# liupei101/AdvMIL

Measured on AMD Instinct MI355X. Metric: WSI bags/sec (full G+D step), higher is better.
Workload: dtype bf16x3 (fp32 operands split hi+lo, 3 bf16 MFMAs per product, fp32 accumulate; fp32 storage); 1 GPU; ABMIL+AdvMIL(RLIP prj discriminator), 8192-patch x 1024 fp32 bags (BASELINE.json configs[1] shape; fp32 storage, bf16x3 split arithmetic: >= the bf16 the config names, within 2e-5 of the fp32 reference); gen_updates=1, distinct_resident_bags_per_gpu=64, parallelism=bag-parallel dp1, dropout=shipped rates, launch=hipGraph replay (4 captured bag groups)

## Files before the change

advmil_amd/_lib.py:

```python
import ctypes
import os
from ctypes import c_float, c_int, c_int32, c_int64, c_size_t, c_uint64, c_void_p

LIB_PATH = os.environ.get("ADVMIL_HIP_LIB") or os.path.join(os.path.dirname(os.path.abspath(__file__)), "libadvmil_hip.so")


class HipLibraryMissing(RuntimeError):
    pass


class AdvmilHipError(RuntimeError):
    pass


class Epilogue(ctypes.Structure):
    _fields_ = [("bias", c_void_p), ("act0", c_int), ("act1", c_int), ("act_split", c_int), ("drop_p", c_float),
                ("seed", c_void_p), ("stream_id", c_uint64), ("rowv", c_void_p), ("colv", c_void_p), ("rowseg", c_void_p),
                ("maskref", c_void_p), ("ldmask", c_int), ("mask_scale", c_float), ("accumulate", c_int),
                ("alpha", c_float), ("a_hi", c_void_p), ("a_lo", c_void_p), ("b_hi", c_void_p), ("b_lo", c_void_p),
                ("c_hi", c_void_p), ("c_lo", c_void_p), ("gate_wc", c_void_p), ("gate_out", c_void_p), ("gate_np", c_int),
                ("rng_row", c_void_p), ("c2", c_void_p), ("ldc2", c_int64), ("n_split", c_int64), ("bias2", c_void_p), ("colsum", c_void_p), ("maskbits", c_void_p), ("ldbits", c_int64),
                ("gate_bits_a", c_void_p), ("gate_bits_b", c_void_p), ("ldgbits", c_int64), ("c_rows_pair32", c_int)]


class DenseLayer(ctypes.Structure):
    _fields_ = [("W", c_void_p), ("bias", c_void_p), ("dW", c_void_p), ("dbias", c_void_p), ("y", c_void_p), ("K", c_int), ("N", c_int),
                ("act", c_int), ("drop_p", c_float), ("stream_id", c_uint64)]


TAIL_MAXL = 3


class DTail(ctypes.Structure):
    _fields_ = [("B", c_int), ("nx", c_int), ("ny", c_int), ("prj_src", c_int), ("xin", c_void_p), ("tin", c_void_p),
                ("x", DenseLayer * TAIL_MAXL), ("y", DenseLayer * TAIL_MAXL), ("u", c_void_p), ("w_prj", c_void_p), ("b_prj", c_void_p),
                ("dw_prj", c_void_p), ("db_prj", c_void_p), ("seed", c_void_p), ("rng_row", c_void_p), ("out", c_void_p),
                ("dout", c_void_p), ("dxin", c_void_p), ("dtin", c_void_p), ("du", c_void_p)]


class GemmTnCall(ctypes.Structure):
    _fields_ = [("M", c_int64), ("N", c_int64), ("K", c_int64), ("A", c_void_p), ("lda", c_int64), ("B", c_void_p), ("ldb", c_int64),
                ("C", c_void_p), ("ldc", c_int64), ("accumulate", ctypes.c_int32)]


class GHead(ctypes.Structure):
    _fields_ = [("B", ctypes.c_int32), ("d0", ctypes.c_int32), ("d1", ctypes.c_int32), ("d2", ctypes.c_int32), ("noise_mode", ctypes.c_int32),
                ("out_act", ctypes.c_int32), ("x", c_void_p), ("ldx", c_int64), ("Wr", c_void_p), ("br", c_void_p), ("W0", c_void_p),
                ("b0", c_void_p), ("W1", c_void_p), ("b1", c_void_p), ("p1", c_float), ("p2", c_float), ("seed", c_void_p),
                ("sid1", c_uint64), ("sid2", c_uint64), ("sid_noise", c_uint64), ("rng_row", c_void_p), ("noise", c_void_p),
                ("hs", c_void_p), ("h2", c_void_p), ("pred", c_void_p), ("dpred", c_void_p), ("dx", c_void_p), ("lddx", c_int64),
                ("dWr", c_void_p), ("dbr", c_void_p), ("dW0", c_void_p), ("db0", c_void_p), ("dW1", c_void_p), ("db1", c_void_p),
                ("ws", c_void_p), ("ws_bytes", c_size_t)]


class GHeadK(ctypes.Structure):
    _fields_ = [("B", ctypes.c_int32), ("d0", ctypes.c_int32), ("d1", ctypes.c_int32), ("d2", ctypes.c_int32), ("K", ctypes.c_int32),
                ("noise_mode", ctypes.c_int32), ("out_act", ctypes.c_int32), ("reserved", ctypes.c_int32)] + GHead._fields_[6:]


class Optim(ctypes.Structure):
    _fields_ = [("kind", ctypes.c_int32), ("lookahead", ctypes.c_int32), ("n", c_int64), ("p", c_void_p), ("grad", c_void_p),
                ("s1", c_void_p), ("s2", c_void_p), ("wd", c_void_p), ("slow", c_void_p), ("lr", ctypes.c_double),
                ("beta1", ctypes.c_double), ("beta2", ctypes.c_double), ("eps", ctypes.c_double), ("schedule_decay", ctypes.c_double),
                ("grad_scale", c_float), ("l1_coef", c_float), ("la_alpha", c_float), ("la_k", ctypes.c_int32), ("tick", ctypes.c_int32),
                ("step", c_void_p), ("la_state", c_void_p), ("m_sched", c_void_p), ("p_hi", c_void_p), ("p_lo", c_void_p),
                ("abs_partial", c_void_p), ("clear_grad", ctypes.c_int32)]


OPT_KINDS = {"adam": 0, "adamw": 1, "nadam": 2, "radam": 3, "adadelta": 4}

CINDEX_BOOT_ROW_TILE = 256
CINDEX_BOOT_RESAMPLE_CHUNK = 8
CINDEX_BOOT_MAX_CHUNK_BLOCKS = 4096


SIGNATURES = {
    "advmil_version": (c_int, []),
    "advmil_gemm_f32_workspace_bytes": (c_size_t, [c_int64, c_int64, c_int]),
    "advmil_gemm_f32": (c_int, [c_int, c_int, c_int64, c_int64, c_int64, c_void_p, c_int64, c_void_p, c_int64, c_void_p,
                                c_int64, ctypes.POINTER(Epilogue), c_int, c_void_p, c_size_t, c_void_p]),
    "advmil_split_planes": (c_int, [c_void_p, c_int64, c_void_p, c_void_p, c_void_p]),
    "advmil_stage_bag": (c_int, [c_void_p, c_void_p, c_size_t, c_void_p, c_void_p, c_void_p, c_void_p, c_size_t, c_void_p]),
    "advmil_stage_bag_masked": (c_int, [c_void_p, c_void_p, c_size_t, c_int64, c_void_p, c_void_p, c_void_p, c_void_p, c_size_t, c_void_p,
                                        c_void_p]),
    "advmil_gate_interleave": (c_int, [c_void_p, c_void_p, c_void_p, c_void_p, c_int, c_void_p, c_void_p, c_void_p, c_void_p, c_int, c_void_p]),
    "advmil_gate_partial_sum": (c_int, [c_void_p, c_int, c_void_p, c_int64, c_void_p, c_void_p]),
    "advmil_gemm_f32_gate_blocks": (c_int, [c_int, c_int64]),
    "advmil_gemm_f32_colsum_rows": (c_int64, [c_int, c_int64, c_int64]),
    "advmil_merge_partials": (c_int, [c_void_p, c_int, c_int64, c_int64, c_void_p, c_int, c_void_p]),
    "advmil_set_gemm_mode": (c_int, [c_int]),
    "advmil_get_gemm_mode": (c_int, []),
    "advmil_gemm_f32_plan": (c_int, [c_int64, c_int64, c_int64, ctypes.POINTER(c_int), ctypes.POINTER(c_int)]),
    "advmil_gemm_f32_plan_layout": (c_int, [c_int, c_int, c_int64, c_int64, c_int64, ctypes.POINTER(c_int), ctypes.POINTER(c_int)]),
    "advmil_gemm_f32_plan_planes": (c_int, [c_int, c_int, c_int64, c_int64, c_int64, ctypes.POINTER(c_int)]),
    "advmil_gemm_f32_plan_tn_planes": (c_int, [c_int64, c_int64, c_int64, ctypes.POINTER(c_int), ctypes.POINTER(c_int)]),
    "advmil_gemm_f32_tiled": (c_int, [c_int, c_int, c_int64, c_int64, c_int64, c_void_p, c_int64, c_void_p, c_int64, c_void_p,
                                      c_int64, ctypes.POINTER(Epilogue), c_int, c_int, c_void_p, c_size_t, c_void_p]),
    "advmil_mha_fwd": (c_int, [c_void_p, c_void_p, c_int64, c_int, c_int, c_int, c_void_p, c_int64, c_float, c_void_p, c_uint64,
                               c_void_p, c_void_p, c_void_p, c_void_p]),
    "advmil_mha_fwd_lse": (c_int, [c_void_p, c_void_p, c_int64, c_int, c_int, c_int, c_void_p, c_int64, c_float, c_void_p, c_uint64,
                                   c_void_p, c_void_p, c_void_p, c_void_p]),
    "advmil_mha_bwd_workspace_bytes": (c_size_t, [c_int64, c_int, c_int]),
    "advmil_mha_bwd": (c_int, [c_void_p, c_void_p, c_void_p, c_void_p, c_void_p, c_int64, c_int, c_int, c_int, c_void_p, c_int64,
                               c_float, c_void_p, c_uint64, c_void_p, c_void_p, c_void_p, c_size_t, c_void_p]),
    "advmil_mha_bwd1_workspace_bytes": (c_size_t, [c_int64, c_int, c_int, c_int64]),
    "advmil_mha_bwd1": (c_int, [c_void_p, c_void_p, c_void_p, c_void_p, c_void_p, c_int64, c_int, c_int, c_int, c_void_p, c_int64,
                                c_float, c_void_p, c_uint64, c_void_p, c_void_p, c_void_p, c_size_t, c_void_p]),
    "advmil_add_dropout_ln_fwd": (c_int, [c_void_p, c_void_p, c_void_p, c_void_p, c_float, c_int64, c_int64, c_float, c_void_p,
                                          c_uint64, c_void_p, c_void_p, c_void_p, c_void_p, c_void_p, c_void_p, c_void_p, c_void_p]),
    "advmil_add_dropout_ln_bwd_workspace_bytes": (c_size_t, [c_int64, c_int64]),
    "advmil_add_dropout_ln_bwd": (c_int, [c_void_p, c_void_p, c_void_p, c_void_p, c_void_p, c_int64, c_int64, c_float, c_void_p,
                                          c_uint64, c_void_p, c_void_p, c_void_p, c_void_p, c_void_p, c_int, c_void_p, c_size_t,
                                          c_void_p]),
    "advmil_gate_score_fwd": (c_int, [c_void_p, c_void_p, c_void_p, c_float, c_void_p, c_uint64, c_uint64, c_int64, c_int64,
                                      c_void_p, c_void_p, c_void_p]),
    "advmil_softmax_pool_workspace_bytes": (c_size_t, [c_int64, c_int64, c_int]),
    "advmil_softmax_pool_fwd": (c_int, [c_void_p, c_void_p, c_int64, c_int64, c_int64, c_int, c_void_p, c_int64, c_void_p,
                                        c_void_p, c_void_p, c_size_t, c_void_p]),
    "advmil_softmax_pool_mean_workspace_bytes": (c_size_t, [c_int64, c_int64, c_int]),
    "advmil_softmax_pool_mean_fwd": (c_int, [c_void_p, c_void_p, c_int64, c_int64, c_int64, c_int, c_void_p, c_int64, c_void_p,
                                             c_void_p, c_void_p, c_void_p, c_size_t, c_void_p]),
    "advmil_softmax_pool_bwd": (c_int, [c_void_p, c_void_p, c_void_p, c_void_p, c_int64, c_int64, c_int64, c_int, c_void_p,
                                        c_int64, c_void_p, c_void_p, c_size_t, c_void_p]),
    "advmil_softmax_pool_fwd_planes": (c_int, [c_void_p, c_void_p, c_void_p, c_int64, c_int64, c_int64, c_int, c_void_p, c_int64, c_void_p,
                                               c_void_p, c_void_p, c_size_t, c_void_p]),
    "advmil_softmax_pool_bwd_planes": (c_int, [c_void_p, c_void_p, c_void_p, c_void_p, c_void_p, c_int64, c_int64, c_int64, c_int, c_void_p,
                                               c_int64, c_void_p, c_void_p, c_size_t, c_void_p]),
    "advmil_dropout_planes": (c_int, [c_void_p, c_void_p, c_int64, c_int64, c_float, c_void_p, c_uint64, c_void_p, c_void_p, c_void_p, c_void_p,
                                      c_float, c_uint64, c_uint64, c_void_p, c_void_p, c_void_p]),
    "advmil_gate_bwd_workspace_bytes": (c_size_t, [c_int64, c_int64]),
    "advmil_gate_bwd": (c_int, [c_void_p, c_void_p, c_void_p, c_float, c_void_p, c_uint64, c_uint64, c_int64, c_int64,
                                c_void_p, c_void_p, c_void_p, c_void_p, c_int, c_void_p, c_void_p, c_void_p, c_int, c_void_p, c_size_t,
                                c_void_p]),
    "advmil_colsum_workspace_bytes": (c_size_t, [c_int64, c_int64]),
    "advmil_act_dropout_bwd": (c_int, [c_void_p, c_void_p, c_int, c_float, c_void_p, c_uint64, c_int64, c_int64, c_void_p,
                                       c_void_p, c_int, c_void_p, c_void_p, c_void_p, c_void_p, c_void_p, c_size_t, c_void_p]),
    "advmil_colsum": (c_int, [c_void_p, c_int64, c_int64, c_void_p, c_int, c_void_p, c_size_t, c_void_p]),
    "advmil_ln_relu_mean16_fwd": (c_int, [c_void_p, c_void_p, c_void_p, c_float, c_int64, c_int64, c_void_p, c_void_p,
                                          c_void_p, c_void_p, c_void_p, c_int, c_void_p]),
    "advmil_ln_relu_mean16_bwd_workspace_bytes": (c_size_t, [c_int64, c_int64]),
    "advmil_ln_relu_mean16_bwd": (c_int, [c_void_p, c_void_p, c_void_p, c_void_p, c_void_p, c_void_p, c_int64, c_int64,
                                          c_void_p, c_void_p, c_void_p, c_int, c_void_p, c_void_p, c_void_p, c_int, c_void_p, c_size_t, c_void_p]),
    "advmil_ln_relu_fwd": (c_int, [c_void_p, c_void_p, c_void_p, c_float, c_int64, c_int64, c_void_p, c_void_p, c_void_p, c_void_p]),
    "advmil_ln_relu_bwd_workspace_bytes": (c_size_t, [c_int64, c_int64]),
    "advmil_ln_relu_bwd": (c_int, [c_void_p, c_void_p, c_void_p, c_void_p, c_void_p, c_void_p, c_int64, c_int64, c_void_p,
                                   c_void_p, c_void_p, c_int, c_void_p, c_size_t, c_void_p]),
    "advmil_gcn_res_fwd": (c_int, [c_void_p, c_void_p, c_int64, c_void_p, c_void_p, c_float, c_int64, c_int64, c_float, c_void_p,
                                   c_uint64, c_void_p, c_void_p, c_int64, c_void_p, c_void_p, c_void_p]),
    "advmil_gcn_res_bwd_workspace_bytes": (c_size_t, [c_int64, c_int64]),
    "advmil_gcn_res_bwd": (c_int, [c_void_p, c_int64, c_void_p, c_void_p, c_void_p, c_void_p, c_void_p, c_int64, c_int64, c_float,
                                   c_void_p, c_uint64, c_void_p, c_void_p, c_void_p, c_int64, c_int, c_void_p, c_void_p, c_int,
                                   c_void_p, c_size_t, c_void_p]),
    "advmil_gapool16_fwd": (c_int, [c_void_p, c_void_p, c_int64, c_int64, c_int64, c_void_p, c_void_p, c_int, c_void_p]),
    "advmil_gapool16_bwd": (c_int, [c_void_p, c_void_p, c_void_p, c_int64, c_int64, c_int64, c_int, c_void_p, c_void_p, c_int, c_void_p]),
    "advmil_genconv_fwd": (c_int, [c_void_p, c_void_p, c_void_p, c_void_p, c_float, c_int64, c_int64, c_void_p, c_void_p,
                                   c_void_p, c_void_p]),
    "advmil_genconv_bwd_workspace_bytes": (c_size_t, [c_int64, c_int64]),
    "advmil_genconv_bwd": (c_int, [c_void_p, c_void_p, c_void_p, c_void_p, c_void_p, c_void_p, c_void_p, c_float, c_int64,
                                   c_int64, c_void_p, c_void_p, c_void_p, c_size_t, c_void_p]),
    "advmil_adam_step": (c_int, [c_void_p, c_void_p, c_void_p, c_void_p, c_void_p, c_int64, c_float, c_float, c_float,
                                 c_float, c_float, c_float, c_void_p, c_void_p, c_void_p, c_int, c_void_p, c_int, c_void_p]),
    "advmil_adam_blocks": (c_int, [c_int64]),
    "advmil_optim_step": (c_int, [ctypes.POINTER(Optim), c_void_p]),
    "advmil_step_seed_tick": (c_int, [c_void_p, c_void_p, c_void_p, c_uint64, c_void_p]),
    "advmil_abs_sum": (c_int, [c_void_p, c_int64, c_void_p, c_void_p, c_size_t, c_void_p]),
    "advmil_abs_sum_workspace_bytes": (c_size_t, [c_int64]),
    "advmil_uniform_fill": (c_int, [c_void_p, c_int64, c_void_p, c_uint64, c_void_p, c_int64, c_void_p]),
    "advmil_dropout_apply": (c_int, [c_void_p, c_void_p, c_int64, c_float, c_void_p, c_uint64, c_void_p, c_int64, c_void_p]),
    "advmil_seed_advance": (c_int, [c_void_p, c_uint64, c_void_p]),
    "advmil_seg_scale_rows": (c_int, [c_void_p, c_void_p, c_void_p, c_int64, c_int64, c_void_p, c_void_p]),
    "advmil_stamp_clock": (c_int, [c_void_p, c_void_p]),
    "advmil_clock_rate_khz": (c_int64, []),
    "advmil_small_linear_fwd": (c_int, [c_void_p, c_int64, c_void_p, c_void_p, c_int, c_int, c_int, c_int, c_float, c_void_p, c_uint64,
                                        c_void_p, c_void_p, c_void_p]),
    "advmil_small_linear_bwd_workspace_bytes": (c_size_t, [c_int, c_int]),
    "advmil_small_linear_bwd": (c_int, [c_void_p, c_void_p, c_void_p, c_int64, c_void_p, c_int, c_int, c_int, c_int, c_float, c_void_p,
                                        c_uint64, c_void_p, c_void_p, c_int, c_void_p, c_int, c_void_p, c_int64, c_void_p, c_size_t, c_void_p]),
    "advmil_skinny_linear_fwd": (c_int, [c_void_p, c_void_p, c_void_p, c_int, c_int, c_int, c_int, c_void_p, c_void_p]),
    "advmil_skinny_linear_bwd": (c_int, [c_void_p, c_void_p, c_void_p, c_void_p, c_int, c_int, c_int, c_int, c_void_p, c_void_p,
                                         c_void_p, c_int, c_void_p]),
    "advmil_prj_head_fwd": (c_int, [c_void_p, c_void_p, c_void_p, c_void_p, c_void_p, c_int, c_int, c_void_p, c_void_p]),
    "advmil_prj_head_bwd": (c_int, [c_void_p, c_void_p, c_void_p, c_void_p, c_void_p, c_int, c_int, c_void_p, c_void_p, c_void_p, c_void_p,
                                    c_void_p, c_int, c_void_p]),
    "advmil_gan_d_loss": (c_int, [c_void_p, c_int, c_void_p, c_void_p, c_int, c_int, c_float, c_float, c_void_p, c_void_p, c_void_p, c_void_p]),
    "advmil_gan_g_loss": (c_int, [c_void_p, c_void_p, c_void_p, c_void_p, c_void_p, c_int, c_float, c_float, c_int, c_float, c_float,
                                  c_float, c_void_p, c_void_p, c_void_p, c_void_p]),
    "advmil_gan_g_loss_disc": (c_int, [c_void_p, c_void_p, c_void_p, c_void_p, c_void_p, c_int, c_int, c_float, c_float, c_float, c_float,
                                       c_float, c_void_p, c_void_p, c_void_p, c_void_p]),
    "advmil_mask_rows": (c_int, [c_void_p, c_void_p, c_int64, c_int64, c_void_p, c_void_p]),
    "advmil_dx_chain_fwd": (c_int, [c_void_p, c_int64, c_int, c_void_p, c_void_p, c_void_p, c_void_p, c_void_p, c_void_p, c_void_p, c_void_p,
                                    c_void_p, c_void_p, c_void_p, c_float, c_float, c_void_p, c_uint64, c_uint64, c_uint64, c_void_p, c_void_p,
                                    c_void_p, c_void_p, c_void_p, c_void_p]),
    "advmil_dx_chain_bwd_workspace_bytes": (c_size_t, [c_int64, c_int]),
    "advmil_dx_chain_prep": (c_int, [c_void_p, c_void_p, c_void_p, c_int, c_void_p, c_void_p, c_void_p, c_void_p, c_void_p, c_void_p, c_void_p]),
    "advmil_dx_chain_bwd": (c_int, [c_int64, c_int, c_void_p, c_void_p, c_void_p, c_void_p, c_void_p, c_void_p, c_void_p, c_void_p, c_void_p,
                                    c_void_p, c_float, c_float, c_void_p, c_uint64, c_uint64, c_void_p, c_void_p, c_void_p, c_void_p, c_void_p,
                                    c_void_p, c_void_p, c_void_p, c_void_p, c_void_p, c_void_p, c_void_p, c_void_p, c_void_p, c_void_p, c_void_p,
                                    c_void_p, c_size_t, c_void_p]),
    "advmil_dtail_fwd": (c_int, [ctypes.POINTER(DTail), c_void_p]),
    "advmil_dtail_bwd": (c_int, [ctypes.POINTER(DTail), c_void_p]),
    "advmil_gemm_tn_group_workspace_bytes": (c_size_t, [ctypes.POINTER(GemmTnCall), c_int]),
    "advmil_gemm_tn_group": (c_int, [ctypes.POINTER(GemmTnCall), c_int, c_void_p, c_size_t, c_void_p]),
    "advmil_ghead_workspace_bytes": (c_size_t, [c_int, c_int, c_int, c_int]),
    "advmil_ghead_fwd": (c_int, [ctypes.POINTER(GHead), c_void_p]),
    "advmil_ghead_bwd": (c_int, [ctypes.POINTER(GHead), c_void_p]),
    "advmil_gheadk_workspace_bytes": (c_size_t, [c_int, c_int, c_int, c_int, c_int]),
    "advmil_gheadk_fwd": (c_int, [ctypes.POINTER(GHeadK), c_void_p]),
    "advmil_gheadk_bwd": (c_int, [ctypes.POINTER(GHeadK), c_void_p]),
# ... 69 lines not shown
```

advmil_amd/csrc/gemm_core.h:

```cpp
#pragma once
#include <cstdlib>
#include "common.h"
#include "bf16split.h"
#include "sumq.h"
#include "../../include/advmil_hip.h"

#define BK 32
#define PITCH_KC 36

#define WAVE_LDS_SYNC()                                   \
  do {                                                    \
    __builtin_amdgcn_fence(__ATOMIC_RELEASE, "wavefront"); \
    __builtin_amdgcn_s_waitcnt(0xc07f);                   \
    __builtin_amdgcn_wave_barrier();                      \
    __builtin_amdgcn_fence(__ATOMIC_ACQUIRE, "wavefront"); \
  } while (0)

struct GemmArgs {
  int64_t M, N, K;
  const float* A; int64_t lda;
  const float* B; int64_t ldb;
  float* C; int64_t ldc;
  int64_t k_chunk;
  float* ws;
  int splits;
  int mtiles, ntiles;
  advmil_epilogue_t epi;
};

__device__ __forceinline__ float epilogue_elem(const advmil_epilogue_t& e, float acc, int64_t m, int64_t n, int64_t N,
                                               uint64_t key, float inv_keep) {
  float v = acc * e.alpha;
  if (e.bias) v += e.bias[n];
  if (e.rowv) v += e.rowv[m] * e.colv[(e.rowseg ? (int64_t)e.rowseg[m] * N : 0) + n];
  v = act_apply(n < e.act_split ? e.act0 : e.act1, v);
  if (e.seed && e.drop_p > 0.0f) v *= rng_keep(key, (uint64_t)((e.rng_row ? e.rng_row[m] : m) * N + n), e.drop_p, inv_keep);
  if (e.maskref) v *= (e.maskref[m * (int64_t)e.ldmask + n] > 0.0f ? e.mask_scale : 0.0f);
  return v;
}

template <bool KC, int ROWS, int BKT, int NT>
__device__ __forceinline__ void load_tile(const float* __restrict__ src, int64_t ld, int64_t row0, int64_t rows,
                                          int64_t k0, int64_t kend, int tid, float4 (&r)[ROWS * BKT / (4 * NT)]) {
#pragma unroll
  for (int p = 0; p < ROWS * BKT / (4 * NT); ++p) {
    const int e = p * NT + tid;
    if (KC) {
      const int64_t row = row0 + e / (BKT / 4);
      const int64_t k = k0 + (e % (BKT / 4)) * 4;
      r[p] = (row < rows && k < kend) ? *reinterpret_cast<const float4*>(src + row * ld + k) : make_float4(0.f, 0.f, 0.f, 0.f);
    } else {
      const int64_t k = k0 + e / (ROWS / 4);
      const int64_t m = row0 + (e % (ROWS / 4)) * 4;
      r[p] = (k < kend && m < rows) ? *reinterpret_cast<const float4*>(src + k * ld + m) : make_float4(0.f, 0.f, 0.f, 0.f);
    }
  }
}

template <bool KC, int ROWS, int BKT, int NT>
__device__ __forceinline__ void store_tile(float* __restrict__ s, int tid, const float4 (&r)[ROWS * BKT / (4 * NT)]) {
#pragma unroll
  for (int p = 0; p < ROWS * BKT / (4 * NT); ++p) {
    const int e = p * NT + tid;
    if (KC)
      *reinterpret_cast<float4*>(s + (e / (BKT / 4)) * (BKT + 4) + (e % (BKT / 4)) * 4) = r[p];
    else
      *reinterpret_cast<float4*>(s + (e / (ROWS / 4)) * ROWS + (e % (ROWS / 4)) * 4) = r[p];
  }
}

template <bool KC, int ROWS, int BKT>
__device__ __forceinline__ void read_frag(const float* __restrict__ s, int rbase, int t4, int i, int hi, float (&f)[4]) {
  if (KC) {
    const float4 v = *reinterpret_cast<const float4*>(s + (rbase + i) * (BKT + 4) + t4 * 8 + hi * 4);
    f[0] = v.x; f[1] = v.y; f[2] = v.z; f[3] = v.w;
  } else {
#pragma unroll
    for (int u = 0; u < 4; ++u) f[u] = s[(t4 * 8 + hi * 4 + u) * ROWS + rbase + i];
  }
}


#define PITCH_PS(BKT) (BKT)
__device__ __forceinline__ int ps_unit(int row, int unit, int units_per_row) {
  return units_per_row == 2 ? (unit ^ ((row >> 3) & 1)) : (unit ^ ((row >> 2) & (units_per_row - 1)));
}

template <int ROWS, int BKT, int NT>
__device__ __forceinline__ void store_tile_presplit(bf16raw* __restrict__ planes, int tid, const float4 (&r)[ROWS * BKT / (4 * NT)]) {
  bf16raw* const hiP = planes;
  bf16raw* const loP = planes + ROWS * PITCH_PS(BKT);
#pragma unroll
  for (int p = 0; p < ROWS * BKT / (4 * NT); ++p) {
    const int e = p * NT + tid;
    const int row = e / (BKT / 4), p4 = e % (BKT / 4);
    const int off = row * PITCH_PS(BKT) + ps_unit(row, p4 >> 1, BKT / 8) * 8 + (p4 & 1) * 4;
    uint2 h, l;
    split4(r[p], h, l);
    *reinterpret_cast<uint2*>(hiP + off) = h;
    *reinterpret_cast<uint2*>(loP + off) = l;
  }
}

template <int ROWS, int BKT>
__device__ __forceinline__ void read_frag_presplit(const bf16raw* __restrict__ planes, int rbase, int ks, int i, int hi,
                                                   bf16x8& h, bf16x8& l) {
  const int row = rbase + i;
  const bf16raw* p = planes + row * PITCH_PS(BKT) + ps_unit(row, ks * 2 + hi, BKT / 8) * 8;
  Frag8 a, b;
  a.u = *reinterpret_cast<const uint4*>(p);
  b.u = *reinterpret_cast<const uint4*>(p + ROWS * PITCH_PS(BKT));
  h = a.v; l = b.v;
}

template <int BKT>
__device__ __forceinline__ void read_frag_hi(const bf16raw* __restrict__ planes, int rbase, int ks, int i, int hi, bf16x8& h) {
  const int row = rbase + i;
  Frag8 a;
  a.u = *reinterpret_cast<const uint4*>(planes + row * PITCH_PS(BKT) + ps_unit(row, ks * 2 + hi, BKT / 8) * 8);
  h = a.v;
}

#define PITCH_MC(ROWS) ((ROWS) + 32)

template <int ROWS, int BKT, int NT>
__device__ __forceinline__ void store_tile_presplit_mc(bf16raw* __restrict__ planes, int tid, const float4 (&r)[ROWS * BKT / (4 * NT)]) {
  bf16raw* const hiP = planes;
  bf16raw* const loP = planes + BKT * PITCH_MC(ROWS);
#pragma unroll
  for (int p = 0; p < ROWS * BKT / (4 * NT); ++p) {
    const int e = p * NT + tid;
    const int k = e / (ROWS / 4), m4 = (e % (ROWS / 4)) * 4;
    uint2 h, l;
    split4(r[p], h, l);
    *reinterpret_cast<uint2*>(hiP + k * PITCH_MC(ROWS) + m4) = h;
    *reinterpret_cast<uint2*>(loP + k * PITCH_MC(ROWS) + m4) = l;
  }
}

template <int ROWS, int BKT>
__device__ __forceinline__ void read_frag_presplit_mc(const bf16raw* __restrict__ planes, int rbase, int ks, int lane,
                                                      bf16x8& h, bf16x8& l) {
  const int krow = ks * 16 + (lane >> 5) * 8 + ((lane & 15) >> 2);
  const int mcol = rbase + ((lane >> 4) & 1) * 16 + (lane & 3) * 4;
  const bf16raw* p = planes + krow * PITCH_MC(ROWS) + mcol;
  union { bf16x4_t q[2]; bf16x8 v; } a, b;
  a.q[0] = __builtin_amdgcn_ds_read_tr16_b64_v4bf16((LDS_AS bf16x4_t*)(p));
  a.q[1] = __builtin_amdgcn_ds_read_tr16_b64_v4bf16((LDS_AS bf16x4_t*)(p + 4 * PITCH_MC(ROWS)));
  b.q[0] = __builtin_amdgcn_ds_read_tr16_b64_v4bf16((LDS_AS bf16x4_t*)(p + BKT * PITCH_MC(ROWS)));
  b.q[1] = __builtin_amdgcn_ds_read_tr16_b64_v4bf16((LDS_AS bf16x4_t*)(p + (BKT + 4) * PITCH_MC(ROWS)));
  h = a.v; l = b.v;
}

__device__ __forceinline__ void emit_planes4(const advmil_epilogue_t& e, int64_t off, const float (&v)[4], int nvalid) {
  union { __bf16 b[4]; uint2 u; bf16raw r[4]; } h, l;
#pragma unroll
  for (int j = 0; j < 4; ++j) {
    h.b[j] = (__bf16)v[j];
    l.b[j] = (__bf16)(v[j] - (float)h.b[j]);
  }
  bf16raw* ch = reinterpret_cast<bf16raw*>(e.c_hi) + off;
  bf16raw* cl = reinterpret_cast<bf16raw*>(e.c_lo) + off;
  if (nvalid == 4 && ((off & 3) == 0)) {
    *reinterpret_cast<uint2*>(ch) = h.u;
    *reinterpret_cast<uint2*>(cl) = l.u;
  } else {
#pragma unroll
    for (int j = 0; j < 4; ++j)
// ... 37 lines not shown

  __device__ __forceinline__ void store(bf16raw* __restrict__ planes, int tid) const {
    if constexpr (!PRE) {
      if (KC) store_tile_presplit<ROWS, BKT, NT>(planes, tid, f);
      else store_tile_presplit_mc<ROWS, BKT, NT>(planes, tid, f);
    } else {
#pragma unroll
      for (int p = 0; p < NP; ++p) {
        const int e = p * NT + tid;
        if (!FULL && e >= NPIECE) break;
        if (KC) {
          const int row = e / (BKT / 8);
          bf16raw* d = planes + row * PITCH_PS(BKT) + ps_unit(row, e % (BKT / 8), BKT / 8) * 8;
          *reinterpret_cast<uint4*>(d) = ph[p];
          *reinterpret_cast<uint4*>(d + ROWS * PITCH_PS(BKT)) = pl[p];
        } else {
          bf16raw* d = planes + (e / (ROWS / 8)) * PITCH_MC(ROWS) + (e % (ROWS / 8)) * 8;
          *reinterpret_cast<uint4*>(d) = ph[p];
          *reinterpret_cast<uint4*>(d + BKT * PITCH_MC(ROWS)) = pl[p];
        }
      }
    }
  }
};

#define EPI_WAVE_FLOATS(TM, TN) (32 * PITCH_KC + 32 * ((TN) + 2 * (TM)) + 32 * (TM) * (TN))

template <int TM, int TN, int WR, int WC, bool PLAIN = false>
__device__ __forceinline__ void gemm_epilogue_stream(const GemmArgs& g, f32x16 (&acc)[TM][TN], float* patch, int lane, int wr, int wc,
                                                     int64_t m0, int64_t n0, uint64_t key, float inv_keep, int nt_i = 0) {
  const advmil_epilogue_t& e = g.epi;
  const int i = lane & 31, hi = lane >> 5;
  const int c4 = (lane & 7) * 4, rq = lane >> 3;
  const int64_t N = g.N, ldo = g.ldc;
  float* const out = g.C;
  const bool drop = !PLAIN && e.seed && e.drop_p > 0.0f;
  const bool mapped = drop && e.rng_row;
  const int kind = PLAIN ? 0 : (e.rowv ? 1 : (e.maskref ? 2 : (e.accumulate ? 3 : 0)));
  const bool rmask = !PLAIN && kind == 1 && e.maskref != nullptr;
  const bool csum = !PLAIN && e.colsum != nullptr;
  const bool bmask = !PLAIN && e.maskbits != nullptr;
  const bool gpair = PLAIN && e.gate_wc != nullptr && e.gate_bits_a != nullptr;
  const float* const xbase = kind == 1 ? e.colv : (kind == 2 ? e.maskref : out);
  const int64_t xld = kind == 1 ? N : (kind == 2 ? (int64_t)e.ldmask : ldo);
  const int64_t rbase = m0 + wr * 32 * TM, cbase = n0 + wc * 32 * TN;
  const int64_t nsp = (PLAIN && e.c2) ? e.n_split : N;
  float* const sbias = patch + 32 * PITCH_KC;
  int* const srow_i = reinterpret_cast<int*>(sbias + 32 * TN);
  float* const srow_f = sbias + 32 * TN + 32 * TM;
  uint32_t* const smask = reinterpret_cast<uint32_t*>(sbias + 32 * TN + 64 * TM);
  if (gpair) {
    constexpr int NW = 32 * TM * TN;
    uint32_t mv[(NW + 63) / 64];
#pragma unroll
    for (int u = 0; u < (NW + 63) / 64; ++u) {
      const int idx = u * 64 + lane;
      const int br = idx & 1, pu = (idx >> 1) % (TN / 2), row = (idx >> 1) / (TN / 2);
      const uint32_t* src = br ? e.gate_bits_b : e.gate_bits_a;
      mv[u] = idx < NW ? src[(rbase + row) * e.ldgbits + (cbase >> 6) + pu] : 0u;
    }
#pragma unroll
    for (int u = 0; u < (NW + 63) / 64; ++u)
      if (u * 64 + lane < NW) smask[u * 64 + lane] = mv[u];
  }
  if (bmask) {
    uint32_t mv[(32 * TM * TN + 63) / 64];
#pragma unroll
    for (int u = 0; u < (32 * TM * TN + 63) / 64; ++u) {
      const int idx = u * 64 + lane;
      mv[u] = idx < 32 * TM * TN ? e.maskbits[(rbase + idx / TN) * e.ldbits + (cbase >> 5) + idx % TN] : 0u;
    }
#pragma unroll
    for (int u = 0; u < (32 * TM * TN + 63) / 64; ++u)
      if (u * 64 + lane < 32 * TM * TN) smask[u * 64 + lane] = mv[u];
  }
  {
    float bv[(32 * TN + 63) / 64];
    int iv[(32 * TM + 63) / 64];
    float fv[(32 * TM + 63) / 64];
#pragma unroll
    for (int u = 0; u < (32 * TN + 63) / 64; ++u) {
      const int c = u * 64 + lane;
      const int64_t cg = cbase + c;
      bv[u] = c >= 32 * TN ? 0.f : (cg < nsp ? (e.bias ? e.bias[cg] : 0.f) : (e.bias2 ? e.bias2[cg - nsp] : 0.f));
    }
#pragma unroll
    for (int u = 0; u < (32 * TM + 63) / 64; ++u) {
      const int r = u * 64 + lane;
      const bool ok = r < 32 * TM;
      iv[u] = !ok ? 0 : (kind == 1 ? (e.rowseg ? e.rowseg[rbase + r] : 0) : (mapped ? (int)e.rng_row[rbase + r] : 0));
      fv[u] = (ok && kind == 1) ? e.rowv[rbase + r] : ((gpair && r < 16 * TN) ? e.gate_wc[(cbase >> 1) + r] : 0.f);
    }
#pragma unroll
    for (int u = 0; u < (32 * TN + 63) / 64; ++u)
      if (u * 64 + lane < 32 * TN) sbias[u * 64 + lane] = bv[u];
#pragma unroll
    for (int u = 0; u < (32 * TM + 63) / 64; ++u)
      if (u * 64 + lane < 32 * TM) { srow_i[u * 64 + lane] = iv[u]; srow_f[u * 64 + lane] = fv[u]; }
    WAVE_LDS_SYNC();
  }
  float4 ext[4], ext2[4];
  float cs[TN][4];
  float gpa[4][4], gps[TM][4];
#pragma unroll
  for (int a_ = 0; a_ < TM; ++a_)
#pragma unroll
    for (int q = 0; q < 4; ++q) gps[a_][q] = 0.f;
#pragma unroll
  for (int q = 0; q < 4; ++q) { ext[q] = make_float4(0.f, 0.f, 0.f, 0.f); ext2[q] = make_float4(1.f, 1.f, 1.f, 1.f); }
#pragma unroll
  for (int b = 0; b < TN; ++b)
#pragma unroll
    for (int t = 0; t < 4; ++t) cs[b][t] = 0.f;
#define ADVMIL_EPI_PREFETCH(a_, b_)                                                                             \
  do {                                                                                                          \
    if (kind != 0) {                                                                                            \
      _Pragma("unroll") for (int q = 0; q < 4; ++q) {                                                           \
        const int rr_ = (a_) * 32 + q * 8 + rq;                                                                 \
        const int64_t xrow_ = kind == 1 ? (int64_t)srow_i[rr_] : rbase + rr_;                                   \
        ext[q] = *reinterpret_cast<const float4*>(xbase + xrow_ * xld + cbase + (b_) * 32 + c4);                \
        if (rmask) ext2[q] = *reinterpret_cast<const float4*>(e.maskref + (rbase + rr_) * (int64_t)e.ldmask + cbase + (b_) * 32 + c4); \
      }                                                                                                         \
    }                                                                                                           \
  } while (0)
  ADVMIL_EPI_PREFETCH(0, 0);
#pragma unroll
  for (int a = 0; a < TM; ++a) {
#pragma unroll
    for (int b = 0; b < TN; ++b) {
      const int64_t col = cbase + b * 32 + c4;
#pragma unroll
      for (int r = 0; r < 16; ++r) patch[((r & 3) + 8 * (r >> 2) + 4 * hi) * PITCH_KC + i] = acc[a][b][r];
      WAVE_LDS_SYNC();
      float res[4][4];
#pragma unroll
      for (int q = 0; q < 4; ++q) {
        const float4 v4 = *reinterpret_cast<const float4*>(patch + (q * 8 + rq) * PITCH_KC + c4);
        res[q][0] = v4.x; res[q][1] = v4.y; res[q][2] = v4.z; res[q][3] = v4.w;
      }
      const float4 b4 = *reinterpret_cast<const float4*>(sbias + b * 32 + c4);
      WAVE_LDS_SYNC();
      const int act = gpair ? ((b & 1) ? ACT_SIGMOID : ACT_TANH) : (cbase + b * 32 < e.act_split ? e.act0 : e.act1);
      const float bb[4] = {b4.x, b4.y, b4.z, b4.w};
      if (!drop && kind == 0 && !bmask) {
        const float al = e.alpha;
        if (act == ACT_RELU) {
#pragma unroll
          for (int q = 0; q < 4; ++q)
#pragma unroll
            for (int t = 0; t < 4; ++t) res[q][t] = fmaxf(res[q][t] * al + bb[t], 0.0f);
        } else if (act == ACT_NONE) {
#pragma unroll
          for (int q = 0; q < 4; ++q)
#pragma unroll
            for (int t = 0; t < 4; ++t) res[q][t] = res[q][t] * al + bb[t];
        } else if (act == ACT_TANH) {
#pragma unroll
          for (int q = 0; q < 4; ++q)
#pragma unroll
            for (int t = 0; t < 4; ++t) res[q][t] = act_apply(ACT_TANH, res[q][t] * al + bb[t]);
        } else {
#pragma unroll
          for (int q = 0; q < 4; ++q)
#pragma unroll
            for (int t = 0; t < 4; ++t) res[q][t] = act_apply(ACT_SIGMOID, res[q][t] * al + bb[t]);
        }
      } else if (!drop && kind == 1 && act == ACT_NONE && !rmask && !bmask) {
// ... 124 lines not shown
#pragma unroll
      for (int q = 0; q < 4; ++q) {
        float t = gps[a_][q];
        t += __shfl_xor(t, 1, 64); t += __shfl_xor(t, 2, 64); t += __shfl_xor(t, 4, 64);
        if ((lane & 7) == 0) e.gate_out[(rbase + a_ * 32 + q * 8 + rq) * e.gate_np + nt_i * WC + wc] = t;
      }
  }
  if (csum) {
    const int64_t prow = (m0 / (32 * TM * WR)) * WR + wr;
#pragma unroll
    for (int b = 0; b < TN; ++b) {
#pragma unroll
      for (int t = 0; t < 4; ++t) {
        float v = cs[b][t];
        v += __shfl_xor(v, 8, 64); v += __shfl_xor(v, 16, 64); v += __shfl_xor(v, 32, 64);
        cs[b][t] = v;
      }
      if (rq == 0) *reinterpret_cast<float4*>(e.colsum + prow * N + cbase + b * 32 + c4) = make_float4(cs[b][0], cs[b][1], cs[b][2], cs[b][3]);
    }
  }
}

template <int TM, int TN, int WR, int WC, bool RAWBAR = false, int EPI = 0>
__device__ __forceinline__ int gemm_epilogue(const GemmArgs& g, f32x16 (&acc)[TM][TN], float* smem, int wave, int lane, int wr, int wc,
                                             int64_t m0, int64_t n0, int z, int nt_i) {
  const int i = lane & 31, hi = lane >> 5;
  const advmil_epilogue_t& e = g.epi;
  const bool direct = (g.splits == 1);
  uint64_t key = 0;
  float inv_keep = 1.0f;
  if (direct && e.seed && e.drop_p > 0.0f) {
    key = rng_key(*e.seed, e.stream_id);
    inv_keep = hw_rcp(1.0f - e.drop_p);
  } else if (direct && e.gate_bits_a && e.drop_p > 0.0f) {
    inv_keep = hw_rcp(1.0f - e.drop_p);
  }
  float* const out = direct ? g.C : g.ws + (int64_t)z * g.M * g.N;
  const int64_t ldo = direct ? g.ldc : g.N;
  const bool vec_ok = ((ldo & 3) == 0) && (((uintptr_t)out & 15) == 0);
  float* const patch = smem + wave * EPI_WAVE_FLOATS(TM, TN);
  if constexpr (RAWBAR) {
    asm volatile("s_waitcnt lgkmcnt(0)" ::: "memory");
    __builtin_amdgcn_s_barrier();
    asm volatile("" ::: "memory");
  } else {
    __syncthreads();
  }
  const bool gate_store = direct && e.gate_wc != nullptr && e.gate_bits_a != nullptr;
  const bool gate_mode = direct && e.gate_wc != nullptr && !gate_store;
  if constexpr (TM * TN >= 4 && EPI != 1) {
    const int nmode = (e.rowv && e.maskref && !e.accumulate) ? 1 : (e.rowv ? 1 : 0) + (e.maskref ? 1 : 0) + (e.accumulate ? 1 : 0);
    const bool stream = direct && !gate_mode && vec_ok && (g.N % (32 * TN * WC)) == 0 && (g.M % (32 * TM * WR)) == 0 && (e.act_split & 31) == 0 &&
                        nmode <= 1 && !(e.rowv && e.seed && e.rng_row) && (!e.bias || ((uintptr_t)e.bias & 15) == 0) && (!e.rowv || ((uintptr_t)e.colv & 15) == 0) &&
                        (!e.maskref || ((e.ldmask & 3) == 0 && ((uintptr_t)e.maskref & 15) == 0)) &&
                        (!e.c_hi || ((((uintptr_t)e.c_hi) | ((uintptr_t)e.c_lo)) & 7) == 0) &&
                        (!e.c2 || ((((uintptr_t)e.c2) & 15) == 0 && (e.ldc2 & 3) == 0 && (e.n_split & 31) == 0));
    if (stream) {
      if constexpr (EPI == 2) {
        if (nmode == 0 && !(e.seed && e.drop_p > 0.0f)) {
          gemm_epilogue_stream<TM, TN, WR, WC, true>(g, acc, patch, lane, wr, wc, m0, n0, key, inv_keep, nt_i);
          return TM * TN * 4;
        }
      } else {
        gemm_epilogue_stream<TM, TN, WR, WC>(g, acc, patch, lane, wr, wc, m0, n0, key, inv_keep);
        return nmode == 0 ? TM * TN * 4 : 0;
      }
    }
  }
#pragma unroll
  for (int a = 0; a < TM; ++a) {
    float gsum[4] = {0.f, 0.f, 0.f, 0.f};
#pragma unroll
    for (int b = 0; b < TN; ++b) {
#pragma unroll
      for (int r = 0; r < 16; ++r) patch[((r & 3) + 8 * (r >> 2) + 4 * hi) * PITCH_KC + i] = acc[a][b][r];
      WAVE_LDS_SYNC();
      const int64_t rbase = m0 + wr * 32 * TM + a * 32;
      if (gate_mode) {
        const int64_t col = n0 + wc * 32 * TN + b * 32 + (lane & 7) * 4;
        float w0 = 0.f, w1 = 0.f;
        float4 b4 = make_float4(0.f, 0.f, 0.f, 0.f);
        if (col < g.N) {
          w0 = e.gate_wc[col >> 1]; w1 = e.gate_wc[(col >> 1) + 1];
          if (e.bias) b4 = *reinterpret_cast<const float4*>(e.bias + col);
        }
#pragma unroll
        for (int q = 0; q < 4; ++q) {
          const int pr = q * 8 + (lane >> 3);
          const float4 v4 = *reinterpret_cast<const float4*>(patch + pr * PITCH_KC + (lane & 7) * 4);
          const float t0 = act_apply(ACT_TANH, v4.x * e.alpha + b4.x), s0 = act_apply(ACT_SIGMOID, v4.y * e.alpha + b4.y);
          const float t1 = act_apply(ACT_TANH, v4.z * e.alpha + b4.z), s1 = act_apply(ACT_SIGMOID, v4.w * e.alpha + b4.w);
          gsum[q] += t0 * s0 * w0 + t1 * s1 * w1;
        }
        WAVE_LDS_SYNC();
        continue;
      }
      const int64_t col = n0 + wc * 32 * TN + b * 32 + (lane & 7) * 4;
      const int nvalid = col >= g.N ? 0 : ((g.N - col >= 4) ? 4 : (int)(g.N - col));
      float bias4[4] = {0.f, 0.f, 0.f, 0.f};
      int act4[4];
#pragma unroll
      for (int t = 0; t < 4; ++t) {
        if (direct && e.bias && t < nvalid) bias4[t] = e.bias[col + t];
        act4[t] = (col + t) < e.act_split ? e.act0 : e.act1;
      }
      const bool same_act = act4[0] == act4[3];
#pragma unroll 1
      for (int q = 0; q < 4; ++q) {
        const int pr = q * 8 + (lane >> 3);
        const int64_t row = rbase + pr;
        const float4 v4 = *reinterpret_cast<const float4*>(patch + pr * PITCH_KC + (lane & 7) * 4);
        float v[4] = {v4.x, v4.y, v4.z, v4.w};
        if (row < g.M && nvalid > 0) {
          float* c = out + row * ldo + col;
          if (direct) {
            float r1 = 0.f;
            const float* cv = nullptr;
            const int64_t grow = (e.seed && e.rng_row) ? e.rng_row[row] : row;
            if (e.rowv) {
              r1 = e.rowv[row];
              cv = e.colv + (e.rowseg ? (int64_t)e.rowseg[row] * g.N : 0) + col;
            }
#pragma unroll
            for (int t = 0; t < 4; ++t)
              if (t < nvalid) {
                float x = v[t] * e.alpha + bias4[t];
                if (cv) x += r1 * cv[t];
                x = act_apply(same_act ? act4[0] : act4[t], x);
                if (e.seed && e.drop_p > 0.0f) x *= rng_keep(key, (uint64_t)(grow * g.N + col + t), e.drop_p, inv_keep);
                if (e.maskref) x *= (e.maskref[row * (int64_t)e.ldmask + col + t] > 0.0f ? e.mask_scale : 0.0f);
                if (e.accumulate) x += c[t];
                v[t] = x;
              }
          }
          if (!out) {
          } else if (nvalid == 4 && vec_ok) {
            *reinterpret_cast<float4*>(c) = make_float4(v[0], v[1], v[2], v[3]);
          } else {
#pragma unroll
            for (int t = 0; t < 4; ++t)
              if (t < nvalid) c[t] = v[t];
          }
          if (direct && e.c_hi) emit_planes4(e, row * ldo + col, v, nvalid);
        }
      }
      WAVE_LDS_SYNC();
    }
    if (gate_mode) {
#pragma unroll
      for (int q = 0; q < 4; ++q) {
        float t = gsum[q];
        t += __shfl_xor(t, 1, 64); t += __shfl_xor(t, 2, 64); t += __shfl_xor(t, 4, 64);
        const int64_t row = m0 + wr * 32 * TM + a * 32 + q * 8 + (lane >> 3);
        if ((lane & 7) == 0 && row < g.M) e.gate_out[row * e.gate_np + nt_i * WC + wc] = t;
      }
    }
  }
  return 0;
}

#define GLB_AS __attribute__((address_space(1)))
template <int N>
__device__ __forceinline__ void wait_vmcnt() { asm volatile("s_waitcnt vmcnt(%0)" ::"n"(N) : "memory"); }
```

advmil_amd/csrc/gemm_host.hip:

```cpp
#include "gemm_core.h"

int advmil_launch_generic(int tile, int a_kc, int b_kc, int pre, dim3 grid, hipStream_t stream, const GemmArgs& g);
int advmil_launch_nt_planes(int tile, bool a_single, dim3 pgrid, hipStream_t stream, const GemmArgs& g);
int advmil_launch_tn_planes(int tile, bool b_single, dim3 tgrid, hipStream_t stream, const GemmArgs& g);
int advmil_launch_splitk_reduce(const GemmArgs& g, hipStream_t stream);

extern "C" size_t advmil_gemm_f32_workspace_bytes(int64_t M, int64_t N, int splits) {
  return splits > 1 ? (size_t)splits * (size_t)M * (size_t)N * sizeof(float) : 0;
}

int g_gemm_mode = 0;
static int g_nt_planes = []() { const char* e = getenv("ADVMIL_NT_PLANES"); return (e && e[0] == '0') ? 0 : 1; }();
extern "C" int advmil_set_gemm_mode(int mode) {
  if (mode != 0 && mode != 1) return ADVMIL_EINVAL;
  g_gemm_mode = mode;
  return ADVMIL_OK;
}
extern "C" int advmil_get_gemm_mode(void) { return g_gemm_mode; }

static int planes_usable(const void* hi, const void* lo, int64_t ld, int64_t contiguous_extent) {
  return hi && !((uintptr_t)hi & 15) && !((uintptr_t)lo & 15) && !(ld & 7) && !(contiguous_extent & 7);
}

static int64_t n_tiles(int tile, int64_t M, int64_t N) {
// ... 132 lines not shown
  return ((M % bm) || (N % bn)) ? 0 : (M / bm) * wr;
}

static int device_cus() {
  static const int ncu = []() { int dev = 0, n = 0; hipGetDevice(&dev); hipDeviceGetAttribute(&n, hipDeviceAttributeMultiprocessorCount, dev); return n > 0 ? n : 256; }();
  return ncu;
}

extern "C" int advmil_merge_partials(const float* partial, int nblk, int64_t stride, int64_t ncols, float* out, int accumulate,
                                     advmil_stream_t stream) {
  if (!partial || !out || nblk <= 0 || ncols <= 0 || stride < ncols) return ADVMIL_EINVAL;
  return advmil_sumq((hipStream_t)stream, partial, nblk, stride, ncols, out, accumulate);
}

extern "C" int advmil_gemm_f32_tiled(int a_kc, int b_kc, int64_t M, int64_t N, int64_t K, const float* A, int64_t lda,
                                     const float* B, int64_t ldb, float* C, int64_t ldc, const advmil_epilogue_t* epi,
                                     int splits, int tile, void* ws, size_t ws_bytes, advmil_stream_t stream_) {
  hipStream_t stream = (hipStream_t)stream_;
  if (!A || !B || !epi || (!C && !epi->gate_wc && !epi->c_hi) || M <= 0 || N <= 0 || K <= 0) return ADVMIL_EINVAL;
  if (!C && !epi->gate_wc && (epi->accumulate || splits != 1 || (epi->c2 && tile != 85 && tile != 86))) return ADVMIL_EINVAL;
  if ((lda & 3) || (ldb & 3)) return ADVMIL_EINVAL;
  if (lda < (a_kc ? K : M) || ldb < (b_kc ? K : N)) return ADVMIL_EINVAL;
  if (ldc < (epi->c2 ? (int64_t)epi->n_split : N) && (C || epi->c_hi)) return ADVMIL_EINVAL;
  if (a_kc ? (K & 3) : (M & 3)) return ADVMIL_EINVAL;
  if (b_kc ? (K & 3) : (N & 3)) return ADVMIL_EINVAL;
  if (((uintptr_t)A & 15) || ((uintptr_t)B & 15)) return ADVMIL_EINVAL;
  if (splits < 1) splits = 1;
  const int64_t kchunks = (K + BK - 1) / BK;
  if (splits > kchunks) splits = (int)kchunks;
  if (splits > 1 && (N & 3)) return ADVMIL_EINVAL;
  GemmArgs g;
  g.M = M; g.N = N; g.K = K; g.A = A; g.lda = lda; g.B = B; g.ldb = ldb; g.C = C; g.ldc = ldc;
  g.k_chunk = ((kchunks + splits - 1) / splits) * BK;
  splits = (int)((K + g.k_chunk - 1) / g.k_chunk);
  g.splits = splits;
  g.ws = (float*)ws;
  g.epi = *epi;
  if (splits > 1) {
    if (!ws || ws_bytes < advmil_gemm_f32_workspace_bytes(M, N, splits)) return ADVMIL_EWORKSPACE;
    if ((uintptr_t)ws & 15) return ADVMIL_EINVAL;
  }
  if (tile == 0) { int t = 0, sp = 0; advmil_gemm_f32_plan_layout(a_kc, b_kc, M, N, K, &t, &sp); tile = t; }
  if (g_gemm_mode != 1) {
    if (tile / 10 == 4) tile = 20 + tile % 10;
    else if (tile % 10 == 4) tile = (tile / 10 == 3) ? 23 : 22;
  }
  const int tm = tile / 10, tn = tile % 10;
  g.mtiles = (int)((M + 64 * tm - 1) / (64 * tm));
  const int ntiles = (int)((N + 64 * tn - 1) / (64 * tn));
  g.ntiles = ntiles;
  dim3 grid(g.mtiles * ntiles, splits);
  int pre = 0;
  if (g_gemm_mode == 1) {
    if (planes_usable(epi->a_hi, epi->a_lo, lda, a_kc ? K : M)) pre |= 1;
    if (planes_usable(epi->b_hi, epi->b_lo, ldb, b_kc ? K : N)) pre |= 2;
  }
  if ((epi->c_hi != nullptr) != (epi->c_lo != nullptr)) return ADVMIL_EINVAL;
  if (epi->c_rows_pair32 && (splits < 2 || !epi->accumulate || (M & 63) || ldc != N)) return ADVMIL_EINVAL;
  if (epi->maskbits) {
    int tm_, tn_, wr_, wc_;
    if (g_gemm_mode != 1 || splits != 1 || !tile_geom(tile, tm_, tn_, wr_, wc_) || tm_ * tn_ < 4 || epi->gate_wc || epi->maskref || epi->accumulate ||
        (M % (32 * tm_ * wr_)) || (N % (32 * tn_ * wc_)) || (epi->act_split & 31) || epi->ldbits < N / 32 || (epi->seed && epi->drop_p > 0.0f && epi->rowv && epi->rng_row))
      return ADVMIL_EINVAL;
    if ((C && ((((uintptr_t)C) & 15) || (ldc & 3))) || (((uintptr_t)epi->bias) & 15) || (epi->rowv && (((uintptr_t)epi->colv) & 15)) ||
        (epi->c_hi && ((((uintptr_t)epi->c_hi) | ((uintptr_t)epi->c_lo)) & 7)) || epi->c2)
      return ADVMIL_EINVAL;
  }
  if (epi->colsum) {
    int tm_, tn_, wr_, wc_;
    if (g_gemm_mode != 1 || splits != 1 || !tile_geom(tile, tm_, tn_, wr_, wc_) || tm_ * tn_ < 4 || epi->gate_wc || epi->accumulate ||
        (epi->seed && epi->drop_p > 0.0f))
      return ADVMIL_EINVAL;
    if ((M % (32 * tm_ * wr_)) || (N % (32 * tn_ * wc_)) || (((uintptr_t)epi->colsum) & 15) || (epi->act_split & 31)) return ADVMIL_EINVAL;
  }
  const bool gate_store = epi->gate_wc && epi->gate_bits_a;
  if (gate_store && (!epi->gate_bits_b || !C || (tile != 85 && tile != 86) || epi->seed || !(epi->drop_p > 0.0f) || epi->drop_p >= 1.0f ||
                     (N & 127) || epi->ldgbits < N / 64 || epi->c2 || epi->c_hi || (((uintptr_t)epi->gate_wc) & 15)))
    return ADVMIL_EINVAL;
  if (epi->gate_wc) {
    if (splits != 1 || !epi->gate_out || (N & 3) || (epi->drop_p > 0.0f && !gate_store)) return ADVMIL_EINVAL;
    if (epi->gate_np != advmil_gemm_f32_gate_blocks(tile, N)) return ADVMIL_EINVAL;
  }
  if (tile == 0 && pre == 3 && splits == 1) { int t = 0; advmil_gemm_f32_plan_planes(a_kc, b_kc, M, N, K, &t); if (t) tile = t; }
  if (tile == 87) {
    if (epi->gate_wc || epi->rowv || epi->maskref || epi->maskbits || epi->colsum || epi->accumulate || epi->c2 || (epi->seed && epi->drop_p > 0.0f))
      return ADVMIL_EINVAL;
    if (g_gemm_mode != 1 || !a_kc || !b_kc || pre != 3 || splits != 1 || (M % 512) || N != 128 || K < 64 || (K % 32) || !epi->b_lo) return ADVMIL_EINVAL;
    if ((uint64_t)M * (uint64_t)lda * 2 >= (1ull << 32) || (uint64_t)N * (uint64_t)ldb * 2 >= (1ull << 32)) return ADVMIL_EINVAL;
    g.mtiles = (int)(M / 512);
    g.ntiles = 1;
    const int cus = device_cus();
    return advmil_launch_nt_planes(tile, !epi->a_lo, dim3(g.mtiles < cus ? g.mtiles : cus), stream, g);
  }
  if (tile >= 82 && tile <= 86) {
    const int tnp = tile == 85 ? 4 : tile == 86 ? 2 : tile % 10, bm = 256, bkt = 32;
    const bool plain = tile == 85 || tile == 86;
    if (tile == 84 && !epi->gate_wc) return ADVMIL_EINVAL;
    if (plain && ((epi->gate_wc && !gate_store) || epi->rowv || epi->maskref || epi->accumulate || (epi->seed && epi->drop_p > 0.0f))) return ADVMIL_EINVAL;
    if (epi->c2) {
      if (!plain || epi->n_split <= 0 || epi->n_split >= N || (epi->n_split & 31) || (epi->ldc2 & 3) || ((uintptr_t)epi->c2 & 15) ||
          epi->act_split != epi->n_split)
        return ADVMIL_EINVAL;
      if ((ldc & 3) || (((uintptr_t)C) & 15) || (((uintptr_t)epi->bias) & 15) || (epi->c_hi && ((((uintptr_t)epi->c_hi) | ((uintptr_t)epi->c_lo)) & 7)))
        return ADVMIL_EINVAL;
    }
    if (g_gemm_mode != 1 || !a_kc || !b_kc || pre != 3 || splits != 1 || (M % bm) || (K % bkt) || (N % (64 * tnp))) return ADVMIL_EINVAL;
    if (epi->gate_wc && (!epi->gate_out || (epi->drop_p > 0.0f && !gate_store) || epi->gate_np != advmil_gemm_f32_gate_blocks(tile, N))) return ADVMIL_EINVAL;
    if (K < 64) return ADVMIL_EINVAL;
    if ((uint64_t)M * (uint64_t)lda * 2 >= (1ull << 32) || (uint64_t)N * (uint64_t)ldb * 2 >= (1ull << 32)) return ADVMIL_EINVAL;
    g.mtiles = (int)(M / bm);
    g.ntiles = (int)(N / (64 * tnp));
    const int ncu = device_cus();
    const int ntile_all = g.mtiles * g.ntiles;
    dim3 pgrid(ntile_all < ncu ? ntile_all : ncu);
    if (!epi->b_lo) return ADVMIL_EINVAL;
    return advmil_launch_nt_planes(tile, !epi->a_lo, pgrid, stream, g);
  }
  if (tile >= 91 && tile <= 93) {
    const int bm = tile == 91 ? 128 : 256, bn = tile == 92 ? 128 : 256;
    if (g_gemm_mode != 1 || a_kc || b_kc || pre != 3 || (M % bm) || (N % bn) || (K % 32) || (g.k_chunk % 32)) return ADVMIL_EINVAL;
    if (g.k_chunk / 32 < 3 || epi->gate_wc || epi->c2) return ADVMIL_EINVAL;
    if ((uint64_t)32 * (uint64_t)lda * 2 + (uint64_t)M * 2 >= (1ull << 32) || (uint64_t)32 * (uint64_t)ldb * 2 + (uint64_t)N * 2 >= (1ull << 32)) return ADVMIL_EINVAL;
    g.mtiles = (int)(M / bm);
    g.ntiles = (int)(N / bn);
    const int gs = M >= N ? g.ntiles : g.mtiles, og = M >= N ? g.mtiles : g.ntiles;
    const dim3 tgrid((unsigned)(8 * ((splits * og + 7) / 8) * gs));
    if (!epi->a_lo) return ADVMIL_EINVAL;
    { const int rc = advmil_launch_tn_planes(tile, !epi->b_lo, tgrid, stream, g); if (rc) return rc; }
    if (splits > 1) {
      const int rc = advmil_launch_splitk_reduce(g, stream);
      if (rc) return rc;
    }
    return ADVMIL_OK;
  }
  { const int rc = advmil_launch_generic(tile, a_kc, b_kc, pre, grid, stream, g); if (rc) return rc; }
  if (splits > 1) {
    const int rc = advmil_launch_splitk_reduce(g, stream);
    if (rc) return rc;
  }
  return ADVMIL_OK;
}

extern "C" int advmil_gemm_f32(int a_kc, int b_kc, int64_t M, int64_t N, int64_t K, const float* A, int64_t lda,
                               const float* B, int64_t ldb, float* C, int64_t ldc, const advmil_epilogue_t* epi,
                               int splits, void* ws, size_t ws_bytes, advmil_stream_t stream) {
  return advmil_gemm_f32_tiled(a_kc, b_kc, M, N, K, A, lda, B, ldb, C, ldc, epi, splits, 0, ws, ws_bytes, stream);
}
```

advmil_amd/csrc/gemm_nt_planes.hip:

```cpp
#include "gemm_core.h"


template <int TN, int NBUF, int WR, int BKT, int EPI = 0, int ALO = 1, int TM = 2>
__global__ __launch_bounds__(128 * WR, 2) void gemm_nt_planes_kernel(GemmArgs g) {
  constexpr int WC = 2, NW = WR * WC;
  constexpr int BM_ = 32 * TM * WR, BN_ = 64 * TN;
  constexpr int AROWS = (1 + ALO) * BM_;
  constexpr int ROWS_ALL = AROWS + 2 * BN_;
  constexpr int RPP = 512 / BKT, LPR = BKT / 8;
  constexpr int NPIECE = ROWS_ALL / RPP, PPW = NPIECE / NW;
  static_assert(NPIECE % NW == 0, "pieces must divide evenly over the waves");
  constexpr int BUF_HW = ROWS_ALL * BKT;
  constexpr int PATCH_FLOATS = NW * EPI_WAVE_FLOATS(TM, TN);
  constexpr bool EPI_IN_SLOT = PATCH_FLOATS <= BUF_HW / 2;
  static_assert(EPI_IN_SLOT || ALO == 0, "the epilogue area must fit one ring slot");
  constexpr int EST = TM * TN * 4;
  static_assert(EST + PPW <= 63, "counted waits are 6-bit");
  __shared__ __attribute__((aligned(16))) float smem[NBUF * BUF_HW / 2 + (EPI_IN_SLOT ? 0 : PATCH_FLOATS)];
  bf16raw* const lds = reinterpret_cast<bf16raw*>(smem);
  const int wave = __builtin_amdgcn_readfirstlane((int)threadIdx.x >> 6);
  const int wr = wave / WC, wc = wave % WC;
  const int ntile = g.mtiles * g.ntiles, G = (int)gridDim.x;
  auto tile_of = [&](int v, int& mt, int& nt) {
    const int inner = g.ntiles, outer = g.mtiles;
    const int per_group = 8 * inner, full = (outer / 8) * per_group;
    if (v < full) {
      const int r = v % per_group;
      mt = (v / per_group) * 8 + (r & 7);
      nt = r >> 3;
    } else {
      const int rem = outer - (outer / 8) * 8, r = v - full;
      mt = (outer / 8) * 8 + r % rem;
      nt = r / rem;
    }
  };
  int v = (int)blockIdx.x;
  int mt_i, nt_i;
  tile_of(v, mt_i, nt_i);
  uint32_t soff[PPW];
  auto set_src = [&](int mt, int nt, int lane) {
#pragma unroll
    for (int it = 0; it < PPW; ++it) {
      const int prow = (wave + NW * it) * RPP + lane / LPR;
      int r;
      int64_t ld, row0;
      if (prow < BM_) { r = prow; ld = g.lda; row0 = (int64_t)mt * BM_; }
      else if (prow < AROWS) { r = prow - BM_; ld = g.lda; row0 = (int64_t)mt * BM_; }
      else if (prow < AROWS + BN_) { r = prow - AROWS; ld = g.ldb; row0 = (int64_t)nt * BN_; }
      else { r = prow - AROWS - BN_; ld = g.ldb; row0 = (int64_t)nt * BN_; }
      soff[it] = (uint32_t)(((row0 + r) * ld + ps_unit(r, lane % LPR, LPR) * 8) * 2);
    }
  };
  set_src(mt_i, nt_i, (int)threadIdx.x & 63);
  int64_t dA = 0, dB = 0;
  auto dma = [&](int buf, int64_t k0, bool next) {
#pragma unroll
    for (int it = 0; it < PPW; ++it) {
      const int p0 = (wave + NW * it) * RPP;
      const char* base = reinterpret_cast<const char*>(p0 < BM_ ? g.epi.a_hi : (p0 < AROWS ? g.epi.a_lo : (p0 < AROWS + BN_ ? g.epi.b_hi : g.epi.b_lo)));
      base += (k0 + (next ? (p0 < AROWS ? dA : dB) : 0)) * 2;
      __builtin_amdgcn_global_load_lds((const GLB_AS void*)(base + soff[it]), (LDS_AS void*)(lds + buf * BUF_HW + (wave + NW * it) * 512), 16, 0, 0);
    }
  };
  const int64_t K = g.K;
  const int C = (int)(K / BKT);
  dma(0, 0, false);
  if (NBUF == 3) dma(1, BKT, false);
  int cur = 0;
  int young = 0;
  for (; v < ntile; v += G) {
    int lane = (int)threadIdx.x & 63;
    asm volatile("" : "+v"(lane));
    const int i = lane & 31, hi = lane >> 5;
    const bool has_next = v + G < ntile;
    const int64_t m0 = (int64_t)mt_i * BM_, n0 = (int64_t)nt_i * BN_;
    int mt_n = mt_i, nt_n = nt_i;
    if (has_next) tile_of(v + G, mt_n, nt_n);
    dA = (int64_t)(mt_n - mt_i) * BM_ * g.lda;
    dB = (int64_t)(nt_n - nt_i) * BN_ * g.ldb;
    f32x16 acc[TM][TN];
#pragma unroll
    for (int a = 0; a < TM; ++a)
#pragma unroll
      for (int b = 0; b < TN; ++b)
#pragma unroll
        for (int r = 0; r < 16; ++r) acc[a][b][r] = 0.0f;
    for (int c = 0; c < C; ++c) {
      const bool more = c + 1 < C || has_next;
      if constexpr (NBUF == 3) {
        const bool st = young && c < 2;
        if (more) { if (st) wait_vmcnt<PPW + EST>(); else wait_vmcnt<PPW>(); }
        else { if (st) wait_vmcnt<EST>(); else wait_vmcnt<0>(); }
      } else {
        if (young && c == 0) wait_vmcnt<EST>(); else wait_vmcnt<0>();
      }
      __builtin_amdgcn_s_barrier();
      asm volatile("" ::: "memory");
      {
        const int pc = c + NBUF - 1;
        const int pbuf = cur == 0 ? NBUF - 1 : cur - 1;
        if (pc < C) dma(pbuf, (int64_t)pc * BKT, false);
        else if (has_next) dma(pbuf, (int64_t)(pc - C) * BKT, true);
      }
      const bf16raw* cA = lds + cur * BUF_HW;
      const bf16raw* cB = cA + AROWS * BKT;
#pragma unroll
      for (int ks = 0; ks < BKT / 16; ++ks) {
        bf16x8 ah[TM], al[TM], bh[TN], bl[TN];
#pragma unroll
        for (int a = 0; a < TM; ++a) {
          if constexpr (ALO) read_frag_presplit<BM_, BKT>(cA, wr * 32 * TM + a * 32, ks, i, hi, ah[a], al[a]);
          else read_frag_hi<BKT>(cA, wr * 32 * TM + a * 32, ks, i, hi, ah[a]);
        }
#pragma unroll
        for (int b = 0; b < TN; ++b) read_frag_presplit<BN_, BKT>(cB, wc * 32 * TN + b * 32, ks, i, hi, bh[b], bl[b]);
#pragma unroll
        for (int a = 0; a < TM; ++a)
#pragma unroll
          for (int b = 0; b < TN; ++b) {
            if constexpr (ALO) acc[a][b] = __builtin_amdgcn_mfma_f32_32x32x16_bf16(al[a], bh[b], acc[a][b], 0, 0, 0);
            acc[a][b] = __builtin_amdgcn_mfma_f32_32x32x16_bf16(ah[a], bl[b], acc[a][b], 0, 0, 0);
            acc[a][b] = __builtin_amdgcn_mfma_f32_32x32x16_bf16(ah[a], bh[b], acc[a][b], 0, 0, 0);
          }
      }
      cur = cur == NBUF - 1 ? 0 : cur + 1;
    }
    const int last = cur == 0 ? NBUF - 1 : cur - 1;
    young = gemm_epilogue<TM, TN, WR, WC, true, EPI>(g, acc, EPI_IN_SLOT ? smem + last * (BUF_HW / 2) : smem + NBUF * (BUF_HW / 2), wave, lane, wr,
                                                     wc, m0, n0, 0, nt_i);
    mt_i = mt_n; nt_i = nt_n;
    if (has_next) {
      int lane2 = (int)threadIdx.x & 63;
      asm volatile("" : "+v"(lane2));
      set_src(mt_i, nt_i, lane2);
    }
  }
}


int advmil_launch_nt_planes(int tile, bool a_single, dim3 pgrid, hipStream_t stream, const GemmArgs& g) {
  if (a_single) {
    switch (tile) {
      case 85: hipLaunchKernelGGL((gemm_nt_planes_kernel<4, 2, 4, 32, 2, 0>), pgrid, dim3(512), 0, stream, g); break;
      case 86: hipLaunchKernelGGL((gemm_nt_planes_kernel<2, 3, 4, 32, 2, 0>), pgrid, dim3(512), 0, stream, g); break;
      case 83: hipLaunchKernelGGL((gemm_nt_planes_kernel<3, 2, 4, 32, 0, 0>), pgrid, dim3(512), 0, stream, g); break;
      case 82: hipLaunchKernelGGL((gemm_nt_planes_kernel<2, 3, 4, 32, 0, 0>), pgrid, dim3(512), 0, stream, g); break;
      case 87: hipLaunchKernelGGL((gemm_nt_planes_kernel<2, 2, 4, 32, 2, 0, 4>), pgrid, dim3(512), 0, stream, g); break;
      default: return ADVMIL_EINVAL;
    }
    ADVMIL_LAUNCH_CHECK();
    return ADVMIL_OK;
  }
  switch (tile) {
    case 84: hipLaunchKernelGGL((gemm_nt_planes_kernel<4, 2, 4, 32, 1>), pgrid, dim3(512), 0, stream, g); break;
    case 85: hipLaunchKernelGGL((gemm_nt_planes_kernel<4, 2, 4, 32, 2>), pgrid, dim3(512), 0, stream, g); break;
    case 86: hipLaunchKernelGGL((gemm_nt_planes_kernel<2, 3, 4, 32, 2>), pgrid, dim3(512), 0, stream, g); break;
    case 83: hipLaunchKernelGGL((gemm_nt_planes_kernel<3, 2, 4, 32>), pgrid, dim3(512), 0, stream, g); break;
    case 82: hipLaunchKernelGGL((gemm_nt_planes_kernel<2, 3, 4, 32>), pgrid, dim3(512), 0, stream, g); break;
    case 87: hipLaunchKernelGGL((gemm_nt_planes_kernel<2, 2, 4, 32, 2, 1, 4>), pgrid, dim3(512), 0, stream, g); break;
    default: return ADVMIL_EINVAL;
  }
  ADVMIL_LAUNCH_CHECK();
// ... 3 lines not shown
```

advmil_amd/csrc/pool.hip:

```cpp
#include <cstdlib>
#include "common.h"
#include "bf16split.h"
#include "sumq.h"
#include "../../include/advmil_hip.h"

#define ROWS_PER_BLOCK 32
static inline int rows_per_block(int64_t rows) {
  int64_t r = (rows + 1023) / 1024;
  r = (r + 31) / 32 * 32;
  if (r < ROWS_PER_BLOCK) r = ROWS_PER_BLOCK;
  if (r > 512) r = 512;
  return (int)r;
}

struct RowColMap {
  int cols4, rpp, c4, r;
  bool active;
};
__device__ __forceinline__ RowColMap make_map(int64_t D) {
  RowColMap m;
  m.cols4 = (int)(D >> 2);
  m.rpp = 256 / m.cols4;
  if (m.rpp < 1) m.rpp = 1;
  m.c4 = threadIdx.x % m.cols4;
// ... 215 lines not shown
  __shared__ __attribute__((aligned(16))) float red[1024];
  const RowColMap m = make_map(D);
  const int b = blockIdx.y;
  int64_t beg, end;
  seg_range(seg_ptr, b, N, beg, end);
  const float mx = stats[2 * b], inv = stats[2 * b + 1];
  const int64_t r0 = beg + (int64_t)blockIdx.x * rpb;
  float4 acc = make_float4(0.f, 0.f, 0.f, 0.f);
  if (m.active) {
    for (int r = m.r; r < rpb; r += m.rpp) {
      const int64_t n = r0 + r;
      if (n >= end) break;
      const float w = hw_exp(s[n] - mx) * inv;
      if (m.c4 == 0) A[n] = w;
      const float4 v = *reinterpret_cast<const float4*>(h + n * ldh + m.c4 * 4);
      acc.x += w * v.x; acc.y += w * v.y; acc.z += w * v.z; acc.w += w * v.w;
    }
  }
  const float4 t = reduce_rows(acc, m, red);
  if (m.active && m.r == 0)
    *reinterpret_cast<float4*>(partial + ((int64_t)b * gridDim.x + blockIdx.x) * D + m.c4 * 4) = t;
}

__global__ __launch_bounds__(256) void pool_partial8_kernel(const float* __restrict__ s, const float* __restrict__ h, int64_t ldh,
                                                            int64_t N, int64_t D, const int64_t* __restrict__ seg_ptr,
                                                            const float* __restrict__ stats, float* __restrict__ A,
                                                            float* __restrict__ partial, int rpb) {
  __shared__ __attribute__((aligned(16))) float red[2048];
  const int cols8 = (int)(D >> 3), rpp = 256 / cols8;
  const int c8 = threadIdx.x % cols8, rl = threadIdx.x / cols8;
  const int b = blockIdx.y;
  int64_t beg, end;
  seg_range(seg_ptr, b, N, beg, end);
  const float mx = stats[2 * b], inv = stats[2 * b + 1];
  const int64_t r0 = beg + (int64_t)blockIdx.x * rpb;
  float acc[8];
#pragma unroll
  for (int j = 0; j < 8; ++j) acc[j] = 0.f;
  if (rl < rpp) {
#pragma unroll 4
    for (int r = rl; r < rpb; r += rpp) {
      const int64_t n = r0 + r;
      const bool ok = n < end;
      const int64_t nn = ok ? n : beg;
      const float w = ok ? hw_exp(s[nn] - mx) * inv : 0.f;
      const float4 v0 = *reinterpret_cast<const float4*>(h + nn * ldh + c8 * 8);
      const float4 v1 = *reinterpret_cast<const float4*>(h + nn * ldh + c8 * 8 + 4);
      if (ok && c8 == 0) A[n] = w;
      acc[0] += w * v0.x; acc[1] += w * v0.y; acc[2] += w * v0.z; acc[3] += w * v0.w;
      acc[4] += w * v1.x; acc[5] += w * v1.y; acc[6] += w * v1.z; acc[7] += w * v1.w;
    }
    float* dst = red + (int64_t)rl * D + c8 * 8;
    *reinterpret_cast<float4*>(dst) = make_float4(acc[0], acc[1], acc[2], acc[3]);
    *reinterpret_cast<float4*>(dst + 4) = make_float4(acc[4], acc[5], acc[6], acc[7]);
  }
  __syncthreads();
  if ((int)threadIdx.x < (int)(D >> 2)) {
    float4 t = make_float4(0.f, 0.f, 0.f, 0.f);
    for (int q = 0; q < rpp; ++q) {
      const float4 v = *reinterpret_cast<const float4*>(red + (int64_t)q * D + threadIdx.x * 4);
      t.x += v.x; t.y += v.y; t.z += v.z; t.w += v.w;
    }
    *reinterpret_cast<float4*>(partial + ((int64_t)b * gridDim.x + blockIdx.x) * D + threadIdx.x * 4) = t;
  }
}

__device__ __forceinline__ void planes8(const bf16raw* __restrict__ hi, const bf16raw* __restrict__ lo, int64_t off, float4& v0, float4& v1) {
  const uint4 a = *reinterpret_cast<const uint4*>(hi + off);
  const uint4 b = *reinterpret_cast<const uint4*>(lo + off);
  v0.x = __uint_as_float(a.x << 16) + __uint_as_float(b.x << 16);
  v0.y = __uint_as_float(a.x & 0xffff0000u) + __uint_as_float(b.x & 0xffff0000u);
  v0.z = __uint_as_float(a.y << 16) + __uint_as_float(b.y << 16);
  v0.w = __uint_as_float(a.y & 0xffff0000u) + __uint_as_float(b.y & 0xffff0000u);
  v1.x = __uint_as_float(a.z << 16) + __uint_as_float(b.z << 16);
  v1.y = __uint_as_float(a.z & 0xffff0000u) + __uint_as_float(b.z & 0xffff0000u);
  v1.z = __uint_as_float(a.w << 16) + __uint_as_float(b.w << 16);
  v1.w = __uint_as_float(a.w & 0xffff0000u) + __uint_as_float(b.w & 0xffff0000u);
}

template <bool MEAN, bool PL = false>
__global__ __launch_bounds__(256) void pool_partial8_online_kernel(const float* __restrict__ s, const float* __restrict__ h, int64_t ldh,
                                                                   int64_t N, int64_t D, const int64_t* __restrict__ seg_ptr,
                                                                   float* __restrict__ partial, float* __restrict__ pstats, int rpb,
                                                                   float* __restrict__ mpartial, const bf16raw* __restrict__ hlo = nullptr) {
  __shared__ __attribute__((aligned(16))) float red[2048];
  __shared__ float wts[512];
  __shared__ float wred[8];
  const int cols8 = (int)(D >> 3), rpp = 256 / cols8;
  const int c8 = threadIdx.x % cols8, rl = threadIdx.x / cols8;
  const int tid = threadIdx.x, lane = tid & 63, w = tid >> 6;
  const int b = blockIdx.y;
  int64_t beg, end;
  seg_range(seg_ptr, b, N, beg, end);
  const int64_t r0 = beg + (int64_t)blockIdx.x * rpb;
  float* pst = pstats + ((int64_t)b * gridDim.x + blockIdx.x) * 2;
  float* prow = partial + ((int64_t)b * gridDim.x + blockIdx.x) * D;
  float* mrow = MEAN ? mpartial + ((int64_t)b * gridDim.x + blockIdx.x) * D : nullptr;
  if (r0 >= end) {
    if (tid < (int)(D >> 2)) {
      *reinterpret_cast<float4*>(prow + tid * 4) = make_float4(0.f, 0.f, 0.f, 0.f);
      if (MEAN) *reinterpret_cast<float4*>(mrow + tid * 4) = make_float4(0.f, 0.f, 0.f, 0.f);
    }
    if (tid == 0) { pst[0] = -INFINITY; pst[1] = 0.f; }
    return;
  }
  float mx = -INFINITY;
  for (int r = tid; r < rpb; r += 256) {
    const int64_t n = r0 + r;
    const float v = n < end ? s[n] : -INFINITY;
    wts[r] = v;
    mx = fmaxf(mx, v);
  }
  mx = wave_max(mx);
  if (lane == 0) wred[w] = mx;
  __syncthreads();
  mx = fmaxf(fmaxf(wred[0], wred[1]), fmaxf(wred[2], wred[3]));
  float ls = 0.f;
  for (int r = tid; r < rpb; r += 256) {
    const float e = (r0 + r < end) ? hw_exp(wts[r] - mx) : 0.f;
    wts[r] = e;
    ls += e;
  }
  ls = wave_sum(ls);
  if (lane == 0) wred[4 + w] = ls;
  __syncthreads();
  if (tid == 0) { pst[0] = mx; pst[1] = (wred[4] + wred[5]) + (wred[6] + wred[7]); }
  float acc[8], macc[8];
#pragma unroll
  for (int j = 0; j < 8; ++j) { acc[j] = 0.f; macc[j] = 0.f; }
  if (rl < rpp) {
#pragma unroll 4
    for (int r = rl; r < rpb; r += rpp) {
      const int64_t n = r0 + r;
      const int64_t nn = n < end ? n : beg;
      const float wgt = wts[r];
      float4 v0, v1;
      if constexpr (PL) {
        planes8(reinterpret_cast<const bf16raw*>(h), hlo, nn * ldh + c8 * 8, v0, v1);
      } else {
        v0 = *reinterpret_cast<const float4*>(h + nn * ldh + c8 * 8);
        v1 = *reinterpret_cast<const float4*>(h + nn * ldh + c8 * 8 + 4);
      }
      acc[0] += wgt * v0.x; acc[1] += wgt * v0.y; acc[2] += wgt * v0.z; acc[3] += wgt * v0.w;
      acc[4] += wgt * v1.x; acc[5] += wgt * v1.y; acc[6] += wgt * v1.z; acc[7] += wgt * v1.w;
      if (MEAN) {
        const float one = n < end ? 1.f : 0.f;
        macc[0] += one * v0.x; macc[1] += one * v0.y; macc[2] += one * v0.z; macc[3] += one * v0.w;
        macc[4] += one * v1.x; macc[5] += one * v1.y; macc[6] += one * v1.z; macc[7] += one * v1.w;
      }
    }
    float* dst = red + (int64_t)rl * D + c8 * 8;
    *reinterpret_cast<float4*>(dst) = make_float4(acc[0], acc[1], acc[2], acc[3]);
    *reinterpret_cast<float4*>(dst + 4) = make_float4(acc[4], acc[5], acc[6], acc[7]);
  }
  __syncthreads();
  if (tid < (int)(D >> 2)) {
    float4 t = make_float4(0.f, 0.f, 0.f, 0.f);
    for (int q = 0; q < rpp; ++q) {
      const float4 v = *reinterpret_cast<const float4*>(red + (int64_t)q * D + tid * 4);
      t.x += v.x; t.y += v.y; t.z += v.z; t.w += v.w;
    }
    *reinterpret_cast<float4*>(prow + tid * 4) = t;
  }
  if (MEAN) {
    __syncthreads();
    if (rl < rpp) {
      float* dst = red + (int64_t)rl * D + c8 * 8;
      *reinterpret_cast<float4*>(dst) = make_float4(macc[0], macc[1], macc[2], macc[3]);
      *reinterpret_cast<float4*>(dst + 4) = make_float4(macc[4], macc[5], macc[6], macc[7]);
    }
    __syncthreads();
    if (tid < (int)(D >> 2)) {
      float4 t = make_float4(0.f, 0.f, 0.f, 0.f);
      for (int q = 0; q < rpp; ++q) {
        const float4 v = *reinterpret_cast<const float4*>(red + (int64_t)q * D + tid * 4);
        t.x += v.x; t.y += v.y; t.z += v.z; t.w += v.w;
      }
      *reinterpret_cast<float4*>(mrow + tid * 4) = t;
    }
  }
}

#define POOL_ONLINE_MAX_NBLK 2048
__global__ __launch_bounds__(256) void pool_merge_online_kernel(const float* __restrict__ partial, const float* __restrict__ pstats, int nblk,
                                                                int64_t D, const float* __restrict__ s, int64_t N,
                                                                const int64_t* __restrict__ seg_ptr, float* __restrict__ pooled,
                                                                float* __restrict__ A, float* __restrict__ stats,
                                                                const float* __restrict__ mpartial = nullptr, float* __restrict__ mean = nullptr) {
  __shared__ float sc[POOL_ONLINE_MAX_NBLK];
  __shared__ float red[16][17];
  __shared__ float wred[8];
  const int tid = threadIdx.x, lane = tid & 63, w = tid >> 6;
  const int b = blockIdx.y;
  const float* pst = pstats + (int64_t)b * nblk * 2;
  float mx = -INFINITY;
  for (int j = tid; j < nblk; j += 256) mx = fmaxf(mx, pst[2 * j]);
  mx = wave_max(mx);
  if (lane == 0) wred[w] = mx;
  __syncthreads();
  const float M = fmaxf(fmaxf(wred[0], wred[1]), fmaxf(wred[2], wred[3]));
  float ls = 0.f;
  for (int j = tid; j < nblk; j += 256) {
    const float mj = pst[2 * j];
    const float c = mj == -INFINITY ? 0.f : hw_exp(mj - M);
    sc[j] = c;
    ls += pst[2 * j + 1] * c;
  }
  ls = wave_sum(ls);
  if (lane == 0) wred[4 + w] = ls;
  __syncthreads();
  const float inv = hw_rcp((wred[4] + wred[5]) + (wred[6] + wred[7]));
  if (blockIdx.x == 0 && tid == 0 && stats) { stats[2 * b] = M; stats[2 * b + 1] = inv; }
  const int cl = tid & 15, rl = tid >> 4;
  const int64_t c = (int64_t)blockIdx.x * 16 + cl;
  const float* pp = partial + (int64_t)b * nblk * D;
  float sv[4] = {0.f, 0.f, 0.f, 0.f};
  if (c < D) {
    int j = rl;
    for (; j + 48 < nblk; j += 64) {
#pragma unroll
      for (int u = 0; u < 4; ++u) sv[u] += pp[(int64_t)(j + 16 * u) * D + c] * sc[j + 16 * u];
    }
    for (; j < nblk; j += 16) sv[0] += pp[(int64_t)j * D + c] * sc[j];
  }
  red[rl][cl] = (sv[0] + sv[1]) + (sv[2] + sv[3]);
  __syncthreads();
  if (rl == 0 && c < D) {
    float t = 0.f;
#pragma unroll
    for (int r = 0; r < 16; ++r) t += red[r][cl];
    pooled[(int64_t)b * D + c] = t * inv;
  }
  int64_t beg, end;
  seg_range(seg_ptr, b, N, beg, end);
  if (mean) {
    __syncthreads();
    const float* mp = mpartial + (int64_t)b * nblk * D;
    float mv[4] = {0.f, 0.f, 0.f, 0.f};
    if (c < D) {
      int j = rl;
      for (; j + 48 < nblk; j += 64) {
#pragma unroll
        for (int u = 0; u < 4; ++u) mv[u] += mp[(int64_t)(j + 16 * u) * D + c];
      }
      for (; j < nblk; j += 16) mv[0] += mp[(int64_t)j * D + c];
    }
    red[rl][cl] = (mv[0] + mv[1]) + (mv[2] + mv[3]);
    __syncthreads();
    if (rl == 0 && c < D) {
      float t = 0.f;
#pragma unroll
      for (int r = 0; r < 16; ++r) t += red[r][cl];
      mean[(int64_t)b * D + c] = end > beg ? t / (float)(end - beg) : 0.f;
    }
  }
  for (int64_t n = beg + (int64_t)blockIdx.x * 256 + tid; n < end; n += (int64_t)gridDim.x * 256) A[n] = hw_exp(s[n] - M) * inv;
}

static inline int64_t pool_nblk(int64_t max_len) { const int r = rows_per_block(max_len); return (max_len + r - 1) / r; }

extern "C" size_t advmil_softmax_pool_workspace_bytes(int64_t max_len, int64_t D, int nseg) {
  if (nseg < 1) nseg = 1;
  const int64_t a = 4 * (int64_t)nseg + (int64_t)nseg * pool_nblk(max_len) * (D + 2);
  const int64_t b = 4 + (int64_t)nseg * ((max_len + 3) / 4);
  return (size_t)(a > b ? a : b) * sizeof(float);
}

static int softmax_pool_fwd_impl(const float* s, const float* h, int64_t ldh, int64_t N, int64_t D, int nseg, const int64_t* seg_ptr,
                                 int64_t max_len, float* A, float* pooled, float* mean, void* ws, size_t ws_bytes, hipStream_t stream,
                                 const bf16raw* hlo = nullptr);

extern "C" int advmil_softmax_pool_fwd(const float* s, const float* h, int64_t ldh, int64_t N, int64_t D, int nseg,
                                       const int64_t* seg_ptr, int64_t max_len, float* A, float* pooled, void* ws,
                                       size_t ws_bytes, advmil_stream_t stream_) {
  return softmax_pool_fwd_impl(s, h, ldh, N, D, nseg, seg_ptr, max_len, A, pooled, nullptr, ws, ws_bytes, (hipStream_t)stream_);
}

extern "C" int advmil_softmax_pool_fwd_planes(const float* s, const void* h_hi, const void* h_lo, int64_t ldh, int64_t N, int64_t D, int nseg,
                                              const int64_t* seg_ptr, int64_t max_len, float* A, float* pooled, void* ws,
                                              size_t ws_bytes, advmil_stream_t stream_) {
  if (!h_hi || !h_lo) return ADVMIL_EINVAL;
  return softmax_pool_fwd_impl(s, (const float*)h_hi, ldh, N, D, nseg, seg_ptr, max_len, A, pooled, nullptr, ws, ws_bytes, (hipStream_t)stream_,
                               (const bf16raw*)h_lo);
}

static inline size_t pool_mean_offset_bytes(int64_t max_len, int64_t D, int nseg) {
  return (advmil_softmax_pool_workspace_bytes(max_len, D, nseg) + 15) / 16 * 16;
}

extern "C" size_t advmil_softmax_pool_mean_workspace_bytes(int64_t max_len, int64_t D, int nseg) {
  if (nseg < 1) nseg = 1;
  return pool_mean_offset_bytes(max_len, D, nseg) + (size_t)((int64_t)nseg * pool_nblk(max_len) * D) * sizeof(float);
}

extern "C" int advmil_softmax_pool_mean_fwd(const float* s, const float* h, int64_t ldh, int64_t N, int64_t D, int nseg,
                                            const int64_t* seg_ptr, int64_t max_len, float* A, float* pooled, float* mean, void* ws,
                                            size_t ws_bytes, advmil_stream_t stream_) {
  if (!mean) return ADVMIL_EINVAL;
  return softmax_pool_fwd_impl(s, h, ldh, N, D, nseg, seg_ptr, max_len, A, pooled, mean, ws, ws_bytes, (hipStream_t)stream_);
}

static int softmax_pool_fwd_impl(const float* s, const float* h, int64_t ldh, int64_t N, int64_t D, int nseg, const int64_t* seg_ptr,
                                 int64_t max_len, float* A, float* pooled, float* mean, void* ws, size_t ws_bytes, hipStream_t stream,
                                 const bf16raw* hlo) {
  if (!s || !h || !A || !pooled || !ws || N <= 0 || D <= 0 || (D & 3) || D > 1024 || (ldh & 3)) return ADVMIL_EINVAL;
  if (ldh < D || ((uintptr_t)h & 15)) return ADVMIL_EINVAL;
  if (hlo && (((uintptr_t)hlo & 15) || (D & 7) || (ldh & 7) || D < 16 || mean)) return ADVMIL_EINVAL;
  if (!seg_ptr && nseg > 1) return ADVMIL_EINVAL;
  if (!seg_ptr) { nseg = 1; max_len = N; }
  if (nseg < 1 || max_len <= 0 || max_len > N) return ADVMIL_EINVAL;
  if (ws_bytes < (mean ? advmil_softmax_pool_mean_workspace_bytes(max_len, D, nseg) : advmil_softmax_pool_workspace_bytes(max_len, D, nseg)))
    return ADVMIL_EWORKSPACE;
  float* stats = (float*)ws;
  float* partial = stats + 4 * nseg;
  const int nblk = (int)pool_nblk(max_len);
  if ((D & 7) == 0 && D >= 16 && nblk <= POOL_ONLINE_MAX_NBLK) {
    float* pstats = partial + (int64_t)nseg * nblk * D;
    if (mean) {
      float* mpartial = (float*)ws + pool_mean_offset_bytes(max_len, D, nseg) / sizeof(float);
      hipLaunchKernelGGL((pool_partial8_online_kernel<true, false>), dim3(nblk, nseg), dim3(256), 0, stream, s, h, ldh, N, D, seg_ptr, partial, pstats,
                         rows_per_block(max_len), mpartial, (const bf16raw*)nullptr);
      ADVMIL_LAUNCH_CHECK();
      hipLaunchKernelGGL(pool_merge_online_kernel, dim3((unsigned)((D + 15) / 16), nseg), dim3(256), 0, stream, partial, pstats, nblk, D, s,
                         N, seg_ptr, pooled, A, stats, (const float*)mpartial, mean);
      ADVMIL_LAUNCH_CHECK();
      return ADVMIL_OK;
    }
    if (hlo)
      hipLaunchKernelGGL((pool_partial8_online_kernel<false, true>), dim3(nblk, nseg), dim3(256), 0, stream, s, h, ldh, N, D, seg_ptr, partial,
                         pstats, rows_per_block(max_len), (float*)nullptr, hlo);
    else
      hipLaunchKernelGGL((pool_partial8_online_kernel<false, false>), dim3(nblk, nseg), dim3(256), 0, stream, s, h, ldh, N, D, seg_ptr, partial,
                         pstats, rows_per_block(max_len), (float*)nullptr, (const bf16raw*)nullptr);
    ADVMIL_LAUNCH_CHECK();
    hipLaunchKernelGGL(pool_merge_online_kernel, dim3((unsigned)((D + 15) / 16), nseg), dim3(256), 0, stream, partial, pstats, nblk, D, s,
                       N, seg_ptr, pooled, A, stats, (const float*)nullptr, (float*)nullptr);
    ADVMIL_LAUNCH_CHECK();
    return ADVMIL_OK;
  }
  if (mean || hlo) return ADVMIL_EINVAL;
  hipLaunchKernelGGL(softmax_stats_kernel, dim3(nseg), dim3(1024), 0, stream, s, N, seg_ptr, stats);
  ADVMIL_LAUNCH_CHECK();
  if ((D & 7) == 0 && D >= 16)
    hipLaunchKernelGGL(pool_partial8_kernel, dim3(nblk, nseg), dim3(256), 0, stream, s, h, ldh, N, D, seg_ptr, stats, A, partial,
                       rows_per_block(max_len));
  else
    hipLaunchKernelGGL(pool_partial_kernel, dim3(nblk, nseg), dim3(256), 0, stream, s, h, ldh, N, D, seg_ptr, stats, A, partial,
                       rows_per_block(max_len));
  ADVMIL_LAUNCH_CHECK();
  hipLaunchKernelGGL(colsum_merge_kernel, dim3((unsigned)((D + 15) / 16), nseg), dim3(256), 0, stream, partial, nblk, D, D, pooled,
                     0, (int64_t)nblk * D, D);
  ADVMIL_LAUNCH_CHECK();
  return ADVMIL_OK;
}

#define PBD_ROWS 4
template <bool PL>
__global__ __launch_bounds__(256) void pool_bwd_dot_kernel(const float* __restrict__ dp, const float* __restrict__ dA,
                                                           const float* __restrict__ A, const float* __restrict__ h,
                                                           int64_t ldh, int64_t N, int64_t D,
                                                           const int64_t* __restrict__ seg_ptr, float* __restrict__ t,
                                                           float* __restrict__ partial, const bf16raw* __restrict__ hlo) {
  __shared__ float red[4];
  const int lane = threadIdx.x & 63, w = threadIdx.x >> 6;
  const int b = blockIdx.y;
  int64_t beg, end;
  seg_range(seg_ptr, b, N, beg, end);
  const int64_t n0 = beg + ((int64_t)blockIdx.x * 4 + w) * PBD_ROWS;
  const float* dpb = dp + (int64_t)b * D;
  float acc[PBD_ROWS];
#pragma unroll
  for (int rr = 0; rr < PBD_ROWS; ++rr) acc[rr] = 0.f;
  if (PL && n0 < end) {
    const int nch = (int)(D >> 3), items = PBD_ROWS * nch;
    for (int g = lane; g < items; g += 64) {
      const int rr = g / nch, ch = g - rr * nch;
      if (n0 + rr < end) {
        float4 v0, v1;
        planes8(reinterpret_cast<const bf16raw*>(h), hlo, (n0 + rr) * ldh + ch * 8, v0, v1);
        const float4 a0 = *reinterpret_cast<const float4*>(dpb + ch * 8), a1 = *reinterpret_cast<const float4*>(dpb + ch * 8 + 4);
        const float d = a0.x * v0.x + a0.y * v0.y + a0.z * v0.z + a0.w * v0.w + a1.x * v1.x + a1.y * v1.y + a1.z * v1.z + a1.w * v1.w;
#pragma unroll
        for (int k = 0; k < PBD_ROWS; ++k) acc[k] += (k == rr) ? d : 0.f;
      }
    }
  } else if (n0 < end) {
    if ((D & 3) == 0 && (ldh & 3) == 0) {
      const float4* d4 = reinterpret_cast<const float4*>(dpb);
      for (int64_t q = lane; q < (D >> 2); q += 64) {
        const float4 a = d4[q];
        float4 v[PBD_ROWS];
#pragma unroll
        for (int rr = 0; rr < PBD_ROWS; ++rr)
          v[rr] = (n0 + rr < end) ? reinterpret_cast<const float4*>(h + (n0 + rr) * ldh)[q] : make_float4(0.f, 0.f, 0.f, 0.f);
#pragma unroll
        for (int rr = 0; rr < PBD_ROWS; ++rr) acc[rr] += a.x * v[rr].x + a.y * v[rr].y + a.z * v[rr].z + a.w * v[rr].w;
      }
    } else {
      for (int64_t j = lane; j < D; j += 64) {
        const float a = dpb[j];
#pragma unroll
        for (int rr = 0; rr < PBD_ROWS; ++rr)
          if (n0 + rr < end) acc[rr] += a * h[(n0 + rr) * ldh + j];
      }
    }
  }
  float contrib = 0.f;
#pragma unroll
  for (int rr = 0; rr < PBD_ROWS; ++rr) {
    const int64_t n = n0 + rr;
    float s = wave_sum(acc[rr]);
    if (n < end) {
      if (dA) s += dA[n];
      if (lane == 0) t[n] = s;
      contrib += A[n] * s;
    }
// ... 1050 lines not shown
```

advmil_amd/ops.py:

```python
import ctypes
import os

import torch

from . import _lib
from ._lib import Epilogue

ACT_NONE, ACT_RELU, ACT_TANH, ACT_SIGMOID = 0, 1, 2, 3
FUSED_WGRAD = True
KERNEL_PROFILE = None
STAMPS = None


class Stamps:

    def __init__(self, device, cap=2048):
        self.buf = torch.zeros(cap, dtype=torch.int64, device=device)
        self.tags = []
        self.khz = int(_lib.lib().advmil_clock_rate_khz()) or 100000

    def mark(self, tag):
        i = len(self.tags)
        if i >= self.buf.numel():
            return
# ... 238 lines not shown
        _lib.check(_lib.lib().advmil_gemm_f32_plan_tn_planes(M, N, K, ctypes.byref(t), ctypes.byref(sp)), "gemm_plan_tn_planes")
        _PLAN_CACHE[key] = (t.value, sp.value)
    return _PLAN_CACHE[key]


TN_GROUP = os.environ.get("ADVMIL_TN_GROUP", "1") != "0"


def gemm_tn_group(calls):
    n = len(calls)
    arr = (_lib.GemmTnCall * n)()
    for c, (A, B, out, acc) in zip(arr, calls):
        K, M = A.shape
        c.M, c.N, c.K = M, B.shape[1], K
        c.A, c.lda, c.B, c.ldb = A.data_ptr(), A.stride(0), B.data_ptr(), B.stride(0)
        c.C, c.ldc, c.accumulate = out.data_ptr(), out.stride(0), 1 if acc else 0
    L = _lib.lib()
    wsb = L.advmil_gemm_tn_group_workspace_bytes(arr, n)
    ws = _ws(wsb, calls[0][0].device) if wsb else None
    _lib.check(L.advmil_gemm_tn_group(arr, n, _p(ws), wsb, _stream()), "gemm_tn_group")


def auto_splits(M, N, K):
    return gemm_plan(M, N, K)[1]


class Planes:
    __slots__ = ("hi", "lo", "fp32_stale")

    def __init__(self, hi, lo):
        self.hi, self.lo = hi, lo
        self.fp32_stale = False

    @property
    def single(self):
        return self.lo is None

    def ptrs(self):
        return self.hi.data_ptr() | (0 if self.lo is None else self.lo.data_ptr())

    def lo_ptr(self):
        return 0 if self.lo is None else self.lo.data_ptr()

    SKEW = 32768

    @staticmethod
    def alloc(shape, device):
        n = 1
        for v in shape:
            n *= int(v)
        pad = (-n) % 8
        buf = torch.empty(2 * n + pad + Planes.SKEW, dtype=torch.bfloat16, device=device)
        return Planes(buf[:n].view(*shape), buf[n + pad + Planes.SKEW:n + pad + Planes.SKEW + n].view(*shape))

    @staticmethod
    def empty_like(x):
        if x.is_contiguous():
            return Planes.alloc(tuple(x.shape), x.device)
        return Planes(torch.empty_strided(x.shape, x.stride(), dtype=torch.bfloat16, device=x.device),
                      torch.empty_strided(x.shape, x.stride(), dtype=torch.bfloat16, device=x.device))

    def view_rows(self, r0, r1):
        return Planes(self.hi[r0:r1], None if self.lo is None else self.lo[r0:r1])


USE_PLANES = os.environ.get("ADVMIL_PLANES", "1") != "0"
DH_NT_FUSED = os.environ.get("ADVMIL_DH_NT_FUSED", "1") != "0"
ACT_BWD_IN_DH = os.environ.get("ADVMIL_ACT_BWD_IN_DH", "1") != "0"
DG_PLANES_ONLY = os.environ.get("ADVMIL_DG_PLANES_ONLY", "1") != "0"
DW_PLANES = os.environ.get("ADVMIL_DW_PLANES", "1") != "0"
MEMO_PLANES = os.environ.get("ADVMIL_MEMO_PLANES", "1") != "0"
H_PLANES_ONLY = os.environ.get("ADVMIL_H_PLANES_ONLY", "1") != "0"
FUSED_GATE_TRAIN = os.environ.get("ADVMIL_FUSED_GATE_TRAIN", "1") != "0"
SLAB_PLANES_ANY = os.environ.get("ADVMIL_SLAB_PLANES_ANY", "1") != "0"
GENERIC_PLANES = os.environ.get("ADVMIL_GENERIC_PLANES", "1") != "0"
SMALL_LINEAR = os.environ.get("ADVMIL_SMALL_LINEAR", "1") != "0"
SMALL_LINEAR_ROWS = int(os.environ.get("ADVMIL_SMALL_LINEAR_ROWS", "8"))


def slab_takes_planes(rows, C):
    return bool(rows >= 4096 and USE_PLANES and get_gemm_mode() == "bf16x3" and (SLAB_PLANES_ANY or gemm_plan_planes(rows, 128, C)))


def planes_transposed(pl):
    R, C = pl.hi.shape
    out = Planes.alloc((C, R), pl.hi.device)
    d = (pl.lo.data_ptr() - pl.hi.data_ptr()) // 2
    do = (out.lo.data_ptr() - out.hi.data_ptr()) // 2
    if (pl.hi.untyped_storage().data_ptr() == pl.lo.untyped_storage().data_ptr() and d > 0 and pl.hi.stride() == pl.lo.stride()
            and pl.hi.stride(1) == 1):
        src = pl.hi.as_strided((2, C, R), (d, 1, pl.hi.stride(0)), pl.hi.storage_offset())
        dst = out.hi.as_strided((2, C, R), (do, R, 1), out.hi.storage_offset())
        dst.copy_(src)
    else:
        out.hi.copy_(pl.hi.t())
        out.lo.copy_(pl.lo.t())
    return out


def _token(M, N, device):
    t = torch.empty(M, N, dtype=torch.float32, device=device)
    if POISON_TOKENS:
        t.fill_(float("nan"))
    return t


def planes_of(x):
    if is_bf16_slab(x):
        return Planes(x, None)
    return getattr(x, "_advmil_planes", None) if USE_PLANES else None


def weight_planes(W):
    if not USE_PLANES:
        return None
    ent = getattr(W, "_advmil_planes", None)
    if ent is None:
        return None
    owner, ver, pl = ent
    if ver != W._version:
        owner.refresh_planes()
        owner, ver, pl = W._advmil_planes
    return pl


def split_planes(x, out=None):
    _chk(x, "x")
    if out is None:
        out = Planes.empty_like(x)
    _lib.check(_lib.lib().advmil_split_planes(_p(x), x.numel(), _p(out.hi), _p(out.lo), _stream()), "split_planes")
    return out


def pre_a_tile_ok(tile, a_kc, b_kc, b_planes=False):
    return tile in (22, 12, 11) or (tile == 43 and not b_kc and not b_planes) or (tile in (34, 24) and not a_kc and not b_kc and b_planes)


def gemm(A, B, a_kc, b_kc, M, N, K, out=None, ldc=None, bias=None, act0=0, act1=None, act_split=None, drop_p=0.0,
         seed=None, stream_id=0, rowv=None, colv=None, rowseg=None, maskref=None, mask_scale=1.0, accumulate=False,
         alpha=1.0, splits=None, tile=0, a_planes=None, b_planes=None, c_planes=None, c_planes_only=False, gate_wc=None, rng_row=None,
         colsum=None, maskbits=None, gate_bits=None, c_rows_pair32=False):
    planes_only_a = A is None
    if planes_only_a:
        if a_planes is None or get_gemm_mode() != "bf16x3":
            raise ValueError("gemm(A=None) needs a_planes in bf16x3 mode")
        A = a_planes.hi
    else:
        if is_bf16_slab(A):
            a_planes = a_planes or Planes(A, None)
            planes_only_a = True
        else:
            _chk(A, "A")
            if a_planes is not None and a_planes.fp32_stale:
                planes_only_a = True
    b_single = False
    planes_only_b = B is None
    if planes_only_b:
        if b_planes is None or b_planes.single or get_gemm_mode() != "bf16x3" or not (82 <= tile <= 87 or 91 <= tile <= 93):
            raise ValueError("gemm(B=None) needs two-plane b_planes, bf16x3 mode and a plane-fed tile")
        B = b_planes.hi
    elif is_bf16_slab(B):
        b_planes = b_planes or Planes(B, None)
        b_single = True
    else:
        _chk(B, "B")
    b_only = b_single or (b_planes is not None and b_planes.fp32_stale)
    if (planes_only_a or b_only) and get_gemm_mode() != "bf16x3":
        raise ValueError("bf16 slabs need gemm_mode 'bf16x3' (ops.as_f32 gives their fp32 image)")
    if (tile == 0 and a_planes is not None and b_planes is not None and (splits is None or splits == 1) and not b_planes.single
            and not ((a_planes.ptrs() | b_planes.ptrs()) & 15)
            and a_planes.hi.stride(0) % 8 == 0 and b_planes.hi.stride(0) % 8 == 0):
        ptile = gemm_plan_planes(M, N, K, a_kc, b_kc)
        if ptile:
            tile, splits = ptile, 1
            if ptile == 87 and (gate_wc is not None or rowv is not None or maskref is not None or maskbits is not None or colsum is not None
                                or accumulate or (drop_p > 0.0 and seed is not None)):
                tile = 82
            if gate_wc is not None and gate_bits is not None:
                tile = 85 if (N % 256 == 0 and (M // 256) * (N // 256) >= 256) else 86
            elif gate_wc is not None and N % 256 == 0 and (M // 256) * (N // 256) >= 384:
                tile = 84
            elif (gate_wc is None and N % 256 == 0 and (M // 256) * (N // 256) >= 384 and rowv is None and maskref is None
                  and not accumulate and (drop_p <= 0.0 or seed is None)):
                tile = 85
    if (tile == 0 and splits is None and a_planes is not None and b_planes is not None and not a_kc and not b_kc and gate_wc is None
            and not a_planes.single and not ((a_planes.ptrs() | b_planes.ptrs()) & 15)
            and a_planes.hi.stride(0) % 8 == 0 and b_planes.hi.stride(0) % 8 == 0):
        ttile, tsplits = gemm_plan_tn_planes(M, N, K)
        if ttile:
            tile, splits = ttile, tsplits
    if gate_wc is not None:
        tile, _ = gemm_plan(M, N, K, a_kc, b_kc) if tile == 0 else (tile, 1)
        npart = _lib.lib().advmil_gemm_f32_gate_blocks(tile, N)
        gate_out = torch.empty(M, npart, dtype=torch.float32, device=A.device)
        splits, ldc = 1, N
        if gate_bits is None:
            out = None
        else:
            if not (85 <= tile <= 86):
                raise ValueError("gemm(gate_bits=...) needs the plane-fed plain tiles (operands as planes, slab-sized M)")
            out = torch.empty(M, N, dtype=torch.float32, device=A.device)
    elif c_planes_only:
        if c_planes is None or out is not None or accumulate:
            raise ValueError("gemm(c_planes_only=True) needs c_planes, no `out`, no accumulate")
        splits, ldc = 1, N
    elif out is None:
        out = torch.empty(M, N, dtype=torch.float32, device=A.device)
        ldc = N
    elif ldc is None:
        ldc = out.stride(0)
    lda = A.stride(0)
    ldb = B.stride(0)
    e = Epilogue()
    if bias is not None:
        e.bias = bias.data_ptr()
    e.act0 = act0
    e.act1 = act0 if act1 is None else act1
    e.act_split = (1 << 30) if act_split is None else act_split
    use_seed = seed is not None and drop_p > 0.0
    if use_seed:
        e.drop_p = float(drop_p)
        e.seed = seed.data_ptr()
        e.stream_id = stream_id
        if rng_row is not None:
            e.rng_row = rng_row.data_ptr()
    elif drop_p:
        e.drop_p = float(drop_p)
    if rowv is not None:
        e.rowv = rowv.data_ptr()
    if colv is not None:
        e.colv = colv.data_ptr()
    if rowseg is not None:
        e.rowseg = rowseg.data_ptr()
    if maskref is not None:
        e.maskref = maskref.data_ptr()
        e.ldmask = maskref.stride(0)
    e.mask_scale = float(mask_scale)
    if accumulate:
        e.accumulate = 1
    e.alpha = float(alpha)
    if a_planes is not None:
        e.a_hi, e.a_lo = a_planes.hi.data_ptr(), a_planes.lo_ptr()
    if b_planes is not None:
        e.b_hi, e.b_lo = b_planes.hi.data_ptr(), b_planes.lo_ptr()
    if c_planes is not None:
        e.c_hi, e.c_lo = c_planes.hi.data_ptr(), c_planes.lo.data_ptr()
    if gate_wc is not None:
        e.gate_wc, e.gate_out, e.gate_np = gate_wc.data_ptr(), gate_out.data_ptr(), npart
        if gate_bits is not None:
            e.gate_bits_a, e.gate_bits_b, e.ldgbits = gate_bits[0].data_ptr(), gate_bits[1].data_ptr(), gate_bits[0].stride(0)
    if c_rows_pair32:
        e.c_rows_pair32 = 1
    if colsum is not None:
        e.colsum = colsum.data_ptr()
    if maskbits is not None:
        e.maskbits, e.ldbits = maskbits.data_ptr(), maskbits.stride(0)
        e.mask_scale = float(mask_scale)
    if splits is None:
        ptile, splits = gemm_plan(M, N, K, a_kc, b_kc)
        if tile == 0:
            tile = ptile
    if accumulate and splits > 1 and _DEFER_KEEP is not None and out is not None and not _is_arena(out):
        splits = 1
    if (b_only and not (91 <= tile <= 93) and not (82 <= tile <= 87 and not b_single) and tile not in (22, 12, 11)
            and not (tile in (34, 24) and not a_kc and not b_kc)):
        tile = 22
    if planes_only_a and a_planes.single and not (82 <= tile <= 87) and tile not in (22, 12, 11):
        tile = 22
    if planes_only_a and a_planes.fp32_stale and not (82 <= tile <= 87) and not (91 <= tile <= 93) and tile not in (22, 12, 11) \
            and not pre_a_tile_ok(tile, a_kc, b_kc, b_planes is not None):
        tile = 22
    if planes_only_a and not (82 <= tile <= 87) and not (91 <= tile <= 93) and not pre_a_tile_ok(tile if tile else gemm_plan(M, N, K, a_kc, b_kc)[0], a_kc, b_kc,
                                                                     b_planes is not None):
        raise ValueError(f"gemm(A=None): tile {tile} has no pre-split-A instantiation for this layout")
    L = _lib.lib()
    wsb = L.advmil_gemm_f32_workspace_bytes(M, N, splits)
    ws = _ws(wsb, A.device) if wsb else None
    prof = KERNEL_PROFILE
    name = None
    if prof is not None or STAMPS is not None:
        name = ("gemm_nt_planes_kernel<%d>" % (tile - 80)) if 82 <= tile <= 84 else "gemm_nt_planes_kernel<4,plain>" if tile == 85 else "gemm_nt_planes_kernel<2,plain>" if tile == 86 else \
            "gemm_nt_planes_kernel<2,plain,512>" if tile == 87 else \
            ("gemm_tn_planes_kernel<%d>" % tile) if 91 <= tile <= 93 else \
            "gemm_f32_kernel<%d,%d,%d,%d>" % (bool(a_kc), bool(b_kc), tile // 10, tile % 10)
    if prof is not None:
        e0 = torch.cuda.Event(enable_timing=True)
        e0.record()
    if STAMPS is not None and M * N * K >= (1 << 30):
        _stamp("b", name, (M, N, K, splits), 2.0 * M * N * K)
    _lib.check(L.advmil_gemm_f32_tiled(1 if a_kc else 0, 1 if b_kc else 0, M, N, K, _p(A), lda, _p(B), ldb, _p(out), ldc,
                                       ctypes.byref(e), splits, tile, _p(ws), wsb, _stream()), f"gemm_f32[{M}x{N}x{K}]")
    if STAMPS is not None and M * N * K >= (1 << 30):
        _stamp("e", name, (M, N, K, splits), 2.0 * M * N * K)
    if prof is not None:
        e1 = torch.cuda.Event(enable_timing=True)
        e1.record()
        prof.append((name, (M, N, K, splits), 2.0 * M * N * K, e0, e1))
    if gate_wc is not None and gate_bits is not None:
        return out, gate_out
    return gate_out if gate_wc is not None else out


ATTN_QKV_PLANES = os.environ.get("ADVMIL_ATTN_QKV_PLANES", "1") != "0"
TWO_LAYERS_MIN_TILES = int(os.environ.get("ADVMIL_TWO_LAYERS_MIN_TILES", "256"))
TWO_LAYERS_NARROW = os.environ.get("ADVMIL_TWO_LAYERS_NARROW", "1") != "0"


def gemm_two_layers_tile(M, N1, N2, K):
    if not (get_gemm_mode() == "bf16x3" and USE_PLANES and M >= 4096 and M % 256 == 0 and K % 32 == 0 and K >= 64 and N1 % 32 == 0
            and M * K * 2 < (1 << 32)):
        return 0
    if (N1 + N2) % 256 == 0 and (M // 256) * ((N1 + N2) // 256) >= TWO_LAYERS_MIN_TILES:
        return 85
    if TWO_LAYERS_NARROW and (N1 + N2) % 128 == 0 and N1 % 128 == 0 and (M // 256) * ((N1 + N2) // 128) >= TWO_LAYERS_MIN_TILES:
        return 86
    return 0


def gemm_two_layers_ok(M, N1, N2, K):
    return gemm_two_layers_tile(M, N1, N2, K) != 0


def gemm_two_layers(x, xpl, W1, w1pl, b1, act1, W2, w2pl, b2, act2, emit_planes1=False, y1_planes_only=False):
    M, K = x.shape
    N1, N2 = W1.shape[0], W2.shape[0]

    def pair(pl, N):
        hi, lo = pl.hi.reshape(N, K), pl.lo.reshape(N, K)
        d = (lo.data_ptr() - hi.data_ptr()) // 2
        if hi.untyped_storage().data_ptr() != lo.untyped_storage().data_ptr() or d <= 0 or not hi.is_contiguous() or not lo.is_contiguous():
            return None
        return hi.as_strided((2, N, K), (d, K, 1), hi.storage_offset())
    v1, v2 = pair(w1pl, N1), pair(w2pl, N2)
    if v1 is not None and v2 is not None:
        stk = torch.cat((v1, v2), dim=1)
        wcat = Planes(stk[0], stk[1])
    else:
        wcat = Planes(torch.cat((w1pl.hi.reshape(N1, K), w2pl.hi.reshape(N2, K)), dim=0), torch.cat((w1pl.lo.reshape(N1, K), w2pl.lo.reshape(N2, K)), dim=0))
    dev = x.device
    y1 = _token(M, N1, dev) if y1_planes_only else torch.empty(M, N1, dtype=torch.float32, device=dev)
    y2 = torch.empty(M, N2, dtype=torch.float32, device=dev)
    cpl = None
    if emit_planes1 or y1_planes_only:
        cpl = Planes.alloc((M, N1), dev)
    e = Epilogue()
    e.bias = None if b1 is None else b1.data_ptr()
    e.bias2 = None if b2 is None else b2.data_ptr()
    e.act0, e.act1, e.act_split = act1, act2, N1
    e.alpha = 1.0
    e.a_hi, e.a_lo = xpl.hi.data_ptr(), xpl.lo_ptr()
    e.b_hi, e.b_lo = wcat.hi.data_ptr(), wcat.lo.data_ptr()
    if cpl is not None:
        e.c_hi, e.c_lo = cpl.hi.data_ptr(), cpl.lo.data_ptr()
    e.c2, e.ldc2, e.n_split = y2.data_ptr(), N2, N1
    prof = KERNEL_PROFILE
    if prof is not None:
        e0 = torch.cuda.Event(enable_timing=True)
        e0.record()
    _stamp("b", f"gemm_nt_planes_kernel<4,two layers,{N1}>", (M, N1 + N2, K, 1), 2.0 * M * (N1 + N2) * K)
    _lib.check(_lib.lib().advmil_gemm_f32_tiled(1, 1, M, N1 + N2, K, _p(x), x.stride(0), _p(W1), K, None if y1_planes_only else _p(y1), N1,
                                                ctypes.byref(e), 1, gemm_two_layers_tile(M, N1, N2, K), None, 0, _stream()),
               f"gemm_two_layers[{M}x({N1}+{N2})x{K}]")
    if cpl is not None:
        cpl.fp32_stale = bool(y1_planes_only)
    _stamp("e", f"gemm_nt_planes_kernel<4,two layers,{N1}>", (M, N1 + N2, K, 1), 2.0 * M * (N1 + N2) * K)
    if prof is not None:
        e1 = torch.cuda.Event(enable_timing=True)
        e1.record()
        prof.append((f"gemm_nt_planes_kernel<4,two layers,{N1}>", (M, N1 + N2, K, 1), 2.0 * M * (N1 + N2) * K, e0, e1))
    return y1, y2, cpl


def gate_score(ab, wc, bc, N, D, p=0.0, seed=None, stream_a=0, stream_b=0, rng_row=None):
    s = torch.empty(N, dtype=torch.float32, device=ab.device)
    sd = seed if p > 0.0 else None
    _lib.check(_lib.lib().advmil_gate_score_fwd(_p(ab), _p(wc), _p(bc), p, _p(sd), stream_a, stream_b, N, D, _p(s),
                                                _p(rng_row if sd is not None else None), _stream()), "gate_score_fwd")
    return s


class Segments:

    def __init__(self, lens, device):
        import numpy as np
        self.lens = [int(v) for v in lens]
        self.nseg = len(self.lens)
        self.total = sum(self.lens)
        self.max_len = max(self.lens)
        self.device = torch.device(device)
        offs = [0]
        for v in self.lens:
            offs.append(offs[-1] + v)
        self.offsets = offs
        nb = (8 * (self.nseg + 1) + 15) // 16 * 16
        host = torch.empty(nb + 4 * self.total, dtype=torch.uint8, pin_memory=self.device.type == "cuda")
        hv = host.numpy()
        hv[:8 * (self.nseg + 1)].view(np.int64)[:] = offs
        hv[nb:].view(np.int32)[:] = np.repeat(np.arange(self.nseg, dtype=np.int32), self.lens)
        buf = host.to(self.device, non_blocking=True)
        self._host, self._buf = host, buf
        self.ptr = buf[:8 * (self.nseg + 1)].view(torch.int64)
        self.rowseg = buf[nb:].view(torch.int32)
        self._div = {}

    @property
    def rowseg_long(self):
        if "long" not in self._div:
            self._div["long"] = self.rowseg.to(torch.long)
        return self._div["long"]

    def div(self, k):
        if k not in self._div:
            assert all(v % k == 0 for v in self.lens)
            self._div[k] = Segments([v // k for v in self.lens], self.device)
        return self._div[k]

    def twice(self):
        if "x2" not in self._div:
            self._div["x2"] = Segments(self.lens + self.lens, self.device)
        return self._div["x2"]

    def uniform(self, rows):
        key = ("u", rows)
        if key not in self._div:
            self._div[key] = Segments([rows] * self.nseg, self.device)
        return self._div[key]


def softmax_pool(s, h, N, D, seg=None, hpl=None):
    L = _lib.lib()
    nseg = 1 if seg is None else seg.nseg
    mlen = N if seg is None else seg.max_len
    A = torch.empty(N, dtype=torch.float32, device=h.device)
    pooled = torch.empty(nseg, D, dtype=torch.float32, device=h.device)
    wsb = L.advmil_softmax_pool_workspace_bytes(mlen, D, nseg)
    ws = _ws(wsb, h.device)
    big = STAMPS is not None and N * D >= (1 << 24)
    if big:
        _stamp("b", "softmax_pool_fwd", (N, D, nseg), 4.0 * N * D + 12.0 * N)
    if hpl is not None:
        _lib.check(L.advmil_softmax_pool_fwd_planes(_p(s), _p(hpl.hi), _p(hpl.lo), hpl.hi.stride(0), N, D, nseg,
                                                    _p(None if seg is None else seg.ptr), mlen, _p(A), _p(pooled), _p(ws), wsb, _stream()),
                   "softmax_pool_fwd_planes")
    else:
        _lib.check(L.advmil_softmax_pool_fwd(_p(s), _p(h), h.stride(0), N, D, nseg, _p(None if seg is None else seg.ptr), mlen, _p(A),
                                             _p(pooled), _p(ws), wsb, _stream()), "softmax_pool_fwd")
    if big:
        _stamp("e", "softmax_pool_fwd", (N, D, nseg), 4.0 * N * D + 12.0 * N)
    return A, pooled


def softmax_pool_mean(s, h, N, D, seg=None):
    L = _lib.lib()
    nseg = 1 if seg is None else seg.nseg
    mlen = N if seg is None else seg.max_len
    A = torch.empty(N, dtype=torch.float32, device=h.device)
    pooled = torch.empty(nseg, D, dtype=torch.float32, device=h.device)
    mean = torch.empty(nseg, D, dtype=torch.float32, device=h.device)
    wsb = L.advmil_softmax_pool_mean_workspace_bytes(mlen, D, nseg)
    ws = _ws(wsb, h.device)
    _lib.check(L.advmil_softmax_pool_mean_fwd(_p(s), _p(h), h.stride(0), N, D, nseg, _p(None if seg is None else seg.ptr), mlen, _p(A),
                                              _p(pooled), _p(mean), _p(ws), wsb, _stream()), "softmax_pool_mean_fwd")
    return A, pooled, mean


def softmax_pool_bwd(dpooled, dA, A, h, N, D, seg=None, hpl=None):
    L = _lib.lib()
    nseg = 1 if seg is None else seg.nseg
    mlen = N if seg is None else seg.max_len
    ds = torch.empty(N, dtype=torch.float32, device=h.device)
    wsb = L.advmil_softmax_pool_workspace_bytes(mlen, D, nseg)
    ws = _ws(wsb, h.device)
    if hpl is not None:
        _lib.check(L.advmil_softmax_pool_bwd_planes(_p(dpooled), _p(dA), _p(A), _p(hpl.hi), _p(hpl.lo), hpl.hi.stride(0), N, D, nseg,
                                                    _p(None if seg is None else seg.ptr), mlen, _p(ds), _p(ws), wsb, _stream()),
                   "softmax_pool_bwd_planes")
    else:
        _lib.check(L.advmil_softmax_pool_bwd(_p(dpooled), _p(dA), _p(A), _p(h), h.stride(0), N, D, nseg,
                                             _p(None if seg is None else seg.ptr), mlen, _p(ds), _p(ws), wsb, _stream()),
                   "softmax_pool_bwd")
    return ds


def dropout_planes(pl, M, N, p, seed, sid, rng_row=None, gate=None):
    out = Planes.alloc((M, N), pl.hi.device)
    out.fp32_stale = True
    bits = torch.empty(M, N // 32, dtype=torch.int32, device=pl.hi.device)
    gb = None
    if gate is not None:
        gb = (torch.empty(M, N // 32, dtype=torch.int32, device=pl.hi.device), torch.empty(M, N // 32, dtype=torch.int32, device=pl.hi.device))
    _lib.check(_lib.lib().advmil_dropout_planes(_p(pl.hi), _p(pl.lo), M, N, float(p), _p(seed), sid, _p(rng_row), _p(out.hi), _p(out.lo),
                                                _p(bits), 0.0 if gate is None else float(gate[0]), 0 if gate is None else int(gate[1]),
                                                0 if gate is None else int(gate[2]), _p(None if gb is None else gb[0]),
                                                _p(None if gb is None else gb[1]), _stream()), "dropout_planes")
    return (out, bits, gb) if gate is not None else (out, bits)


def planes_f32(pl):
    return pl.hi.float().add_(pl.lo)


def gate_bwd(ab, ds, wc, N, D, p=0.0, seed=None, stream_a=0, stream_b=0, dwc=None, dbc=None, dbias=None, rng_row=None, planes=None,
             planes_only=False, pair32=False):
    L = _lib.lib()
    dev = ab.device
    acc = dwc is not None
    dG = None if (planes_only and planes is not None) else torch.empty(N, 2 * D, dtype=torch.float32, device=dev)
    if not acc:
        dwc = torch.empty(D, dtype=torch.float32, device=dev)
        dbc = torch.empty(1, dtype=torch.float32, device=dev)
        dbias = torch.empty(2 * D, dtype=torch.float32, device=dev)
    wsb = L.advmil_gate_bwd_workspace_bytes(N, D)
    ws = _ws(wsb, dev)
    sd = seed if p > 0.0 else None
    _lib.check(L.advmil_gate_bwd(_p(ab), _p(ds), _p(wc), p, _p(sd), stream_a, stream_b, N, D, _p(dG), _p(dwc), _p(dbc),
                                 _p(dbias), 1 if acc else 0, _p(rng_row if sd is not None else None),
                                 _p(None if planes is None else planes.hi), _p(None if planes is None else planes.lo), 1 if pair32 else 0,
                                 _p(ws), wsb, _stream()), "gate_bwd")
    return dG, dwc, dbc, dbias


def act_dropout_bwd(dy, y, act, M, N, p=0.0, seed=None, stream_id=0, want_bias=True, db_out=None, rng_row=None, planes=None,
                    planes_only=False, bits=None):
    L = _lib.lib()
    dpre = None if (planes_only and planes is not None) else torch.empty(M, N, dtype=torch.float32, device=dy.device)
    acc = db_out is not None
    db = db_out if acc else (torch.empty(N, dtype=torch.float32, device=dy.device) if want_bias else None)
    need = acc or want_bias
    wsb = L.advmil_colsum_workspace_bytes(M, N) if need else 0
    ws = _ws(wsb, dy.device) if need else None
    sd = seed if p > 0.0 else None
    _lib.check(L.advmil_act_dropout_bwd(_p(dy), _p(y), act, p, _p(sd), stream_id, M, N, _p(dpre), _p(db), 1 if acc else 0,
                                        _p(rng_row if sd is not None else None), _p(None if planes is None else planes.hi),
                                        _p(None if planes is None else planes.lo), _p(bits), _p(ws), wsb, _stream()), "act_dropout_bwd")
    return dpre, db


def colsum(x, M, N, out=None):
    L = _lib.lib()
    acc = out is not None
    if not acc:
        out = torch.empty(N, dtype=torch.float32, device=x.device)
    wsb = L.advmil_colsum_workspace_bytes(M, N)
# ... 45 lines not shown
               "adam_step")


class OptimCall:

    def __init__(self, kind, p, grad, s1, s2, wd, step, planes=None, m_sched=None, slow=None, la_state=None):
        for nm, t in (("p", p), ("grad", grad), ("s1", s1), ("s2", s2), ("wd", wd), ("slow", slow)):
            if t is not None and (t.dtype != torch.float32 or t.numel() != p.numel() or not t.is_contiguous()):
                raise ValueError(f"optim_step: {nm} must be a contiguous fp32 arena of p's size")
        if m_sched is not None and (m_sched.dtype != torch.float64 or m_sched.numel() < 2):
            raise ValueError("optim_step: m_sched holds two float64")
        if la_state is not None and (la_state.dtype != torch.int32 or la_state.numel() < 2):
            raise ValueError("optim_step: la_state holds two int32")
        self.keep = (p, grad, s1, s2, wd, step, planes, m_sched, slow, la_state)
        self.blocks, self.wd = adam_blocks(p.numel()), _p(wd)
        a = self.a = _lib.Optim()
        a.kind, a.lookahead, a.n = _lib.OPT_KINDS[kind], 0 if slow is None else 1, p.numel()
        a.p, a.grad, a.s1, a.s2, a.wd, a.slow = _p(p), _p(grad), _p(s1), _p(s2), self.wd, _p(slow)
        a.step, a.la_state, a.m_sched = _p(step), _p(la_state), _p(m_sched)
        a.p_hi, a.p_lo = _p(None if planes is None else planes.hi), _p(None if planes is None else planes.lo)
        self.ref = ctypes.byref(a)

    def __call__(self, lr, beta1=0.9, beta2=0.999, eps=1e-8, grad_scale=1.0, l1_coef=0.0, tick=True, abs_partial=None, clear_grad=False,
                 schedule_decay=4e-3, la_alpha=0.5, la_k=6, use_wd=True):
        if abs_partial is not None and (abs_partial.numel() < self.blocks or abs_partial.dtype != torch.float32):
            raise ValueError("optim_step: abs_partial needs adam_blocks(n) fp32 entries")
        a = self.a
        a.lr, a.beta1, a.beta2, a.eps, a.schedule_decay = lr, beta1, beta2, eps, schedule_decay
        a.grad_scale, a.l1_coef, a.la_alpha, a.la_k, a.tick = grad_scale, l1_coef, la_alpha, la_k, 1 if tick else 0
        a.wd = self.wd if use_wd else None
        a.abs_partial, a.clear_grad = _p(abs_partial), 1 if clear_grad else 0
        _lib.check(_lib.lib().advmil_optim_step(self.ref, _stream()), "optim_step")


def optim_step(kind, p, grad, s1, s2, wd, step, lr, beta1=0.9, beta2=0.999, eps=1e-8, grad_scale=1.0, l1_coef=0.0, planes=None, tick=True,
               abs_partial=None, clear_grad=False, schedule_decay=4e-3, m_sched=None, slow=None, la_state=None, la_alpha=0.5, la_k=6):
    OptimCall(kind, p, grad, s1, s2, wd, step, planes=planes, m_sched=m_sched, slow=slow, la_state=la_state)(
        lr, beta1, beta2, eps, grad_scale, l1_coef, tick=tick, abs_partial=abs_partial, clear_grad=clear_grad,
        schedule_decay=schedule_decay, la_alpha=la_alpha, la_k=la_k)


def step_seed_tick(step, seed, inc=1, step2=None):
    _lib.check(_lib.lib().advmil_step_seed_tick(_p(step), _p(step2), _p(seed), int(inc), _stream()), "step_seed_tick")


def abs_sum(p):
    L = _lib.lib()
    out = torch.empty(1, dtype=torch.float32, device=p.device)
    wsb = L.advmil_abs_sum_workspace_bytes(p.numel())
    ws = _ws(wsb, p.device)
    _lib.check(L.advmil_abs_sum(_p(p), p.numel(), _p(out), _p(ws), wsb, _stream()), "abs_sum")
    return out


def _arena_grad(p):
    g = getattr(p, "_arena_grad", None) if p is not None else None
    if g is not None and FUSED_WGRAD and p.requires_grad:
        o = getattr(p, "_arena_owner", None)
        if o is not None and o._grad_clean and not torch.cuda.is_current_stream_capturing():
            o._grad_clean = False
        return g
    return None


ARENA_STORAGES = set()


def _is_arena(t):
    return t.untyped_storage().data_ptr() in ARENA_STORAGES


def _adjacent(a, b, itemsize=4):
    return (a is not None and b is not None and a.is_contiguous() and b.is_contiguous()
            and b.data_ptr() == a.data_ptr() + a.numel() * itemsize
            and a.untyped_storage().data_ptr() == b.untyped_storage().data_ptr())


def _stack2(a, b, rows, cols):
    if _adjacent(a, b):
        shape = (2 * rows, cols) if cols else (2 * rows,)
        stride = (cols, 1) if cols else (1,)
        return a.detach().as_strided(shape, stride, a.storage_offset()), True
    return torch.cat([a.detach(), b.detach()], dim=0).contiguous(), False


class DropoutFn(torch.autograd.Function):

    @staticmethod
    def forward(ctx, x, p, seed, sid, rr=None):
        x = x.contiguous()
        y = torch.empty_like(x)
        w = x.shape[-1] if rr is not None else 0
        _lib.check(_lib.lib().advmil_dropout_apply(_p(x), _p(y), x.numel(), p, _p(seed), sid, _p(rr), w, _stream()), "dropout_apply")
        ctx.cfg = (p, seed, sid, rr, w)
        return y

    @staticmethod
    def backward(ctx, dy):
        p, seed, sid, rr, w = ctx.cfg
        dy = dy.contiguous()
        dx = torch.empty_like(dy)
        _lib.check(_lib.lib().advmil_dropout_apply(_p(dy), _p(dx), dy.numel(), p, _p(seed), sid, _p(rr), w, _stream()), "dropout_apply")
        return dx, None, None, None, None


def dropout(x, p, rng, tag=""):
    if p <= 0.0 or x.numel() == 0:
        return x
    _chk(x, "x")
    sid = rng.site(tag, tuple(x.shape), p)
    return DropoutFn.apply(x, float(p), rng.seed, sid, rng.row_map(x.numel() // x.shape[-1], tag))


class LinearActFn(torch.autograd.Function):
    last_planes = None
    last_wants_dy_planes = False
    last_act_fusable = None
    last_maskbits = None
    gate_request = None
    last_gate = None

    @staticmethod
    def forward(ctx, x, W, b, act, p, seed, sid, y0=None, rr=None, xpl=None, wpl=None, emit=False):
        if not is_bf16_slab(x):
            _chk(x, "x")
        _chk(W, "weight")
        x = x.contiguous()
        W2 = W.detach().reshape(W.shape[0], -1)
        M, K = x.shape
        N = W2.shape[0]
        cpl = None
        ctx.small = False
        y0pl = getattr(y0, "_advmil_planes", None) if (y0 is not None and getattr(y0, "_advmil_planes_only", False)) else None
        if (SMALL_LINEAR and y0 is None and M <= min(32, SMALL_LINEAR_ROWS) and K % 4 == 0 and N <= 1024 and xpl is None and not emit and x.dtype == torch.float32
                and (b is None or b.dtype == torch.float32)):
            y = torch.empty(M, N, dtype=torch.float32, device=x.device)
            use = seed is not None and p > 0.0
            _lib.check(_lib.lib().advmil_small_linear_fwd(_p(x), K, _p(W2), _p(b), M, N, K, act, float(p) if use else 0.0,
                                                          _p(seed if use else None), sid, _p(rr if use else None), _p(y), _stream()),
                       f"small_linear_fwd[{M}x{N}x{K}]")
            ctx.small = True
        elif y0 is None:
            if emit and get_gemm_mode() == "bf16x3":
                cpl = Planes.alloc((M, N), x.device)
            if emit == "only" and cpl is not None:
                gemm(x, W2, True, True, M, N, K, bias=b, act0=act, drop_p=p, seed=seed, stream_id=sid, rng_row=rr,
                     a_planes=xpl, b_planes=wpl, c_planes=cpl, c_planes_only=True)
                cpl.fp32_stale = True
                y = _token(M, N, x.device)
            else:
                y = gemm(x, W2, True, True, M, N, K, bias=b, act0=act, drop_p=p, seed=seed, stream_id=sid, rng_row=rr,
                         a_planes=xpl, b_planes=wpl, c_planes=cpl, splits=1 if cpl is not None else None)
        elif p > 0.0 and y0pl is not None:
            greq, LinearActFn.gate_request = LinearActFn.gate_request, None
            gate = None
            if greq is not None and N % 32 == 0:
                pg, tag_a, tag_b, grng = greq
                if grng.row_map(M, tag_a) is rr and grng.row_map(M, tag_b) is rr:
                    gate = (pg, grng.site(tag_a, (M, N), pg), grng.site(tag_b, (M, N), pg))
            if gate is not None:
                cpl, mbits, gb = dropout_planes(y0pl, M, N, p, seed, sid, rr, gate=gate)
                LinearActFn.last_gate = (gate[1], gate[2], gb[0], gb[1], gate[0], rr)
            else:
                cpl, mbits = dropout_planes(y0pl, M, N, p, seed, sid, rr)
            y = _token(M, N, x.device)
            LinearActFn.last_maskbits = mbits if act == ACT_RELU else None
# ... 170 lines not shown
    if PREFILL and p <= 0.0:
        pf = PREFILL.pop((x2.data_ptr(), tuple(x2.shape), W.data_ptr(), W._version, _ACT[act]), None)
        if pf is not None:
            y0, pre_planes = pf
    if y0 is None and memo is not None and memo.mode == "replay":
        y0 = memo.store.pop(key, None)
        if y0 is not None:
            y0.record_stream(torch.cuda.current_stream())
    xpl = wpl = None
    if y0 is not None and p <= 0.0 and emit_planes:
        emit_planes = False
    big = x2.shape[0] >= 4096 and get_gemm_mode() == "bf16x3"
    stale = bool(getattr(x2, "_advmil_fp32_stale", False))
    if stale and (planes_of(x2) is None or get_gemm_mode() != "bf16x3"):
        raise RuntimeError("advmil_amd: a step slab staged as operand planes only reached a layer without its planes")
    if (y0 is None and big and (gemm_plan_planes(x2.shape[0], W.shape[0], x2.shape[1]) or (GENERIC_PLANES and planes_of(x2) is not None))) or stale:
        xpl, wpl = planes_of(x2), weight_planes(W)
        if wpl is not None:
            wpl = Planes(wpl.hi.reshape(W.shape[0], -1), wpl.lo.reshape(W.shape[0], -1))
    if is_bf16_slab(x2) and get_gemm_mode() != "bf16x3":
        x2 = as_f32(x2)
    emit = bool(emit_planes) and big and bool(gemm_plan_planes(x2.shape[0], 2 * W.shape[0], W.shape[0]))
    if emit_planes == "only":
        emit = "only" if (big and (act == "none" or not torch.is_grad_enabled()) and p <= 0.0 and y0 is None and W.shape[0] % 8 == 0
                          and ATTN_QKV_PLANES and (act == "none" or emit)) else (emit if act != "none" else False)
    LinearActFn.gate_request = ((float(gate_sites[0]), gate_sites[1], gate_sites[2], rng) if (gate_sites is not None and FUSED_GATE_TRAIN
                                and p > 0.0 and gate_sites[0] > 0.0 and torch.is_grad_enabled()) else None)
    LinearActFn.last_gate = None
    y = LinearActFn.apply(x2, W, b, _ACT[act], float(p), seed, sid, y0, rr, xpl, wpl, emit)
    LinearActFn.gate_request = None
    cpl, LinearActFn.last_planes = LinearActFn.last_planes, None
    if pre_planes is not None and cpl is None:
        cpl = pre_planes
    if memo is not None and memo.mode == "record" and p <= 0.0 and not torch.is_grad_enabled():
        memo.store[key] = y
        memo.derived[y.data_ptr()] = y
    out = y if len(lead) == 1 else y.reshape(*lead, y.shape[-1])
    if cpl is not None:
        out._advmil_planes = cpl
        if emit == "only" or cpl.fp32_stale:
            out._advmil_planes_only = True
    if LinearActFn.last_wants_dy_planes:
        out._advmil_wants_dy_planes = True
    LinearActFn.last_wants_dy_planes = False
    if LinearActFn.last_act_fusable is not None and out.requires_grad:
        out._advmil_act_fusable = LinearActFn.last_act_fusable + (LinearActFn.last_maskbits,)
    LinearActFn.last_act_fusable = None
    LinearActFn.last_maskbits = None
    if LinearActFn.last_gate is not None:
        out._advmil_gate = LinearActFn.last_gate
        LinearActFn.last_gate = None
    return out


def linear_act_any(x, W, b, act="none", p=0.0, rng=None, tag=""):
    K, N = W.shape[1], W.shape[0]
    if x.dim() != 2 or not x.is_cuda:
        raise RuntimeError("advmil_amd: linear layers run on 2-D HIP tensors only (no CPU / eager fallback)")
    if K % 4 == 0 and N % 4 == 0:
        return linear_act(x, W, b, act, p, rng, tag)
    pk, pn = (-K) % 4, (-N) % 4
    xp = torch.nn.functional.pad(x, (0, pk)) if pk else x
    Wp = torch.nn.functional.pad(W, (0, pk, 0, pn)) if (pk or pn) else W
    bp = None if b is None else (torch.nn.functional.pad(b, (0, pn)) if pn else b)
    y = linear_act(xp.contiguous(), Wp.contiguous(), bp, act)[:, :N]
    if p > 0.0:
        y = dropout(y.contiguous(), p, rng or default_rng(x.device), tag)
    return y


class GatedAttnPoolFn(torch.autograd.Function):

    @staticmethod
    def forward(ctx, h, Wa, ba, Wb, bb, wc, bc, p, seed, sa, sb, seg, nograd=False, rr=None, hpl=None, act_fuse=None, gate=None):
        _chk(h, "h")
        h = h.contiguous()
        N, D = h.shape
        ctx.act_fuse = act_fuse
        ctx.pair32 = False
        wcv = wc.detach().reshape(-1)
        stale = hpl is not None and hpl.fp32_stale
        ppl = hpl if stale else None
        if FUSED_GATE_SCORE and p <= 0.0 and N >= 4096 and nograd:
            Wi, bi, wipl = gate_interleave(Wa.detach(), ba.detach(), Wb.detach(), bb.detach(), D, planes=hpl is not None)
            s = gate_partial_sum(gemm(h, Wi, True, True, N, 2 * D, D, bias=bi, gate_wc=wcv, a_planes=hpl, b_planes=wipl), bc.detach())
            A, pooled = softmax_pool(s, h, N, D, seg, ppl)
            ctx.mark_non_differentiable(s)
            return pooled, A, s
        gs = [_arena_grad(t) for t in (Wa, ba, Wb, bb, wc, bc)]
        arena_ok = all(g is not None for g in gs) and _adjacent(gs[0], gs[2]) and _adjacent(gs[1], gs[3])
        if (gate is not None and FUSED_GATE_TRAIN and p > 0.0 and hpl is not None and arena_ok and N % 256 == 0 and D % 64 == 0
                and get_gemm_mode() == "bf16x3" and gemm_plan_planes(N, 2 * D, D) and gemm_plan_tn_planes(2 * D, D, N)[1] > 1
                and gemm_plan_planes(N, D, 2 * D)):
            Wp, bp, wppl = gate_interleave(Wa.detach(), ba.detach(), Wb.detach(), bb.detach(), D, planes=True, pair32=True)
            ab, part = gemm(h, Wp, True, True, N, 2 * D, D, bias=bp, gate_wc=wcv, drop_p=p, a_planes=hpl, b_planes=wppl, gate_bits=gate)
            s = gate_partial_sum(part, bc.detach())
            A, pooled = softmax_pool(s, h, N, D, seg, ppl)
            ctx.save_for_backward(h, Wp, ab, A, wcv)
            ctx.hpl, ctx.wabpl, ctx.pair32 = hpl, wppl, True
            ctx.cfg = (p, seed, sa, sb, N, D, wc.shape, seg, rr)
            ctx.arena = (gs[0].as_strided((2 * D, D), (D, 1), gs[0].storage_offset()),
                         gs[1].as_strided((2 * D,), (1,), gs[1].storage_offset()), gs[4].view(-1), gs[5])
            ctx.mark_non_differentiable(s)
            ctx.set_materialize_grads(False)
            return pooled, A, s
        Wab, _ = _stack2(Wa, Wb, D, D)
        bab, _ = _stack2(ba, bb, D, 0)
        wabpl = None
        if hpl is not None:
            pa_, pb_ = weight_planes(Wa), weight_planes(Wb)
            if pa_ is not None and pb_ is not None and _adjacent(pa_.hi, pb_.hi, 2) and _adjacent(pa_.lo, pb_.lo, 2):
                wabpl = Planes(pa_.hi.as_strided((2 * D, D), (D, 1), pa_.hi.storage_offset()),
                               pa_.lo.as_strided((2 * D, D), (D, 1), pa_.lo.storage_offset()))
            if wabpl is None and stale:
                wabpl = split_planes(Wab.detach().contiguous())
        ab = gemm(h, Wab, True, True, N, 2 * D, D, bias=bab, act0=ACT_TANH, act1=ACT_SIGMOID, act_split=D,
                  a_planes=hpl if wabpl is not None else None, b_planes=wabpl)
        s = gate_score(ab, wcv, bc, N, D, p, seed, sa, sb, rr)
        A, pooled = softmax_pool(s, h, N, D, seg, ppl)
        ctx.save_for_backward(h, Wab, ab, A, wcv)
        ctx.hpl = hpl
        ctx.wabpl = wabpl
        ctx.cfg = (p, seed, sa, sb, N, D, wc.shape, seg, rr)
        ctx.arena = None
        if arena_ok:
            ctx.arena = (gs[0].as_strided((2 * D, D), (D, 1), gs[0].storage_offset()),
                         gs[1].as_strided((2 * D,), (1,), gs[1].storage_offset()), gs[4].view(-1), gs[5])
        ctx.mark_non_differentiable(s)
        ctx.set_materialize_grads(False)
        return pooled, A, s

    @staticmethod
    def backward(ctx, dpooled, dA, _ds_unused):
        h, Wab, ab, A, wcv = ctx.saved_tensors
        p, seed, sa, sb, N, D, wcshape, seg, rr = ctx.cfg
        pair32 = bool(getattr(ctx, "pair32", False))
        nseg = 1 if seg is None else seg.nseg
        dpooled = (torch.zeros(nseg, D, dtype=torch.float32, device=h.device) if dpooled is None
                   else dpooled.contiguous().reshape(nseg, D))
        dA_ = None if dA is None else dA.contiguous()
        stale = ctx.hpl is not None and ctx.hpl.fp32_stale
        ds = softmax_pool_bwd(dpooled, dA_, A, h, N, D, seg, ctx.hpl if stale else None)
        need_h = ctx.needs_input_grad[0]
        gpl = None
        dh_tile = gemm_plan_planes(N, D, 2 * D) if (need_h and USE_PLANES and get_gemm_mode() == "bf16x3") else 0
        if dh_tile == 87:
            dh_tile = 82
        dh_nt = bool(dh_tile and DH_NT_FUSED and ctx.act_fuse is not None and ctx.act_fuse[2] is not None
                     and getattr(ctx, "wabpl", None) is not None and int(_lib.lib().advmil_gemm_f32_colsum_rows(dh_tile, N, D)) > 0)
        only = (DG_PLANES_ONLY and USE_PLANES and get_gemm_mode() == "bf16x3" and N >= 4096 and (2 * D) % 8 == 0
                and pre_a_tile_ok(gemm_plan(2 * D, D, N, False, False)[0], False, False)
                and (not need_h or pre_a_tile_ok(gemm_plan(N, D, 2 * D, True, False)[0], True, False)))
        if only and gpl is None:
            gpl = Planes.alloc((N, 2 * D), h.device)
        if ctx.arena is not None:
            gWab, gbab, gwc, gbc = ctx.arena
            dG, _, _, _ = gate_bwd(ab, ds, wcv, N, D, p, seed, sa, sb, dwc=gwc, dbc=gbc, dbias=gbab, rng_row=rr, planes=gpl, planes_only=only,
                                   pair32=pair32)
        else:
            dG, dwc, dbc, dbias = gate_bwd(ab, ds, wcv, N, D, p, seed, sa, sb, rng_row=rr, planes=gpl, planes_only=only)
        dh = None
        fuse = ctx.act_fuse if (need_h and only and ctx.act_fuse is not None) else None
        if fuse is not None and stale and fuse[2] is None:
            fuse = None
        wtpl = None
        if fuse is not None and dh_nt:
            nrow = int(_lib.lib().advmil_gemm_f32_colsum_rows(dh_tile, N, D))
            tile = dh_tile
            wtpl = planes_transposed(ctx.wabpl)
        elif fuse is not None:
            tile = gemm_plan(N, D, 2 * D, True, False)[0]
            nrow = int(_lib.lib().advmil_gemm_f32_colsum_rows(tile, N, D)) if pre_a_tile_ok(tile, True, False) else 0
            if nrow <= 0:
                fuse = None
        if fuse is not None:
            p1, gb1, mbits = fuse
            dpl = Planes.alloc((N, D), h.device)
            cws = _ws(nrow * D * 4, h.device) if gb1 is not None else None
            if wtpl is not None:
                gemm(None, None, True, True, N, D, 2 * D, rowv=A, colv=dpooled, rowseg=None if seg is None else seg.rowseg, a_planes=gpl,
                     b_planes=wtpl, maskbits=mbits, mask_scale=1.0 / (1.0 - p1) if p1 > 0.0 else 1.0, c_planes=dpl, c_planes_only=True,
                     colsum=cws, tile=tile)
            else:
                gemm(None, Wab, True, False, N, D, 2 * D, rowv=A, colv=dpooled, rowseg=None if seg is None else seg.rowseg, a_planes=gpl,
                     maskref=h if mbits is None else None, maskbits=mbits, mask_scale=1.0 / (1.0 - p1) if p1 > 0.0 else 1.0, c_planes=dpl,
                     c_planes_only=True, colsum=cws, tile=tile)
            if gb1 is not None:
                _lib.check(_lib.lib().advmil_merge_partials(_p(cws), nrow, D, D, _p(gb1), 1, _stream()), "merge_partials")
            dh = torch.empty(N, D, dtype=torch.float32, device=h.device)
            DY_PLANES.put(dh, dpl, (N, D), "dpre")
        elif need_h:
            if only:
                dh = gemm(None, Wab, True, False, N, D, 2 * D, rowv=A, colv=dpooled, rowseg=None if seg is None else seg.rowseg, a_planes=gpl)
            else:
                dh = gemm(dG, Wab, True, False, N, D, 2 * D, rowv=A, colv=dpooled, rowseg=None if seg is None else seg.rowseg)
        nones = (None,) * 10
        apl = gpl if only else None
        if ctx.arena is not None:
            bpl = ctx.hpl if (stale or (apl is not None and gemm_plan_tn_planes(2 * D, D, N)[0])) else None
            if pair32 and (apl is None or bpl is None):
                raise RuntimeError("advmil_amd: the pair-block gate backward needs dG and h as operand planes")
            gemm(dG, h, False, False, 2 * D, D, N, out=gWab, ldc=D, accumulate=True, a_planes=apl, b_planes=bpl, c_rows_pair32=pair32)
            return (dh, None, None, None, None, None, None) + nones
        bpl = ctx.hpl if (stale or (apl is not None and gemm_plan_tn_planes(2 * D, D, N)[0])) else None
        dWab = gemm(dG, h, False, False, 2 * D, D, N, a_planes=apl, b_planes=bpl)
        return (dh, dWab[:D], dbias[:D], dWab[D:], dbias[D:], dwc.reshape(wcshape), dbc) + nones


def gated_attn_pool(h, Wa, ba, Wb, bb, wc, bc, p=0.0, rng=None, tag="", seg=None):
    sa = sb = 0
    seed = rr = None
    gate = None
    if p > 0.0:
        rng = rng or default_rng(h.device)
        pre = getattr(h, "_advmil_gate", None)
        if pre is not None and pre[4] == float(p):
            sa, sb, gate = pre[0], pre[1], (pre[2], pre[3])
            seed, rr = rng.seed, pre[5]
        else:
            sa = rng.site(tag + "att_a", tuple(h.shape), p)
            sb = rng.site(tag + "att_b", tuple(h.shape), p)
            seed, rr = rng.seed, rng.row_map(h.shape[0], tag + "att_a")
    nograd = not torch.is_grad_enabled() or not any(t.requires_grad for t in (h, Wa, ba, Wb, bb, wc, bc))
    hpl = planes_of(h) if (h.shape[0] >= 4096 and h.is_contiguous() and get_gemm_mode() == "bf16x3"
                           and gemm_plan_planes(h.shape[0], 2 * h.shape[1], h.shape[1])) else None
    if getattr(h, "_advmil_planes_only", False):
        hpl = planes_of(h)
        if hpl is None or not hpl.fp32_stale:
            raise RuntimeError("advmil_amd: a planes-only activation reached the gated-attention pool without its planes")
    pooled, A, s = GatedAttnPoolFn.apply(h, Wa, ba, Wb, bb, wc, bc, float(p), seed, sa, sb, seg, nograd, rr, hpl,
                                         getattr(h, "_advmil_act_fusable", None), gate)
    return (pooled[0] if seg is None else pooled), A, s


class LNReLUMean16Fn(torch.autograd.Function):

    @staticmethod
    def forward(ctx, y, gamma, beta, eps, ycol=None, dy_planes=False, dup=1, memo=None):
        _chk(y, "y")
        y = y.contiguous()
        N, d = y.shape
        ctx.dup = dup
        if memo is not None:
            emb, mean, rstd = memo
            epl = None
        else:
            epl = None
            emb, mean, rstd = ln_relu_mean16_fwd(y, gamma, beta, N, d, eps, planes=epl, dup=dup)
        LNReLUMean16Fn.last_stats = (mean, rstd)
        LNReLUMean16Fn.last_planes = epl
        ctx.save_for_backward(y, gamma.detach(), beta.detach(), mean, rstd)
        gg, gb = _arena_grad(gamma), _arena_grad(beta)
        ctx.arena = (gg, gb) if (gg is not None and gb is not None) else None
        ctx.ycol = ycol
        ctx.dy_planes = bool(dy_planes)
        return emb

# ... 1481 lines not shown
```

include/advmil_hip.h:

```cpp
#ifndef ADVMIL_HIP_H
#define ADVMIL_HIP_H
#include <stddef.h>
#include <stdint.h>

#ifdef __cplusplus
extern "C" {
#endif

typedef void* advmil_stream_t;

enum { ADVMIL_ACT_NONE = 0, ADVMIL_ACT_RELU = 1, ADVMIL_ACT_TANH = 2, ADVMIL_ACT_SIGMOID = 3 };

int advmil_version(void);

typedef struct {
  const float* bias;
  int act0, act1, act_split;
  float drop_p;
  const uint64_t* seed;
  uint64_t stream_id;
  const float* rowv;
  const float* colv;
  const int32_t* rowseg;
  const float* maskref;
  int ldmask;
  float mask_scale;
  int accumulate;
  float alpha;
  const void* a_hi;
  const void* a_lo;
  const void* b_hi;
  const void* b_lo;
  void* c_hi;
  void* c_lo;
  const float* gate_wc;
  float* gate_out;
  int gate_np;
  const int64_t* rng_row;
  float* c2;
  int64_t ldc2;
  int64_t n_split;
  const float* bias2;
  float* colsum;
  const uint32_t* maskbits;
  int64_t ldbits;
  const uint32_t* gate_bits_a;
  const uint32_t* gate_bits_b;
  int64_t ldgbits;
  int c_rows_pair32;
} advmil_epilogue_t;

size_t advmil_gemm_f32_workspace_bytes(int64_t M, int64_t N, int splits);
int advmil_gemm_f32(int a_kc, int b_kc, int64_t M, int64_t N, int64_t K, const float* A, int64_t lda,
                    const float* B, int64_t ldb, float* C, int64_t ldc, const advmil_epilogue_t* epi,
                    int splits, void* ws, size_t ws_bytes, advmil_stream_t stream);
int advmil_split_planes(const float* src, int64_t n, void* hi, void* lo, advmil_stream_t stream);
int advmil_gate_interleave(const float* Wa, const float* Wb, const float* ba, const float* bb, int D, float* Wi, void* Wi_hi, void* Wi_lo,
                           float* bi, int pair32, advmil_stream_t stream);
int advmil_gate_partial_sum(const float* partial, int np, const float* bc, int64_t N, float* s, advmil_stream_t stream);
int advmil_gemm_f32_gate_blocks(int tile, int64_t N);
int64_t advmil_gemm_f32_colsum_rows(int tile, int64_t M, int64_t N);
int advmil_merge_partials(const float* partial, int nblk, int64_t stride, int64_t ncols, float* out, int accumulate, advmil_stream_t stream);
int advmil_set_gemm_mode(int mode);
int advmil_get_gemm_mode(void);
int advmil_gemm_f32_plan(int64_t M, int64_t N, int64_t K, int* tile, int* splits);
int advmil_gemm_f32_plan_layout(int a_kc, int b_kc, int64_t M, int64_t N, int64_t K, int* tile, int* splits);
int advmil_gemm_f32_plan_planes(int a_kc, int b_kc, int64_t M, int64_t N, int64_t K, int* tile);
int advmil_gemm_f32_plan_tn_planes(int64_t M, int64_t N, int64_t K, int* tile, int* splits);
int advmil_gemm_f32_tiled(int a_kc, int b_kc, int64_t M, int64_t N, int64_t K, const float* A, int64_t lda,
                          const float* B, int64_t ldb, float* C, int64_t ldc, const advmil_epilogue_t* epi,
                          int splits, int tile, void* ws, size_t ws_bytes, advmil_stream_t stream);

int advmil_mha_fwd(const void* qkv_hi, const void* qkv_lo, int64_t Ltot, int nhead, int head_dim, int nseg, const int64_t* ptr,
                   int64_t max_len, float drop_p, const uint64_t* seed, uint64_t stream_id, const int64_t* rng_rowoff, float* out,
                   float* lse, advmil_stream_t stream);
int advmil_mha_fwd_lse(const void* qkv_hi, const void* qkv_lo, int64_t Ltot, int nhead, int head_dim, int nseg, const int64_t* ptr,
                       int64_t max_len, float drop_p, const uint64_t* seed, uint64_t stream_id, const int64_t* rng_rowoff, float* out,
                       const float* lse, advmil_stream_t stream);
size_t advmil_mha_bwd_workspace_bytes(int64_t Ltot, int nhead, int head_dim);
int advmil_mha_bwd(const void* qkv_hi, const void* qkv_lo, const float* out, const float* dout, const float* lse, int64_t Ltot,
                   int nhead, int head_dim, int nseg, const int64_t* ptr, int64_t max_len, float drop_p, const uint64_t* seed,
                   uint64_t stream_id, const int64_t* rng_rowoff, float* dqkv, void* ws, size_t ws_bytes, advmil_stream_t stream);
size_t advmil_mha_bwd1_workspace_bytes(int64_t Ltot, int nhead, int head_dim, int64_t max_len);
int advmil_mha_bwd1(const void* qkv_hi, const void* qkv_lo, const float* out, const float* dout, const float* lse, int64_t Ltot,
                    int nhead, int head_dim, int nseg, const int64_t* ptr, int64_t max_len, float drop_p, const uint64_t* seed,
                    uint64_t stream_id, const int64_t* rng_rowoff, float* dqkv, void* ws, size_t ws_bytes, advmil_stream_t stream);
int advmil_add_dropout_ln_fwd(const float* x, const float* o, const float* gamma, const float* beta, float eps, int64_t R,
                              int64_t d, float drop_p, const uint64_t* seed, uint64_t stream_id, const int64_t* rng_row, float* z,
                              float* y, float* mean, float* rstd, void* y_hi, void* y_lo, advmil_stream_t stream);
size_t advmil_add_dropout_ln_bwd_workspace_bytes(int64_t R, int64_t d);
int advmil_add_dropout_ln_bwd(const float* dy, const float* z, const float* gamma, const float* mean, const float* rstd, int64_t R,
                              int64_t d, float drop_p, const uint64_t* seed, uint64_t stream_id, const int64_t* rng_row, float* dx,
                              float* dob, float* dgamma, float* dbeta, int accumulate, void* ws, size_t ws_bytes,
                              advmil_stream_t stream);

int advmil_gate_score_fwd(const float* ab, const float* wc, const float* bc, float drop_p, const uint64_t* seed,
                          uint64_t stream_a, uint64_t stream_b, int64_t N, int64_t D, float* s, const int64_t* rng_row,
                          advmil_stream_t stream);
size_t advmil_softmax_pool_workspace_bytes(int64_t max_len, int64_t D, int nseg);
int advmil_softmax_pool_fwd(const float* s, const float* h, int64_t ldh, int64_t N, int64_t D, int nseg,
                            const int64_t* seg_ptr, int64_t max_len, float* A, float* pooled, void* ws, size_t ws_bytes,
                            advmil_stream_t stream);
size_t advmil_softmax_pool_mean_workspace_bytes(int64_t max_len, int64_t D, int nseg);
int advmil_softmax_pool_mean_fwd(const float* s, const float* h, int64_t ldh, int64_t N, int64_t D, int nseg, const int64_t* seg_ptr,
                                 int64_t max_len, float* A, float* pooled, float* mean, void* ws, size_t ws_bytes, advmil_stream_t stream);
int advmil_softmax_pool_bwd(const float* dpooled, const float* dA, const float* A, const float* h, int64_t ldh,
                            int64_t N, int64_t D, int nseg, const int64_t* seg_ptr, int64_t max_len, float* ds, void* ws,
                            size_t ws_bytes, advmil_stream_t stream);
int advmil_softmax_pool_fwd_planes(const float* s, const void* h_hi, const void* h_lo, int64_t ldh, int64_t N, int64_t D, int nseg,
                                   const int64_t* seg_ptr, int64_t max_len, float* A, float* pooled, void* ws, size_t ws_bytes,
                                   advmil_stream_t stream);
int advmil_softmax_pool_bwd_planes(const float* dpooled, const float* dA, const float* A, const void* h_hi, const void* h_lo, int64_t ldh,
                                   int64_t N, int64_t D, int nseg, const int64_t* seg_ptr, int64_t max_len, float* ds, void* ws,
                                   size_t ws_bytes, advmil_stream_t stream);
int advmil_dropout_planes(const void* in_hi, const void* in_lo, int64_t M, int64_t N, float drop_p, const uint64_t* seed, uint64_t stream_id,
                          const int64_t* rng_row, void* out_hi, void* out_lo, void* bits, float gate_p, uint64_t gate_stream_a,
                          uint64_t gate_stream_b, void* gate_bits_a, void* gate_bits_b, advmil_stream_t stream);
int advmil_seg_scale_rows(const float* dpooled, const float* A, const int32_t* rowseg, int64_t N, int64_t D, float* dh,
                          advmil_stream_t stream);
size_t advmil_gate_bwd_workspace_bytes(int64_t N, int64_t D);
int advmil_gate_bwd(const float* ab, const float* ds, const float* wc, float drop_p, const uint64_t* seed,
                    uint64_t stream_a, uint64_t stream_b, int64_t N, int64_t D, float* dG, float* dwc, float* dbc,
                    float* dbias, int accumulate, const int64_t* rng_row, void* dG_hi, void* dG_lo, int pair32, void* ws, size_t ws_bytes,
                    advmil_stream_t stream);

size_t advmil_colsum_workspace_bytes(int64_t M, int64_t N);
int advmil_act_dropout_bwd(const float* dy, const float* y, int act, float drop_p, const uint64_t* seed,
                           uint64_t stream_id, int64_t M, int64_t N, float* dpre, float* dbias, int accumulate,
                           const int64_t* rng_row, void* out_hi, void* out_lo, void* bits, void* ws, size_t ws_bytes,
                           advmil_stream_t stream);
int advmil_colsum(const float* x, int64_t M, int64_t N, float* out, int accumulate, void* ws, size_t ws_bytes,
                  advmil_stream_t stream);

int advmil_defer_sums(advmil_stream_t stream, int on);
int advmil_flush_sums(advmil_stream_t stream);
int advmil_pending_sums(advmil_stream_t stream);

int advmil_ln_relu_mean16_fwd(const float* y, const float* gamma, const float* beta, float eps, int64_t N, int64_t d,
                              float* emb, float* mean, float* rstd, void* emb_hi, void* emb_lo, int dup, advmil_stream_t stream);
size_t advmil_ln_relu_mean16_bwd_workspace_bytes(int64_t N, int64_t d);
int advmil_ln_relu_mean16_bwd(const float* demb, const float* y, const float* gamma, const float* beta,
                              const float* mean, const float* rstd, int64_t N, int64_t d, float* dy, float* dgamma,
                              float* dbeta, int accumulate, float* dycol, void* dy_hi, void* dy_lo, int dup, void* ws, size_t ws_bytes,
                              advmil_stream_t stream);

int advmil_ln_relu_fwd(const float* y, const float* gamma, const float* beta, float eps, int64_t N, int64_t d, float* out,
                       float* mean, float* rstd, advmil_stream_t stream);
size_t advmil_ln_relu_bwd_workspace_bytes(int64_t N, int64_t d);
int advmil_ln_relu_bwd(const float* dout, const float* y, const float* gamma, const float* beta, const float* mean,
                       const float* rstd, int64_t N, int64_t d, float* dy, float* dgamma, float* dbeta, int accumulate,
                       void* ws, size_t ws_bytes, advmil_stream_t stream);

int advmil_gcn_res_fwd(const float* h, const float* x, int64_t ldx, const float* gamma, const float* beta, float eps, int64_t N,
                       int64_t d, float drop_p, const uint64_t* seed, uint64_t stream_id, const int64_t* rng_row, float* out,
                       int64_t ldo, float* mean, float* rstd, advmil_stream_t stream);
size_t advmil_gcn_res_bwd_workspace_bytes(int64_t N, int64_t d);
int advmil_gcn_res_bwd(const float* dout, int64_t lddo, const float* h, const float* gamma, const float* beta, const float* mean,
                       const float* rstd, int64_t N, int64_t d, float drop_p, const uint64_t* seed, uint64_t stream_id,
                       const int64_t* rng_row, float* dh, float* dx, int64_t lddx, int dx_accumulate, float* dgamma, float* dbeta,
                       int accumulate, void* ws, size_t ws_bytes, advmil_stream_t stream);

int advmil_gapool16_fwd(const float* s, const float* z, int64_t ldz, int64_t N, int64_t d, float* A, float* emb, int dup,
                        advmil_stream_t stream);
int advmil_gapool16_bwd(const float* demb, const float* A, const float* z, int64_t ldz, int64_t N, int64_t d, int dup, float* ds,
                        float* dz, int dz_accumulate, advmil_stream_t stream);

int advmil_genconv_fwd(const float* x, const int32_t* rowptr_dst, const int32_t* col_src, const float* t, float eps, int64_t N,
                       int64_t C, float* out, float* lse, float* agg, advmil_stream_t stream);
size_t advmil_genconv_bwd_workspace_bytes(int64_t N, int64_t C);
int advmil_genconv_bwd(const float* dout, const float* x, const float* agg, const float* lse, const int32_t* rowptr_src,
                       const int32_t* col_dst, const float* t, float eps, int64_t N, int64_t C, float* dx, float* dt, void* ws,
                       size_t ws_bytes, advmil_stream_t stream);

int advmil_adam_blocks(int64_t n);
int advmil_adam_step(float* p, float* grad, float* m, float* v, const float* wd, int64_t n, float lr,
                     float beta1, float beta2, float eps, float grad_scale, float l1_coef, int32_t* step, void* p_hi, void* p_lo,
                     int tick, float* abs_partial, int clear_grad, advmil_stream_t stream);
int advmil_step_seed_tick(int32_t* step, int32_t* step2, uint64_t* seed, uint64_t inc, advmil_stream_t stream);
int advmil_abs_sum(const float* p, int64_t n, float* out, void* ws, size_t ws_bytes, advmil_stream_t stream);
size_t advmil_abs_sum_workspace_bytes(int64_t n);

enum { ADVMIL_OPT_ADAM = 0, ADVMIL_OPT_ADAMW = 1, ADVMIL_OPT_NADAM = 2, ADVMIL_OPT_RADAM = 3, ADVMIL_OPT_ADADELTA = 4 };
typedef struct {
  int32_t kind;
  int32_t lookahead;
  int64_t n;
  float* p;
  float* grad;
  float* s1;
  float* s2;
  const float* wd;
// ... 236 lines not shown
```

Baseline: 5869 bags/s.

## Read stacked gate weights via row remap and fold gate partial-sum into pooling

The gated-attention GEMM now reads the adjacent Wa/Wb weight planes directly through an in-kernel row remap (interleave or pair32), so the per-step gate_interleave copy of weights and biases is no longer needed. The separate gate_partial_sum launch is folded into the online softmax-pool partial kernel, which sums the per-block partials plus bc while loading scores and writes s back. The backward pass uses a pair32-aware transpose or a permuted view of the stacked weights. This trades weight-copy and launch overhead for extra index arithmetic in the DMA address path and more validation conditions. A two-B-source (b2_hi/lo) path is also plumbed into the kernel.

```diff
diff --git a/advmil_amd/_lib.py b/advmil_amd/_lib.py
--- a/advmil_amd/_lib.py
+++ b/advmil_amd/_lib.py
@@ -20,7 +20,19 @@
                 ("alpha", c_float), ("a_hi", c_void_p), ("a_lo", c_void_p), ("b_hi", c_void_p), ("b_lo", c_void_p),
                 ("c_hi", c_void_p), ("c_lo", c_void_p), ("gate_wc", c_void_p), ("gate_out", c_void_p), ("gate_np", c_int),
                 ("rng_row", c_void_p), ("c2", c_void_p), ("ldc2", c_int64), ("n_split", c_int64), ("bias2", c_void_p), ("colsum", c_void_p), ("maskbits", c_void_p), ("ldbits", c_int64),
-                ("gate_bits_a", c_void_p), ("gate_bits_b", c_void_p), ("ldgbits", c_int64), ("c_rows_pair32", c_int)]
+                ("gate_bits_a", c_void_p), ("gate_bits_b", c_void_p), ("ldgbits", c_int64), ("c_rows_pair32", c_int),
+                ("b_rowmap", c_int), ("b2_hi", c_void_p), ("b2_lo", c_void_p)]
+
+
+ROWMAP_NONE, ROWMAP_INTERLEAVE, ROWMAP_PAIR32 = 0, 1, 2
+
+
+def rowmap_src(mode, r, D):
+    if mode == ROWMAP_INTERLEAVE:
+        return (r & 1) * D + (r >> 1)
+    if mode == ROWMAP_PAIR32:
+        return ((r >> 5) & 1) * D + (((r >> 6) << 5) | (r & 31))
+    return r
 
 
 class DenseLayer(ctypes.Structure):
@@ -124,6 +136,8 @@
                                         c_int64, c_void_p, c_void_p, c_size_t, c_void_p]),
     "advmil_softmax_pool_fwd_planes": (c_int, [c_void_p, c_void_p, c_void_p, c_int64, c_int64, c_int64, c_int, c_void_p, c_int64, c_void_p,
                                                c_void_p, c_void_p, c_size_t, c_void_p]),
+    "advmil_softmax_pool_fwd_partials": (c_int, [c_void_p, c_int, c_void_p, c_void_p, c_void_p, c_void_p, c_int64, c_int64, c_int64, c_int,
+                                                 c_void_p, c_int64, c_void_p, c_void_p, c_void_p, c_void_p, c_size_t, c_void_p]),
     "advmil_softmax_pool_bwd_planes": (c_int, [c_void_p, c_void_p, c_void_p, c_void_p, c_void_p, c_int64, c_int64, c_int64, c_int, c_void_p,
                                                c_int64, c_void_p, c_void_p, c_size_t, c_void_p]),
     "advmil_dropout_planes": (c_int, [c_void_p, c_void_p, c_int64, c_int64, c_float, c_void_p, c_uint64, c_void_p, c_void_p, c_void_p, c_void_p,
diff --git a/advmil_amd/csrc/gemm_core.h b/advmil_amd/csrc/gemm_core.h
--- a/advmil_amd/csrc/gemm_core.h
+++ b/advmil_amd/csrc/gemm_core.h
@@ -84,6 +84,12 @@
 #define PITCH_PS(BKT) (BKT)
 __device__ __forceinline__ int ps_unit(int row, int unit, int units_per_row) {
   return units_per_row == 2 ? (unit ^ ((row >> 3) & 1)) : (unit ^ ((row >> 2) & (units_per_row - 1)));
+}
+
+__device__ __forceinline__ int64_t b_rowmap_src(int mode, int64_t r, int64_t D) {
+  if (mode == ADVMIL_ROWMAP_INTERLEAVE) return (r & 1) * D + (r >> 1);
+  if (mode == ADVMIL_ROWMAP_PAIR32) return ((r >> 5) & 1) * D + (((r >> 6) << 5) | (r & 31));
+  return r;
 }
 
 template <int ROWS, int BKT, int NT>
@@ -287,7 +293,7 @@
     for (int u = 0; u < (32 * TN + 63) / 64; ++u) {
       const int c = u * 64 + lane;
       const int64_t cg = cbase + c;
-      bv[u] = c >= 32 * TN ? 0.f : (cg < nsp ? (e.bias ? e.bias[cg] : 0.f) : (e.bias2 ? e.bias2[cg - nsp] : 0.f));
+      bv[u] = c >= 32 * TN ? 0.f : (cg < nsp ? (e.bias ? e.bias[PLAIN ? b_rowmap_src(e.b_rowmap, cg, N >> 1) : cg] : 0.f) : (e.bias2 ? e.bias2[cg - nsp] : 0.f));
     }
 #pragma unroll
     for (int u = 0; u < (32 * TM + 63) / 64; ++u) {
@@ -578,7 +584,12 @@
         float4 b4 = make_float4(0.f, 0.f, 0.f, 0.f);
         if (col < g.N) {
           w0 = e.gate_wc[col >> 1]; w1 = e.gate_wc[(col >> 1) + 1];
-          if (e.bias) b4 = *reinterpret_cast<const float4*>(e.bias + col);
+          if (e.bias && e.b_rowmap == ADVMIL_ROWMAP_INTERLEAVE) {
+            const int64_t j = col >> 1, D = g.N >> 1;
+            b4 = make_float4(e.bias[j], e.bias[D + j], e.bias[j + 1], e.bias[D + j + 1]);
+          } else if (e.bias) {
+            b4 = *reinterpret_cast<const float4*>(e.bias + col);
+          }
         }
 #pragma unroll
         for (int q = 0; q < 4; ++q) {
diff --git a/advmil_amd/csrc/gemm_host.hip b/advmil_amd/csrc/gemm_host.hip
--- a/advmil_amd/csrc/gemm_host.hip
+++ b/advmil_amd/csrc/gemm_host.hip
@@ -238,6 +238,22 @@
     if (epi->gate_np != advmil_gemm_f32_gate_blocks(tile, N)) return ADVMIL_EINVAL;
   }
   if (tile == 0 && pre == 3 && splits == 1) { int t = 0; advmil_gemm_f32_plan_planes(a_kc, b_kc, M, N, K, &t); if (t) tile = t; }
+  if (epi->b_rowmap || epi->b2_hi || epi->b2_lo) {
+    if (tile < 82 || tile > 86) return ADVMIL_EINVAL;
+    if (epi->b_rowmap && (epi->b2_hi || epi->b2_lo)) return ADVMIL_EINVAL;
+    if (epi->b_rowmap == ADVMIL_ROWMAP_INTERLEAVE) {
+      if (!epi->gate_wc || gate_store || (N & 3)) return ADVMIL_EINVAL;
+    } else if (epi->b_rowmap == ADVMIL_ROWMAP_PAIR32) {
+      if (!gate_store || (N & 63) || (((uintptr_t)epi->bias) & 15)) return ADVMIL_EINVAL;
+    } else if (epi->b_rowmap) {
+      return ADVMIL_EINVAL;
+    }
+    if (epi->b2_hi || epi->b2_lo) {
+      if (!epi->b2_hi || !epi->b2_lo || !epi->c2 || (epi->n_split & 15) || epi->n_split <= 0 || epi->n_split >= N ||
+          (((uintptr_t)epi->b2_hi | (uintptr_t)epi->b2_lo) & 15))
+        return ADVMIL_EINVAL;
+    }
+  }
   if (tile == 87) {
     if (epi->gate_wc || epi->rowv || epi->maskref || epi->maskbits || epi->colsum || epi->accumulate || epi->c2 || (epi->seed && epi->drop_p > 0.0f))
       return ADVMIL_EINVAL;
diff --git a/advmil_amd/csrc/gemm_nt_planes.hip b/advmil_amd/csrc/gemm_nt_planes.hip
--- a/advmil_amd/csrc/gemm_nt_planes.hip
+++ b/advmil_amd/csrc/gemm_nt_planes.hip
@@ -38,26 +38,39 @@
   int mt_i, nt_i;
   tile_of(v, mt_i, nt_i);
   uint32_t soff[PPW];
+  const int rmap = g.epi.b_rowmap;
+  const int64_t Dmap = g.N >> 1;
   auto set_src = [&](int mt, int nt, int lane) {
 #pragma unroll
     for (int it = 0; it < PPW; ++it) {
       const int prow = (wave + NW * it) * RPP + lane / LPR;
       int r;
-      int64_t ld, row0;
-      if (prow < BM_) { r = prow; ld = g.lda; row0 = (int64_t)mt * BM_; }
-      else if (prow < AROWS) { r = prow - BM_; ld = g.lda; row0 = (int64_t)mt * BM_; }
-      else if (prow < AROWS + BN_) { r = prow - AROWS; ld = g.ldb; row0 = (int64_t)nt * BN_; }
-      else { r = prow - AROWS - BN_; ld = g.ldb; row0 = (int64_t)nt * BN_; }
-      soff[it] = (uint32_t)(((row0 + r) * ld + ps_unit(r, lane % LPR, LPR) * 8) * 2);
+      int64_t ld, srow;
+      if (prow < BM_) { r = prow; ld = g.lda; srow = (int64_t)mt * BM_ + r; }
+      else if (prow < AROWS) { r = prow - BM_; ld = g.lda; srow = (int64_t)mt * BM_ + r; }
+      else {
+        r = prow < AROWS + BN_ ? prow - AROWS : prow - AROWS - BN_;
+        ld = g.ldb;
+        srow = b_rowmap_src(rmap, (int64_t)nt * BN_ + r, Dmap);
+      }
+      soff[it] = (uint32_t)((srow * ld + ps_unit(r, lane % LPR, LPR) * 8) * 2);
     }
   };
   set_src(mt_i, nt_i, (int)threadIdx.x & 63);
   int64_t dA = 0, dB = 0;
+  const bool two_b = g.epi.b2_hi != nullptr;
+  const int64_t b2_back = g.epi.n_split * g.ldb * 2;
+  int nB0 = nt_i * BN_, nB1 = nB0;
   auto dma = [&](int buf, int64_t k0, bool next) {
 #pragma unroll
     for (int it = 0; it < PPW; ++it) {
       const int p0 = (wave + NW * it) * RPP;
       const char* base = reinterpret_cast<const char*>(p0 < BM_ ? g.epi.a_hi : (p0 < AROWS ? g.epi.a_lo : (p0 < AROWS + BN_ ? g.epi.b_hi : g.epi.b_lo)));
+      if (p0 >= AROWS && two_b) {
+        const bool lo = p0 >= AROWS + BN_;
+        if ((next ? nB1 : nB0) + (p0 - AROWS - (lo ? BN_ : 0)) >= g.epi.n_split)
+          base = reinterpret_cast<const char*>(lo ? g.epi.b2_lo : g.epi.b2_hi) - b2_back;
+      }
       base += (k0 + (next ? (p0 < AROWS ? dA : dB) : 0)) * 2;
       __builtin_amdgcn_global_load_lds((const GLB_AS void*)(base + soff[it]), (LDS_AS void*)(lds + buf * BUF_HW + (wave + NW * it) * 512), 16, 0, 0);
     }
@@ -77,7 +90,8 @@
     int mt_n = mt_i, nt_n = nt_i;
     if (has_next) tile_of(v + G, mt_n, nt_n);
     dA = (int64_t)(mt_n - mt_i) * BM_ * g.lda;
-    dB = (int64_t)(nt_n - nt_i) * BN_ * g.ldb;
+    dB = (int64_t)(nt_n - nt_i) * (rmap ? BN_ / 2 : BN_) * g.ldb;
+    nB0 = nt_i * BN_; nB1 = nt_n * BN_;
     f32x16 acc[TM][TN];
 #pragma unroll
     for (int a = 0; a < TM; ++a)
diff --git a/advmil_amd/csrc/pool.hip b/advmil_amd/csrc/pool.hip
--- a/advmil_amd/csrc/pool.hip
+++ b/advmil_amd/csrc/pool.hip
@@ -321,7 +321,9 @@
 __global__ __launch_bounds__(256) void pool_partial8_online_kernel(const float* __restrict__ s, const float* __restrict__ h, int64_t ldh,
                                                                    int64_t N, int64_t D, const int64_t* __restrict__ seg_ptr,
                                                                    float* __restrict__ partial, float* __restrict__ pstats, int rpb,
-                                                                   float* __restrict__ mpartial, const bf16raw* __restrict__ hlo = nullptr) {
+                                                                   float* __restrict__ mpartial, const bf16raw* __restrict__ hlo = nullptr,
+                                                                   const float* __restrict__ gpart = nullptr, int gnp = 0,
+                                                                   const float* __restrict__ gbc = nullptr, float* __restrict__ s_out = nullptr) {
   __shared__ __attribute__((aligned(16))) float red[2048];
   __shared__ float wts[512];
   __shared__ float wred[8];
@@ -346,7 +348,17 @@
   float mx = -INFINITY;
   for (int r = tid; r < rpb; r += 256) {
     const int64_t n = r0 + r;
-    const float v = n < end ? s[n] : -INFINITY;
+    float v = -INFINITY;
+    if (n < end) {
+      if (gpart) {
+        float a = 0.f;
+        for (int j = 0; j < gnp; ++j) a += gpart[n * gnp + j];
+        v = a + (gbc ? gbc[0] : 0.f);
+        s_out[n] = v;
+      } else {
+        v = s[n];
+      }
+    }
     wts[r] = v;
     mx = fmaxf(mx, v);
   }
@@ -507,7 +519,7 @@
 
 static int softmax_pool_fwd_impl(const float* s, const float* h, int64_t ldh, int64_t N, int64_t D, int nseg, const int64_t* seg_ptr,
                                  int64_t max_len, float* A, float* pooled, float* mean, void* ws, size_t ws_bytes, hipStream_t stream,
-                                 const bf16raw* hlo = nullptr);
+                                 const bf16raw* hlo = nullptr, const float* gpart = nullptr, int gnp = 0, const float* gbc = nullptr);
 
 extern "C" int advmil_softmax_pool_fwd(const float* s, const float* h, int64_t ldh, int64_t N, int64_t D, int nseg,
                                        const int64_t* seg_ptr, int64_t max_len, float* A, float* pooled, void* ws,
@@ -523,6 +535,14 @@
                                (const bf16raw*)h_lo);
 }
 
+extern "C" int advmil_softmax_pool_fwd_partials(const float* partial, int np, const float* bc, float* s, const void* h, const void* h_lo,
+                                                int64_t ldh, int64_t N, int64_t D, int nseg, const int64_t* seg_ptr, int64_t max_len, float* A,
+                                                float* pooled, float* mean, void* ws, size_t ws_bytes, advmil_stream_t stream_) {
+  if (!partial || np <= 0 || !h) return ADVMIL_EINVAL;
+  return softmax_pool_fwd_impl(s, (const float*)h, ldh, N, D, nseg, seg_ptr, max_len, A, pooled, mean, ws, ws_bytes, (hipStream_t)stream_,
+                               (const bf16raw*)h_lo, partial, np, bc);
+}
+
 static inline size_t pool_mean_offset_bytes(int64_t max_len, int64_t D, int nseg) {
   return (advmil_softmax_pool_workspace_bytes(max_len, D, nseg) + 15) / 16 * 16;
 }
@@ -541,7 +561,7 @@
 
 static int softmax_pool_fwd_impl(const float* s, const float* h, int64_t ldh, int64_t N, int64_t D, int nseg, const int64_t* seg_ptr,
                                  int64_t max_len, float* A, float* pooled, float* mean, void* ws, size_t ws_bytes, hipStream_t stream,
-                                 const bf16raw* hlo) {
+                                 const bf16raw* hlo, const float* gpart, int gnp, const float* gbc) {
   if (!s || !h || !A || !pooled || !ws || N <= 0 || D <= 0 || (D & 3) || D > 1024 || (ldh & 3)) return ADVMIL_EINVAL;
   if (ldh < D || ((uintptr_t)h & 15)) return ADVMIL_EINVAL;
   if (hlo && (((uintptr_t)hlo & 15) || (D & 7) || (ldh & 7) || D < 16 || mean)) return ADVMIL_EINVAL;
@@ -553,12 +573,18 @@
   float* stats = (float*)ws;
   float* partial = stats + 4 * nseg;
   const int nblk = (int)pool_nblk(max_len);
+  float* const s_out = const_cast<float*>(s);
+  if (gpart && ((D & 7) || D < 16 || nblk > POOL_ONLINE_MAX_NBLK)) {
+    const int rc = advmil_gate_partial_sum(gpart, gnp, gbc, N, s_out, (advmil_stream_t)stream);
+    if (rc) return rc;
+    gpart = nullptr;
+  }
   if ((D & 7) == 0 && D >= 16 && nblk <= POOL_ONLINE_MAX_NBLK) {
     float* pstats = partial + (int64_t)nseg * nblk * D;
     if (mean) {
       float* mpartial = (float*)ws + pool_mean_offset_bytes(max_len, D, nseg) / sizeof(float);
       hipLaunchKernelGGL((pool_partial8_online_kernel<true, false>), dim3(nblk, nseg), dim3(256), 0, stream, s, h, ldh, N, D, seg_ptr, partial, pstats,
-                         rows_per_block(max_len), mpartial, (const bf16raw*)nullptr);
+                         rows_per_block(max_len), mpartial, (const bf16raw*)nullptr, gpart, gnp, gbc, s_out);
       ADVMIL_LAUNCH_CHECK();
       hipLaunchKernelGGL(pool_merge_online_kernel, dim3((unsigned)((D + 15) / 16), nseg), dim3(256), 0, stream, partial, pstats, nblk, D, s,
                          N, seg_ptr, pooled, A, stats, (const float*)mpartial, mean);
@@ -567,10 +593,10 @@
     }
     if (hlo)
       hipLaunchKernelGGL((pool_partial8_online_kernel<false, true>), dim3(nblk, nseg), dim3(256), 0, stream, s, h, ldh, N, D, seg_ptr, partial,
-                         pstats, rows_per_block(max_len), (float*)nullptr, hlo);
+                         pstats, rows_per_block(max_len), (float*)nullptr, hlo, gpart, gnp, gbc, s_out);
     else
       hipLaunchKernelGGL((pool_partial8_online_kernel<false, false>), dim3(nblk, nseg), dim3(256), 0, stream, s, h, ldh, N, D, seg_ptr, partial,
-                         pstats, rows_per_block(max_len), (float*)nullptr, (const bf16raw*)nullptr);
+                         pstats, rows_per_block(max_len), (float*)nullptr, (const bf16raw*)nullptr, gpart, gnp, gbc, s_out);
     ADVMIL_LAUNCH_CHECK();
     hipLaunchKernelGGL(pool_merge_online_kernel, dim3((unsigned)((D + 15) / 16), nseg), dim3(256), 0, stream, partial, pstats, nblk, D, s,
                        N, seg_ptr, pooled, A, stats, (const float*)nullptr, (float*)nullptr);
diff --git a/advmil_amd/ops.py b/advmil_amd/ops.py
--- a/advmil_amd/ops.py
+++ b/advmil_amd/ops.py
@@ -344,14 +344,28 @@
     return bool(rows >= 4096 and USE_PLANES and get_gemm_mode() == "bf16x3" and (SLAB_PLANES_ANY or gemm_plan_planes(rows, 128, C)))
 
 
-def planes_transposed(pl):
+def planes_transposed(pl, pair32=False):
     R, C = pl.hi.shape
     out = Planes.alloc((C, R), pl.hi.device)
     d = (pl.lo.data_ptr() - pl.hi.data_ptr()) // 2
     do = (out.lo.data_ptr() - out.hi.data_ptr()) // 2
-    if (pl.hi.untyped_storage().data_ptr() == pl.lo.untyped_storage().data_ptr() and d > 0 and pl.hi.stride() == pl.lo.stride()
-            and pl.hi.stride(1) == 1):
-        src = pl.hi.as_strided((2, C, R), (d, 1, pl.hi.stride(0)), pl.hi.storage_offset())
+    ld = pl.hi.stride(0)
+    one = (pl.hi.untyped_storage().data_ptr() == pl.lo.untyped_storage().data_ptr() and d > 0 and pl.hi.stride() == pl.lo.stride()
+           and pl.hi.stride(1) == 1)
+    if pair32:
+        if R % 64:
+            raise ValueError("planes_transposed(pair32=True) needs whole pair blocks (rows % 64 == 0)")
+        D = R // 2
+        if one:
+            src = pl.hi.as_strided((2, C, D // 32, 2, 32), (d, 1, 32 * ld, D * ld, ld), pl.hi.storage_offset())
+            dst = out.hi.as_strided((2, C, D // 32, 2, 32), (do, R, 64, 32, 1), out.hi.storage_offset())
+            dst.copy_(src)
+        else:
+            for s_, o_ in ((pl.hi, out.hi), (pl.lo, out.lo)):
+                o_.view(C, D // 32, 2, 32).copy_(s_.as_strided((C, D // 32, 2, 32), (s_.stride(1), 32 * s_.stride(0), D * s_.stride(0), s_.stride(0)),
+                                                               s_.storage_offset()))
+    elif one:
+        src = pl.hi.as_strided((2, C, R), (d, 1, ld), pl.hi.storage_offset())
         dst = out.hi.as_strided((2, C, R), (do, R, 1), out.hi.storage_offset())
         dst.copy_(src)
     else:
@@ -401,7 +415,7 @@
 def gemm(A, B, a_kc, b_kc, M, N, K, out=None, ldc=None, bias=None, act0=0, act1=None, act_split=None, drop_p=0.0,
          seed=None, stream_id=0, rowv=None, colv=None, rowseg=None, maskref=None, mask_scale=1.0, accumulate=False,
          alpha=1.0, splits=None, tile=0, a_planes=None, b_planes=None, c_planes=None, c_planes_only=False, gate_wc=None, rng_row=None,
-         colsum=None, maskbits=None, gate_bits=None, c_rows_pair32=False):
+         colsum=None, maskbits=None, gate_bits=None, c_rows_pair32=False, b_rowmap=0):
     planes_only_a = A is None
     if planes_only_a:
         if a_planes is None or get_gemm_mode() != "bf16x3":
@@ -513,6 +527,8 @@
             e.gate_bits_a, e.gate_bits_b, e.ldgbits = gate_bits[0].data_ptr(), gate_bits[1].data_ptr(), gate_bits[0].stride(0)
     if c_rows_pair32:
         e.c_rows_pair32 = 1
+    if b_rowmap:
+        e.b_rowmap = b_rowmap
     if colsum is not None:
         e.colsum = colsum.data_ptr()
     if maskbits is not None:
@@ -587,18 +603,9 @@
     M, K = x.shape
     N1, N2 = W1.shape[0], W2.shape[0]
 
-    def pair(pl, N):
-        hi, lo = pl.hi.reshape(N, K), pl.lo.reshape(N, K)
-        d = (lo.data_ptr() - hi.data_ptr()) // 2
-        if hi.untyped_storage().data_ptr() != lo.untyped_storage().data_ptr() or d <= 0 or not hi.is_contiguous() or not lo.is_contiguous():
-            return None
-        return hi.as_strided((2, N, K), (d, K, 1), hi.storage_offset())
-    v1, v2 = pair(w1pl, N1), pair(w2pl, N2)
-    if v1 is not None and v2 is not None:
-        stk = torch.cat((v1, v2), dim=1)
-        wcat = Planes(stk[0], stk[1])
-    else:
-        wcat = Planes(torch.cat((w1pl.hi.reshape(N1, K), w2pl.hi.reshape(N2, K)), dim=0), torch.cat((w1pl.lo.reshape(N1, K), w2pl.lo.reshape(N2, K)), dim=0))
+    w1h, w1l, w2h, w2l = w1pl.hi.reshape(N1, K), w1pl.lo.reshape(N1, K), w2pl.hi.reshape(N2, K), w2pl.lo.reshape(N2, K)
+    if not all(w.is_contiguous() for w in (w1h, w1l, w2h, w2l)) or N1 % 16:
+        raise ValueError("gemm_two_layers: weight planes must be dense [N, K] and N1 a multiple of 16")
     dev = x.device
     y1 = _token(M, N1, dev) if y1_planes_only else torch.empty(M, N1, dtype=torch.float32, device=dev)
     y2 = torch.empty(M, N2, dtype=torch.float32, device=dev)
@@ -611,7 +618,8 @@
     e.act0, e.act1, e.act_split = act1, act2, N1
     e.alpha = 1.0
     e.a_hi, e.a_lo = xpl.hi.data_ptr(), xpl.lo_ptr()
-    e.b_hi, e.b_lo = wcat.hi.data_ptr(), wcat.lo.data_ptr()
+    e.b_hi, e.b_lo = w1h.data_ptr(), w1l.data_ptr()
+    e.b2_hi, e.b2_lo = w2h.data_ptr(), w2l.data_ptr()
     if cpl is not None:
         e.c_hi, e.c_lo = cpl.hi.data_ptr(), cpl.lo.data_ptr()
     e.c2, e.ldc2, e.n_split = y2.data_ptr(), N2, N1
@@ -689,8 +697,17 @@
         return self._div[key]
 
 
-def softmax_pool(s, h, N, D, seg=None, hpl=None):
+def pending_scores(part, bc):
+    s = torch.empty(part.shape[0], dtype=torch.float32, device=part.device)
+    s._advmil_partials = (part, bc)
+    return s
+
+
+def softmax_pool(s, h, N, D, seg=None, hpl=None, partials=None):
     L = _lib.lib()
+    if partials is None and getattr(s, "_advmil_partials", None) is not None:
+        partials = s._advmil_partials
+        s._advmil_partials = None
     nseg = 1 if seg is None else seg.nseg
     mlen = N if seg is None else seg.max_len
     A = torch.empty(N, dtype=torch.float32, device=h.device)
@@ -700,7 +717,14 @@
     big = STAMPS is not None and N * D >= (1 << 24)
     if big:
         _stamp("b", "softmax_pool_fwd", (N, D, nseg), 4.0 * N * D + 12.0 * N)
-    if hpl is not None:
+    if partials is not None:
+        part, bc = partials
+        hsrc = h if hpl is None else hpl.hi
+        _lib.check(L.advmil_softmax_pool_fwd_partials(_p(part), part.shape[1], _p(None if bc is None else bc.reshape(-1)), _p(s), _p(hsrc),
+                                                      _p(None if hpl is None else hpl.lo), hsrc.stride(0), N, D, nseg,
+                                                      _p(None if seg is None else seg.ptr), mlen, _p(A), _p(pooled), None, _p(ws), wsb, _stream()),
+                   "softmax_pool_fwd_partials")
+    elif hpl is not None:
         _lib.check(L.advmil_softmax_pool_fwd_planes(_p(s), _p(hpl.hi), _p(hpl.lo), hpl.hi.stride(0), N, D, nseg,
                                                     _p(None if seg is None else seg.ptr), mlen, _p(A), _p(pooled), _p(ws), wsb, _stream()),
                    "softmax_pool_fwd_planes")
@@ -712,7 +736,7 @@
     return A, pooled
 
 
-def softmax_pool_mean(s, h, N, D, seg=None):
+def softmax_pool_mean(s, h, N, D, seg=None, partials=None):
     L = _lib.lib()
     nseg = 1 if seg is None else seg.nseg
     mlen = N if seg is None else seg.max_len
@@ -721,6 +745,12 @@
     mean = torch.empty(nseg, D, dtype=torch.float32, device=h.device)
     wsb = L.advmil_softmax_pool_mean_workspace_bytes(mlen, D, nseg)
     ws = _ws(wsb, h.device)
+    if partials is not None:
+        part, bc = partials
+        _lib.check(L.advmil_softmax_pool_fwd_partials(_p(part), part.shape[1], _p(None if bc is None else bc.reshape(-1)), _p(s), _p(h), None,
+                                                      h.stride(0), N, D, nseg, _p(None if seg is None else seg.ptr), mlen, _p(A), _p(pooled),
+                                                      _p(mean), _p(ws), wsb, _stream()), "softmax_pool_fwd_partials")
+        return A, pooled, mean
     _lib.check(L.advmil_softmax_pool_mean_fwd(_p(s), _p(h), h.stride(0), N, D, nseg, _p(None if seg is None else seg.ptr), mlen, _p(A),
                                               _p(pooled), _p(mean), _p(ws), wsb, _stream()), "softmax_pool_mean_fwd")
     return A, pooled, mean
@@ -932,6 +962,17 @@
         stride = (cols, 1) if cols else (1,)
         return a.detach().as_strided(shape, stride, a.storage_offset()), True
     return torch.cat([a.detach(), b.detach()], dim=0).contiguous(), False
+
+
+def _gate_stacked(Wa, ba, Wb, bb, D, hpl):
+    if not (_adjacent(Wa, Wb) and _adjacent(ba, bb)) or D % 8 or ba.data_ptr() % 16:
+        return None
+    if hpl is None or hpl.single or hpl.ptrs() & 15 or hpl.hi.stride(0) % 8:
+        return None
+    pl = _stacked_planes(Wa, Wb, D)
+    if pl is None or pl.ptrs() & 15:
+        return None
+    return _stack2(Wa, Wb, D, D)[0], _stack2(ba, bb, D, 0)[0], pl
 
 
 class DropoutFn(torch.autograd.Function):
@@ -1268,22 +1309,33 @@
         stale = hpl is not None and hpl.fp32_stale
         ppl = hpl if stale else None
         if FUSED_GATE_SCORE and p <= 0.0 and N >= 4096 and nograd:
-            Wi, bi, wipl = gate_interleave(Wa.detach(), ba.detach(), Wb.detach(), bb.detach(), D, planes=hpl is not None)
-            s = gate_partial_sum(gemm(h, Wi, True, True, N, 2 * D, D, bias=bi, gate_wc=wcv, a_planes=hpl, b_planes=wipl), bc.detach())
-            A, pooled = softmax_pool(s, h, N, D, seg, ppl)
+            wst = _gate_stacked(Wa, ba, Wb, bb, D, hpl) if gemm_plan_planes(N, 2 * D, D) else None
+            if wst is not None:
+                Wab, bab, wabpl = wst
+                part = gemm(h, Wab, True, True, N, 2 * D, D, bias=bab, gate_wc=wcv, a_planes=hpl, b_planes=wabpl, b_rowmap=_lib.ROWMAP_INTERLEAVE)
+                s = pending_scores(part, bc.detach())
+                A, pooled = softmax_pool(s, h, N, D, seg, ppl)
+            else:
+                Wi, bi, wipl = gate_interleave(Wa.detach(), ba.detach(), Wb.detach(), bb.detach(), D, planes=hpl is not None)
+                s = gate_partial_sum(gemm(h, Wi, True, True, N, 2 * D, D, bias=bi, gate_wc=wcv, a_planes=hpl, b_planes=wipl), bc.detach())
+                A, pooled = softmax_pool(s, h, N, D, seg, ppl)
             ctx.mark_non_differentiable(s)
             return pooled, A, s
         gs = [_arena_grad(t) for t in (Wa, ba, Wb, bb, wc, bc)]
         arena_ok = all(g is not None for g in gs) and _adjacent(gs[0], gs[2]) and _adjacent(gs[1], gs[3])
+        wst = None
         if (gate is not None and FUSED_GATE_TRAIN and p > 0.0 and hpl is not None and arena_ok and N % 256 == 0 and D % 64 == 0
                 and get_gemm_mode() == "bf16x3" and gemm_plan_planes(N, 2 * D, D) and gemm_plan_tn_planes(2 * D, D, N)[1] > 1
                 and gemm_plan_planes(N, D, 2 * D)):
-            Wp, bp, wppl = gate_interleave(Wa.detach(), ba.detach(), Wb.detach(), bb.detach(), D, planes=True, pair32=True)
-            ab, part = gemm(h, Wp, True, True, N, 2 * D, D, bias=bp, gate_wc=wcv, drop_p=p, a_planes=hpl, b_planes=wppl, gate_bits=gate)
-            s = gate_partial_sum(part, bc.detach())
+            wst = _gate_stacked(Wa, ba, Wb, bb, D, hpl)
+        if wst is not None:
+            Wab, bab, wabpl = wst
+            ab, part = gemm(h, Wab, True, True, N, 2 * D, D, bias=bab, gate_wc=wcv, drop_p=p, a_planes=hpl, b_planes=wabpl, gate_bits=gate,
+                            b_rowmap=_lib.ROWMAP_PAIR32)
+            s = pending_scores(part, bc.detach())
             A, pooled = softmax_pool(s, h, N, D, seg, ppl)
-            ctx.save_for_backward(h, Wp, ab, A, wcv)
-            ctx.hpl, ctx.wabpl, ctx.pair32 = hpl, wppl, True
+            ctx.save_for_backward(h, Wab, ab, A, wcv)
+            ctx.hpl, ctx.wabpl, ctx.pair32 = hpl, wabpl, True
             ctx.cfg = (p, seed, sa, sb, N, D, wc.shape, seg, rr)
             ctx.arena = (gs[0].as_strided((2 * D, D), (D, 1), gs[0].storage_offset()),
                          gs[1].as_strided((2 * D,), (1,), gs[1].storage_offset()), gs[4].view(-1), gs[5])
@@ -1353,12 +1405,14 @@
         if fuse is not None and dh_nt:
             nrow = int(_lib.lib().advmil_gemm_f32_colsum_rows(dh_tile, N, D))
             tile = dh_tile
-            wtpl = planes_transposed(ctx.wabpl)
+            wtpl = planes_transposed(ctx.wabpl, pair32=pair32)
         elif fuse is not None:
             tile = gemm_plan(N, D, 2 * D, True, False)[0]
             nrow = int(_lib.lib().advmil_gemm_f32_colsum_rows(tile, N, D)) if pre_a_tile_ok(tile, True, False) else 0
             if nrow <= 0:
                 fuse = None
+        if pair32 and need_h and wtpl is None:
+            Wab = Wab.view(2, D // 32, 32, D).permute(1, 0, 2, 3).reshape(2 * D, D)
         if fuse is not None:
             p1, gb1, mbits = fuse
             dpl = Planes.alloc((N, D), h.device)
diff --git a/include/advmil_hip.h b/include/advmil_hip.h
--- a/include/advmil_hip.h
+++ b/include/advmil_hip.h
@@ -48,7 +48,13 @@
   const uint32_t* gate_bits_b;
   int64_t ldgbits;
   int c_rows_pair32;
+  int b_rowmap;
+  const void* b2_hi;
+  const void* b2_lo;
 } advmil_epilogue_t;
+#define ADVMIL_ROWMAP_NONE 0
+#define ADVMIL_ROWMAP_INTERLEAVE 1
+#define ADVMIL_ROWMAP_PAIR32 2
 
 size_t advmil_gemm_f32_workspace_bytes(int64_t M, int64_t N, int splits);
 int advmil_gemm_f32(int a_kc, int b_kc, int64_t M, int64_t N, int64_t K, const float* A, int64_t lda,
@@ -107,6 +113,9 @@
 int advmil_softmax_pool_bwd(const float* dpooled, const float* dA, const float* A, const float* h, int64_t ldh,
                             int64_t N, int64_t D, int nseg, const int64_t* seg_ptr, int64_t max_len, float* ds, void* ws,
                             size_t ws_bytes, advmil_stream_t stream);
+int advmil_softmax_pool_fwd_partials(const float* partial, int np, const float* bc, float* s, const void* h, const void* h_lo, int64_t ldh,
+                                     int64_t N, int64_t D, int nseg, const int64_t* seg_ptr, int64_t max_len, float* A, float* pooled,
+                                     float* mean, void* ws, size_t ws_bytes, advmil_stream_t stream);
 int advmil_softmax_pool_fwd_planes(const float* s, const void* h_hi, const void* h_lo, int64_t ldh, int64_t N, int64_t D, int nseg,
                                    const int64_t* seg_ptr, int64_t max_len, float* A, float* pooled, void* ws, size_t ws_bytes,
                                    advmil_stream_t stream);
```

After: 5774 bags/s. -1.6%, worse.
